# CESNET/GPUJPEG

Measured on NVIDIA H100. Metric: Mpix/s encode+decode 8k RGB q75, higher is better.
Workload: dtype f32+i32 (u8 in, i16 coefficients)

## Files before the change

gpujpeg_b200/csrc/gj_dct.cu:

```cuda
#include <cuda_runtime.h>
#include <stdint.h>
#include <stdlib.h>
#include <string.h>

#include "gj_device.cuh"
#include "gj_internal.h"
#include "gj_launch.cuh"

namespace {

constexpr int TB = 64;
constexpr int NT = 192;
constexpr int STRIP_PX = TB * 8;
constexpr int GROUPS = 8 * (STRIP_PX / 4);
constexpr int BLK_F = 68;
constexpr int K1_SMEM = 3 * TB * BLK_F * 4;
constexpr int K1_OUT_STRIDE = 9;
constexpr int K4_PLANE = 8 * STRIP_PX;

struct FdctParams {
    float fwd_zz[2][64];
};
struct IdctParams {
    uint16_t q_zz[GJ_MAX_COMP][64];
// ... 312 lines not shown
            const int row = g >> 7, gx = g & 127, px0 = gx * 4;
            float4 y4 = make_float4(0.f, 0.f, 0.f, 0.f), cb4 = y4, cr4 = y4;
            if ( row < vh && px0 < vw ) {
                const uint32_t a0 = w0[it], a1 = w1[it], a2 = w2[it];
                gj_rgb_to_ycbcr_m(gj_byte_as_magic(a0, 0), gj_byte_as_magic(a0, 1), gj_byte_as_magic(a0, 2), y4.x, cb4.x, cr4.x);
                gj_rgb_to_ycbcr_m(gj_byte_as_magic(a0, 3), gj_byte_as_magic(a1, 0), gj_byte_as_magic(a1, 1), y4.y, cb4.y, cr4.y);
                gj_rgb_to_ycbcr_m(gj_byte_as_magic(a1, 2), gj_byte_as_magic(a1, 3), gj_byte_as_magic(a2, 0), y4.z, cb4.z, cr4.z);
                gj_rgb_to_ycbcr_m(gj_byte_as_magic(a2, 1), gj_byte_as_magic(a2, 2), gj_byte_as_magic(a2, 3), y4.w, cb4.w, cr4.w);
                if ( px0 + 4 > vw ) {
                    if ( px0 + 1 >= vw ) { y4.y = cb4.y = cr4.y = 0.f; }
                    if ( px0 + 2 >= vw ) { y4.z = cb4.z = cr4.z = 0.f; }
                    if ( px0 + 3 >= vw ) { y4.w = cb4.w = cr4.w = 0.f; }
                }
            }
            *reinterpret_cast<float4*>(s_y + (half * TB + (gx >> 1)) * BLK_F + row * 8 + (gx & 1) * 4) = y4;
            const int srow = half * 8 + row;
            if ( VS == 1 || (srow & 1) == 0 ) {
                const int crow = srow / VS;
                if ( HS == 1 ) {
                    const int off = (gx >> 1) * BLK_F + crow * 8 + (gx & 1) * 4;
                    *reinterpret_cast<float4*>(s_c + off) = cb4;
                    *reinterpret_cast<float4*>(s_c + CB * BLK_F + off) = cr4;
                }
                else {
                    const int off = (gx >> 2) * BLK_F + crow * 8 + (gx & 3) * 2;
                    *reinterpret_cast<float2*>(s_c + off) = make_float2(cb4.x, cb4.z);
                    *reinterpret_cast<float2*>(s_c + CB * BLK_F + off) = make_float2(cr4.x, cr4.z);
                }
            }
        }
    }
    __syncthreads();

    auto locate = [&](int t, int& comp, int& bx, int& by) {
        if ( t < TB * VS ) {
            comp = 0;
            bx = bx0 + (t & (TB - 1));
            by = blockIdx.y * VS + t / TB;
        }
        else {
            const int u = t - TB * VS;
            comp = 1 + u / CB;
            bx = bx0 / HS + u % CB;
            by = blockIdx.y;
        }
        return bx < grid.bcx[comp] && by < grid.bcy[comp];
    };
    int comp, bx, by;
    const bool active = locate(threadIdx.x, comp, bx, by);
    float v[64];
    {
        const float4* in = reinterpret_cast<const float4*>(s_y + threadIdx.x * BLK_F);
#pragma unroll
        for ( int i = 0; i < 16; i++ ) {
            const float4 t = in[i];
            v[4 * i] = t.x; v[4 * i + 1] = t.y; v[4 * i + 2] = t.z; v[4 * i + 3] = t.w;
        }
    }
    __syncthreads();
    gj_fdct_block(v);
    uint4* const s_out = reinterpret_cast<uint4*>(smem);
    {
        uint32_t packed[32];
        const uint64_t nz = quantise_pack(v, prm.fwd_zz[comp == 0 ? 0 : 1], packed);
        if ( active ) nzmask[(size_t)grid.blk_off[comp] + (size_t)by * grid.bcx[comp] + bx] = nz;
#pragma unroll
        for ( int i = 0; i < 8; i++ )
            s_out[threadIdx.x * K1_OUT_STRIDE + i] = make_uint4(packed[4 * i], packed[4 * i + 1], packed[4 * i + 2], packed[4 * i + 3]);
    }
    __syncthreads();
#pragma unroll
    for ( int k = 0; k < 8; k++ ) {
        const int q = threadIdx.x + k * NTS;
        const int slot = q >> 3, part = q & 7;
        int c2, bx2, by2;
        if ( locate(slot, c2, bx2, by2) ) {
            const size_t bi = (size_t)grid.blk_off[c2] + (size_t)by2 * grid.bcx[c2] + bx2;
            reinterpret_cast<uint4*>(coef + bi * 64)[part] = s_out[slot * K1_OUT_STRIDE + part];
        }
    }
}


template <int VEC, int FLAVOUR, bool DEQ>
__global__ void __launch_bounds__(NT)
k_idct_rgb444(const int16_t* __restrict__ coef, int bcx, int nblk, uint8_t* __restrict__ raw, int width, int height,
              size_t pitch, const __grid_constant__ IdctParams prm)
{
    gj_pdl_wait();
    __shared__ __align__(16) uint8_t s_pl[3 * K4_PLANE];

    const int bx0 = blockIdx.x * TB;
    const int by = blockIdx.y;
    const int x0 = bx0 * 8;
    const int vw = min(STRIP_PX, width - x0);
    const int vh = min(8, height - by * 8);

    {
        const int comp = threadIdx.x >> 6;
        const int b = threadIdx.x & 63;
        if ( bx0 + b < bcx ) {
            const uint4* src = reinterpret_cast<const uint4*>(coef + ((size_t)comp * nblk + (size_t)by * bcx + bx0 + b) * 64);
            uint32_t packed[32];
#pragma unroll
            for ( int i = 0; i < 8; i++ ) {
                const uint4 t = __ldg(src + i);
                packed[4 * i] = t.x; packed[4 * i + 1] = t.y; packed[4 * i + 2] = t.z; packed[4 * i + 3] = t.w;
            }
            const uint16_t* q = prm.q_zz[comp];
            uint32_t px[16];
            if ( FLAVOUR == 0 ) {
                int v[64];
#pragma unroll
                for ( int k = 0; k < 64; k++ ) {
                    const int c = (k & 1) ? (int)packed[k >> 1] >> 16 : (int)(short)(packed[k >> 1] & 0xFFFFu);
                    v[gj_zz2nat(k)] = DEQ ? gj_s16(c * (int)(short)q[k]) : c;
                }
                gj_idct_int_block_px(v);
#pragma unroll
                for ( int i = 0; i < 16; i++ )
                    px[i] = pack4_sat_u8(v[4 * i], v[4 * i + 1], v[4 * i + 2], v[4 * i + 3]);
            }
            else {
                float f[64];
#pragma unroll
                for ( int k = 0; k < 64; k++ ) {
                    const int c = (k & 1) ? (int)packed[k >> 1] >> 16 : (int)(short)(packed[k >> 1] & 0xFFFFu);
                    f[gj_zz2nat(k)] = (float)(c * (int)q[k]);
                }
                gj_idct_float_block(f);
#pragma unroll
                for ( int i = 0; i < 16; i++ )
                    px[i] = pack4_sat_u8(GJ_RINT(GJ_FADD(f[4 * i], 128.0f)), GJ_RINT(GJ_FADD(f[4 * i + 1], 128.0f)),
                                         GJ_RINT(GJ_FADD(f[4 * i + 2], 128.0f)), GJ_RINT(GJ_FADD(f[4 * i + 3], 128.0f)));
            }
            uint8_t* dst = s_pl + comp * K4_PLANE + b * 8;
#pragma unroll
            for ( int r = 0; r < 8; r++ )
                *reinterpret_cast<uint2*>(dst + r * STRIP_PX) = make_uint2(px[2 * r], px[2 * r + 1]);
        }
    }
    __syncthreads();

    uint8_t* out = raw + (size_t)by * 8 * pitch + (size_t)x0 * 3;
    for ( int g = threadIdx.x; g < GROUPS; g += NT ) {
        const int row = g >> 7, gx = g & 127;
        const int px0 = gx * 4;
        if ( row >= vh || px0 >= vw ) continue;
        const uint32_t yw = *reinterpret_cast<const uint32_t*>(s_pl + row * STRIP_PX + px0);
        const uint32_t bw = *reinterpret_cast<const uint32_t*>(s_pl + K4_PLANE + row * STRIP_PX + px0);
        const uint32_t rw = *reinterpret_cast<const uint32_t*>(s_pl + 2 * K4_PLANE + row * STRIP_PX + px0);
        int r[4], gg[4], bb[4];
#pragma unroll
        for ( int j = 0; j < 4; j++ )
            gj_ycbcr_to_rgb_raw((yw >> (8 * j)) & 0xFF, (bw >> (8 * j)) & 0xFF, (rw >> (8 * j)) & 0xFF, r[j], gg[j], bb[j]);
        const uint32_t o0 = pack4_sat_u8(r[0], gg[0], bb[0], r[1]);
        const uint32_t o1 = pack4_sat_u8(gg[1], bb[1], r[2], gg[2]);
        const uint32_t o2 = pack4_sat_u8(bb[2], r[3], gg[3], bb[3]);
        uint8_t* p = out + (size_t)row * pitch + gx * 12;
        if ( VEC == 4 && px0 + 4 <= vw ) {
            uint32_t* w = reinterpret_cast<uint32_t*>(p);
            w[0] = o0;
            w[1] = o1;
            w[2] = o2;
        }
        else {
            const int nb = min(12, (vw - px0) * 3);
            const uint32_t o[3] = {o0, o1, o2};
#pragma unroll
            for ( int i = 0; i < 12; i++ )
                if ( i < nb ) p[i] = (uint8_t)(o[i >> 2] >> (8 * (i & 3)));
        }
    }
}

template <int HS, int VS, int VEC, int FLAVOUR, bool DEQ>
__global__ void __launch_bounds__(TB * VS + 2 * TB / HS)
k_idct_rgb_ss(const int16_t* __restrict__ coef, const __grid_constant__ SsGrid grid, uint8_t* __restrict__ raw, int width,
              int height, size_t pitch, const __grid_constant__ IdctParams prm)
{
    gj_pdl_wait();
    constexpr int NTS = TB * VS + 2 * TB / HS;
    constexpr int CB = TB / HS;
    constexpr int CW = STRIP_PX / HS;
    __shared__ __align__(16) uint8_t s_y[8 * VS * STRIP_PX];
    __shared__ __align__(16) uint8_t s_c[2][8 * CW];

    const int bx0 = blockIdx.x * TB;
    const int x0 = bx0 * 8;
    const int y0 = blockIdx.y * 8 * VS;
    const int vw = min(STRIP_PX, width - x0);
    const int vh = min(8 * VS, height - y0);

    {
        int comp, bx, by;
        uint8_t* dst;
        int dpitch;
        if ( threadIdx.x < TB * VS ) {
            comp = 0;
            const int b = threadIdx.x & (TB - 1), byl = threadIdx.x / TB;
            bx = bx0 + b;
            by = blockIdx.y * VS + byl;
            dst = s_y + byl * 8 * STRIP_PX + b * 8;
            dpitch = STRIP_PX;
        }
        else {
            const int u = threadIdx.x - TB * VS;
            comp = 1 + u / CB;
            bx = bx0 / HS + u % CB;
            by = blockIdx.y;
            dst = s_c[comp - 1] + (u % CB) * 8;
            dpitch = CW;
        }
        if ( bx < grid.bcx[comp] && by < grid.bcy[comp] ) {
            const uint4* src =
                reinterpret_cast<const uint4*>(coef + ((size_t)grid.blk_off[comp] + (size_t)by * grid.bcx[comp] + bx) * 64);
            uint32_t packed[32];
#pragma unroll
            for ( int i = 0; i < 8; i++ ) {
                const uint4 t = __ldg(src + i);
                packed[4 * i] = t.x; packed[4 * i + 1] = t.y; packed[4 * i + 2] = t.z; packed[4 * i + 3] = t.w;
            }
            const uint16_t* q = prm.q_zz[comp];
            uint32_t px[16];
            if ( FLAVOUR == 0 ) {
                int v[64];
#pragma unroll
                for ( int k = 0; k < 64; k++ ) {
                    const int c = (k & 1) ? (int)packed[k >> 1] >> 16 : (int)(short)(packed[k >> 1] & 0xFFFFu);
                    v[gj_zz2nat(k)] = DEQ ? gj_s16(c * (int)(short)q[k]) : c;
                }
                gj_idct_int_block_px(v);
#pragma unroll
                for ( int i = 0; i < 16; i++ )
                    px[i] = pack4_sat_u8(v[4 * i], v[4 * i + 1], v[4 * i + 2], v[4 * i + 3]);
            }
            else {
                float f[64];
#pragma unroll
                for ( int k = 0; k < 64; k++ ) {
                    const int c = (k & 1) ? (int)packed[k >> 1] >> 16 : (int)(short)(packed[k >> 1] & 0xFFFFu);
                    f[gj_zz2nat(k)] = (float)(c * (int)q[k]);
                }
                gj_idct_float_block(f);
#pragma unroll
                for ( int i = 0; i < 16; i++ )
                    px[i] = pack4_sat_u8(GJ_RINT(GJ_FADD(f[4 * i], 128.0f)), GJ_RINT(GJ_FADD(f[4 * i + 1], 128.0f)),
                                         GJ_RINT(GJ_FADD(f[4 * i + 2], 128.0f)), GJ_RINT(GJ_FADD(f[4 * i + 3], 128.0f)));
            }
#pragma unroll
            for ( int r = 0; r < 8; r++ )
                *reinterpret_cast<uint2*>(dst + r * dpitch) = make_uint2(px[2 * r], px[2 * r + 1]);
        }
    }
    __syncthreads();

    uint8_t* out = raw + (size_t)y0 * pitch + (size_t)x0 * 3;
    for ( int g = threadIdx.x; g < GROUPS * VS; g += NTS ) {
        const int row = g >> 7, gx = g & 127;
        const int px0 = gx * 4;
        if ( row >= vh || px0 >= vw ) continue;
        const uint32_t yw = *reinterpret_cast<const uint32_t*>(s_y + row * STRIP_PX + px0);
        uint32_t bw, rw;
        if ( HS == 1 ) {
            bw = *reinterpret_cast<const uint32_t*>(s_c[0] + (row / VS) * CW + px0);
            rw = *reinterpret_cast<const uint32_t*>(s_c[1] + (row / VS) * CW + px0);
        }
        else {
            const uint32_t b2 = *reinterpret_cast<const uint16_t*>(s_c[0] + (row / VS) * CW + px0 / 2);
            const uint32_t r2 = *reinterpret_cast<const uint16_t*>(s_c[1] + (row / VS) * CW + px0 / 2);
            bw = __byte_perm(b2, 0u, 0x1100);
            rw = __byte_perm(r2, 0u, 0x1100);
        }
        int r[4], gg[4], bb[4];
#pragma unroll
        for ( int j = 0; j < 4; j++ )
            gj_ycbcr_to_rgb_raw((yw >> (8 * j)) & 0xFF, (bw >> (8 * j)) & 0xFF, (rw >> (8 * j)) & 0xFF, r[j], gg[j], bb[j]);
        const uint32_t o0 = pack4_sat_u8(r[0], gg[0], bb[0], r[1]);
        const uint32_t o1 = pack4_sat_u8(gg[1], bb[1], r[2], gg[2]);
        const uint32_t o2 = pack4_sat_u8(bb[2], r[3], gg[3], bb[3]);
        uint8_t* p = out + (size_t)row * pitch + gx * 12;
        if ( VEC == 4 && px0 + 4 <= vw ) {
            uint32_t* w = reinterpret_cast<uint32_t*>(p);
            w[0] = o0;
            w[1] = o1;
            w[2] = o2;
        }
        else {
            const int nb = min(12, (vw - px0) * 3);
            const uint32_t o[3] = {o0, o1, o2};
#pragma unroll
            for ( int i = 0; i < 12; i++ )
                if ( i < nb ) p[i] = (uint8_t)(o[i >> 2] >> (8 * (i & 3)));
        }
    }
}

struct SampleGrid {
    unsigned long long off[GJ_MAX_COMP], pitch[GJ_MAX_COMP];
    int xs[GJ_MAX_COMP], cw[GJ_MAX_COMP], ch[GJ_MAX_COMP], bcx[GJ_MAX_COMP], blk_off[GJ_MAX_COMP + 1], table[GJ_MAX_COMP];
};
constexpr int SG_THREADS = 128;

__global__ void __launch_bounds__(SG_THREADS)
k_fdct_samples(const uint8_t* __restrict__ raw, const __grid_constant__ SampleGrid g, int total_blocks,
               int16_t* __restrict__ coef, uint64_t* __restrict__ nzmask, const __grid_constant__ FdctParams prm)
{
    const int bi = blockIdx.x * SG_THREADS + threadIdx.x;
    if ( bi >= total_blocks ) return;
    const int comp = (bi >= g.blk_off[1]) + (bi >= g.blk_off[2]) + (bi >= g.blk_off[3]);
    const int local = bi - g.blk_off[comp];
    const int by = local / g.bcx[comp], bx = local - by * g.bcx[comp];
    const int vw = min(8, g.cw[comp] - bx * 8), vh = min(8, g.ch[comp] - by * 8);
    const uint8_t* src = raw + g.off[comp] + (size_t)by * 8 * g.pitch[comp] + (size_t)bx * 8 * g.xs[comp];
    float v[64];
    const bool rows8 = g.xs[comp] == 1 && vw == 8 && ((reinterpret_cast<uintptr_t>(src) | g.pitch[comp]) & 7) == 0;
#pragma unroll
    for ( int y = 0; y < 8; y++ ) {
        if ( y < vh && rows8 ) {
            const uint2 t = __ldg(reinterpret_cast<const uint2*>(src + (size_t)y * g.pitch[comp]));
#pragma unroll
            for ( int x = 0; x < 8; x++ )
                v[8 * y + x] = (float)(((x < 4 ? t.x : t.y) >> (8 * (x & 3))) & 0xFFu);
        }
        else {
#pragma unroll
            for ( int x = 0; x < 8; x++ )
                v[8 * y + x] = (y < vh && x < vw) ? (float)__ldg(src + (size_t)y * g.pitch[comp] + (size_t)x * g.xs[comp]) : 0.f;
        }
    }
    gj_fdct_block(v);
    quantise_store(v, prm.fwd_zz[g.table[comp]], coef + (size_t)bi * 64, nzmask + bi);
}

template <int FLAVOUR, bool DEQ>
__global__ void __launch_bounds__(SG_THREADS)
k_idct_samples(const int16_t* __restrict__ coef, const __grid_constant__ SampleGrid g, int total_blocks,
               uint8_t* __restrict__ raw, const __grid_constant__ IdctParams prm)
{
    const int bi = blockIdx.x * SG_THREADS + threadIdx.x;
    if ( bi >= total_blocks ) return;
    const int comp = (bi >= g.blk_off[1]) + (bi >= g.blk_off[2]) + (bi >= g.blk_off[3]);
    const int local = bi - g.blk_off[comp];
    const int by = local / g.bcx[comp], bx = local - by * g.bcx[comp];
    const int vw = min(8, g.cw[comp] - bx * 8), vh = min(8, g.ch[comp] - by * 8);
    if ( vw <= 0 || vh <= 0 ) return;
    const uint4* src = reinterpret_cast<const uint4*>(coef + (size_t)bi * 64);
    uint32_t packed[32];
#pragma unroll
    for ( int i = 0; i < 8; i++ ) {
        const uint4 t = __ldg(src + i);
        packed[4 * i] = t.x; packed[4 * i + 1] = t.y; packed[4 * i + 2] = t.z; packed[4 * i + 3] = t.w;
    }
    const uint16_t* q = prm.q_zz[comp];
    uint32_t px[16];
    if ( FLAVOUR == 0 ) {
        int v[64];
#pragma unroll
        for ( int k = 0; k < 64; k++ ) {
            const int c = (k & 1) ? (int)packed[k >> 1] >> 16 : (int)(short)(packed[k >> 1] & 0xFFFFu);
            v[gj_zz2nat(k)] = DEQ ? gj_s16(c * (int)(short)q[k]) : c;
        }
        gj_idct_int_block_px(v);
#pragma unroll
        for ( int i = 0; i < 16; i++ )
            px[i] = pack4_sat_u8(v[4 * i], v[4 * i + 1], v[4 * i + 2], v[4 * i + 3]);
    }
    else {
        float f[64];
#pragma unroll
        for ( int k = 0; k < 64; k++ ) {
            const int c = (k & 1) ? (int)packed[k >> 1] >> 16 : (int)(short)(packed[k >> 1] & 0xFFFFu);
            f[gj_zz2nat(k)] = (float)(c * (int)q[k]);
        }
        gj_idct_float_block(f);
#pragma unroll
        for ( int i = 0; i < 16; i++ )
            px[i] = pack4_sat_u8(GJ_RINT(GJ_FADD(f[4 * i], 128.0f)), GJ_RINT(GJ_FADD(f[4 * i + 1], 128.0f)),
                                 GJ_RINT(GJ_FADD(f[4 * i + 2], 128.0f)), GJ_RINT(GJ_FADD(f[4 * i + 3], 128.0f)));
    }
    uint8_t* dst = raw + g.off[comp] + (size_t)by * 8 * g.pitch[comp] + (size_t)bx * 8 * g.xs[comp];
    const bool rows8 = g.xs[comp] == 1 && vw == 8 && ((reinterpret_cast<uintptr_t>(dst) | g.pitch[comp]) & 7) == 0;
#pragma unroll
    for ( int y = 0; y < 8; y++ ) {
        if ( y >= vh ) continue;
        if ( rows8 ) {
            *reinterpret_cast<uint2*>(dst + (size_t)y * g.pitch[comp]) = make_uint2(px[2 * y], px[2 * y + 1]);
        }
        else {
#pragma unroll
            for ( int x = 0; x < 8; x++ )
                if ( x < vw ) dst[(size_t)y * g.pitch[comp] + (size_t)x * g.xs[comp]] = (uint8_t)(px[2 * y + (x >> 2)] >> (8 * (x & 3)));
        }
    }
}

int pick_vec(const void* p, size_t pitch)
{
    const uintptr_t a = reinterpret_cast<uintptr_t>(p) | pitch;
    return (a & 3) == 0 ? 4 : 1;
}

}

static int launch_fdct_rgb444(const uint8_t* d_raw, int width, int height, int pitch, int16_t* d_coef, uint64_t* d_nzmask,
                              int bcx, int bcy, int nblk, const struct gj_dev_enc_tables* h_tables, gj_stream_t stream)
{
    FdctParams prm;
    memcpy(prm.fwd_zz, h_tables->fwd_zz, sizeof prm.fwd_zz);
    const dim3 grid((bcx + TB - 1) / TB, bcy);
    static int attr_done[64];
    int dev = 0;
    if ( cudaGetDevice(&dev) != cudaSuccess || dev < 0 || dev >= 64 ) return -1;
    if ( !__atomic_load_n(&attr_done[dev], __ATOMIC_ACQUIRE) ) {
        if ( cudaFuncSetAttribute(k_fdct_rgb444<4>, cudaFuncAttributeMaxDynamicSharedMemorySize, K1_SMEM) != cudaSuccess ||
             cudaFuncSetAttribute(k_fdct_rgb444<1>, cudaFuncAttributeMaxDynamicSharedMemorySize, K1_SMEM) != cudaSuccess )
            return -1;
        __atomic_store_n(&attr_done[dev], 1, __ATOMIC_RELEASE);
    }
    static int use_bulk = -1;
    if ( use_bulk < 0 ) {
        const char* e = getenv("GPUJPEG_B200_K1");
        use_bulk = e && strcmp(e, "bulk") == 0;
    }
    const bool aligned16 = ((reinterpret_cast<uintptr_t>(d_raw) | (size_t)pitch) & 15) == 0 && ((size_t)(width % STRIP_PX) * 3) % 16 == 0;
    if ( use_bulk && aligned16 ) {
        static int bulk_attr[64];
        if ( !__atomic_load_n(&bulk_attr[dev], __ATOMIC_ACQUIRE) ) {
            if ( cudaFuncSetAttribute(k_fdct_rgb444_bulk, cudaFuncAttributeMaxDynamicSharedMemorySize, K1T_SMEM) != cudaSuccess ) return -1;
            __atomic_store_n(&bulk_attr[dev], 1, __ATOMIC_RELEASE);
        }
        int sms = 132;
        cudaDeviceGetAttribute(&sms, cudaDevAttrMultiProcessorCount, dev);
        const int n_strips = (int)grid.x * (int)grid.y;
        const int ctas = n_strips < sms * 3 ? n_strips : sms * 3;
        k_fdct_rgb444_bulk<<<ctas, NT, K1T_SMEM, stream>>>(d_raw, width, height, (size_t)pitch, d_coef, d_nzmask, bcx, bcy, nblk, prm);
    }
    else if ( pick_vec(d_raw, (size_t)pitch) == 4 )
        gj_launch_pdl(k_fdct_rgb444<4>, grid, dim3(NT), K1_SMEM, stream, d_raw, width, height, (size_t)pitch, d_coef, d_nzmask, bcx, nblk, prm);
    else
        gj_launch_pdl(k_fdct_rgb444<1>, grid, dim3(NT), K1_SMEM, stream, d_raw, width, height, (size_t)pitch, d_coef, d_nzmask, bcx, nblk, prm);
    return cudaGetLastError() == cudaSuccess ? 0 : -1;
}

extern "C" int gj_launch_fdct_rgb444(const uint8_t* d_raw, int width, int height, int pitch, int16_t* d_coef,
                                     uint64_t* d_nzmask, int bcx, int bcy, const struct gj_dev_enc_tables* h_tables,
                                     gj_stream_t stream)
{
    return launch_fdct_rgb444(d_raw, width, height, pitch, d_coef, d_nzmask, bcx, bcy, bcx * bcy, h_tables, stream);
}
extern "C" int gj_launch_fdct_rgb444_rows(const uint8_t* d_raw, int width, int height, int pitch, int16_t* d_coef,
                                          uint64_t* d_nzmask, int bcx, int bcy, int by0, int by1,
                                          const struct gj_dev_enc_tables* h_tables, gj_stream_t stream)
{
    if ( by0 < 0 || by1 > bcy || by0 >= by1 ) return -1;
    const int rows = (by1 * 8 < height ? by1 * 8 : height) - by0 * 8;
    return launch_fdct_rgb444(d_raw + (ptrdiff_t)by0 * 8 * pitch, width, rows, pitch, d_coef + (size_t)by0 * bcx * 64,
                              d_nzmask + (size_t)by0 * bcx, bcx, by1 - by0, bcx * bcy, h_tables, stream);
}

static int launch_idct_rgb444(const int16_t* d_coef, int bcx, int bcy, int nblk, const int comp_tq[3], uint8_t* d_raw, int width,
                              int height, int pitch, int idct_flavour, int coef_dequantized,
                              const struct gj_dev_dec_tables* h_tables, gj_stream_t stream)
{
    IdctParams prm;
    for ( int c = 0; c < 3; c++ )
        memcpy(prm.q_zz[c], h_tables->qinv_zz[comp_tq[c]], sizeof prm.q_zz[c]);
    const dim3 grid((bcx + TB - 1) / TB, bcy);
    const int vec = pick_vec(d_raw, (size_t)pitch);
    if ( idct_flavour != 0 && coef_dequantized ) return -1;
#define GJ_K4(V, F, D) gj_launch_pdl(k_idct_rgb444<V, F, D>, grid, dim3(NT), 0, stream, d_coef, bcx, nblk, d_raw, width, height, (size_t)pitch, prm)
    if ( idct_flavour == 0 && coef_dequantized ) {
        if ( vec == 4 ) GJ_K4(4, 0, false); else GJ_K4(1, 0, false);
    }
    else if ( idct_flavour == 0 ) {
        if ( vec == 4 ) GJ_K4(4, 0, true); else GJ_K4(1, 0, true);
    }
    else {
        if ( vec == 4 ) GJ_K4(4, 1, true); else GJ_K4(1, 1, true);
    }
#undef GJ_K4
    return cudaGetLastError() == cudaSuccess ? 0 : -1;
}
extern "C" int gj_launch_idct_rgb444(const int16_t* d_coef, int bcx, int bcy, const int comp_tq[3], uint8_t* d_raw,
                                     int width, int height, int pitch, int idct_flavour, int coef_dequantized,
                                     const struct gj_dev_dec_tables* h_tables, gj_stream_t stream)
{
    return launch_idct_rgb444(d_coef, bcx, bcy, bcx * bcy, comp_tq, d_raw, width, height, pitch, idct_flavour, coef_dequantized,
                              h_tables, stream);
}
extern "C" int gj_launch_idct_rgb444_rows(const int16_t* d_coef, int bcx, int bcy, int by0, int by1, const int comp_tq[3],
                                          uint8_t* d_raw, int width, int height, int pitch, int idct_flavour,
                                          int coef_dequantized, const struct gj_dev_dec_tables* h_tables, gj_stream_t stream)
{
    if ( by0 < 0 || by1 > bcy || by0 >= by1 ) return -1;
    const int rows = (by1 * 8 < height ? by1 * 8 : height) - by0 * 8;
    return launch_idct_rgb444(d_coef + (size_t)by0 * bcx * 64, bcx, by1 - by0, bcx * bcy, comp_tq, d_raw + (ptrdiff_t)by0 * 8 * pitch,
                              width, rows, pitch, idct_flavour, coef_dequantized, h_tables, stream);
}

static int ss_grid_rows(SsGrid* sg, const struct gj_comp_geo comp[3], int my0, int my1, int height)
{
    const int vs = comp[0].vs;
    for ( int c = 0; c < 3; c++ ) {
        const int per = c == 0 ? vs : 1;
        const int lo = my0 * per, hi = my1 * per < comp[c].bcy ? my1 * per : comp[c].bcy;
        sg->bcx[c] = comp[c].bcx;
        sg->bcy[c] = hi > lo ? hi - lo : 0;
        sg->blk_off[c] = comp[c].blk_off + lo * comp[c].bcx;
    }
    const int y0 = my0 * 8 * vs, y1 = my1 * 8 * vs < height ? my1 * 8 * vs : height;
    return y1 > y0 ? y1 - y0 : 0;
}

extern "C" int gj_launch_fdct_rgb_ss_rows(const uint8_t* d_raw, int width, int height, int pitch, int16_t* d_coef,
                                          uint64_t* d_nzmask, const struct gj_comp_geo comp[3], int my0, int my1,
                                          const struct gj_dev_enc_tables* h_tables, gj_stream_t stream)
{
    FdctParams prm;
    memcpy(prm.fwd_zz, h_tables->fwd_zz, sizeof prm.fwd_zz);
    const int hs = comp[0].hs, vs = comp[0].vs;
    if ( comp[1].hs != 1 || comp[1].vs != 1 || comp[2].hs != 1 || comp[2].vs != 1 ) return -1;
    const int mcu_rows = (comp[0].bcy + vs - 1) / vs;
    if ( my0 < 0 || my1 > mcu_rows || my0 >= my1 ) return -1;
    SsGrid sg;
    height = ss_grid_rows(&sg, comp, my0, my1, height);
    d_raw += (ptrdiff_t)my0 * 8 * vs * pitch;
    const dim3 grid((comp[0].bcx + TB - 1) / TB, my1 - my0);
    const int vec = pick_vec(d_raw, (size_t)pitch);
    static int attr_done[64][4];
    int dev = 0;
    if ( cudaGetDevice(&dev) != cudaSuccess || dev < 0 || dev >= 64 ) return -1;
#define GJ_K1SS(H, V)                                                                                                        \
    do {                                                                                                                     \
        constexpr int nt = TB * V + 2 * TB / H;                                                                              \
        constexpr int sm = nt * BLK_F * 4;                                                                                   \
        if ( !__atomic_load_n(&attr_done[dev][H * 2 + V - 3], __ATOMIC_ACQUIRE) ) {                                          \
            if ( cudaFuncSetAttribute(k_fdct_rgb_ss<H, V, 4>, cudaFuncAttributeMaxDynamicSharedMemorySize, sm) != cudaSuccess || \
                 cudaFuncSetAttribute(k_fdct_rgb_ss<H, V, 1>, cudaFuncAttributeMaxDynamicSharedMemorySize, sm) != cudaSuccess )  \
                return -1;                                                                                                   \
            __atomic_store_n(&attr_done[dev][H * 2 + V - 3], 1, __ATOMIC_RELEASE);                                           \
        }                                                                                                                    \
        if ( vec == 4 )                                                                                                      \
            gj_launch_pdl(k_fdct_rgb_ss<H, V, 4>, grid, dim3(nt), sm, stream, d_raw, width, height, (size_t)pitch, d_coef, d_nzmask, sg, prm); \
        else                                                                                                                 \
            gj_launch_pdl(k_fdct_rgb_ss<H, V, 1>, grid, dim3(nt), sm, stream, d_raw, width, height, (size_t)pitch, d_coef, d_nzmask, sg, prm); \
    } while ( 0 )
    if ( hs == 2 && vs == 2 ) GJ_K1SS(2, 2);
    else if ( hs == 2 && vs == 1 ) GJ_K1SS(2, 1);
    else if ( hs == 1 && vs == 2 ) GJ_K1SS(1, 2);
    else return -1;
#undef GJ_K1SS
    return cudaGetLastError() == cudaSuccess ? 0 : -1;
}
extern "C" int gj_launch_fdct_rgb_ss(const uint8_t* d_raw, int width, int height, int pitch, int16_t* d_coef,
                                     uint64_t* d_nzmask, const struct gj_comp_geo comp[3],
                                     const struct gj_dev_enc_tables* h_tables, gj_stream_t stream)
{
    const int vs = comp[0].vs > 0 ? comp[0].vs : 1;
    return gj_launch_fdct_rgb_ss_rows(d_raw, width, height, pitch, d_coef, d_nzmask, comp, 0, (comp[0].bcy + vs - 1) / vs, h_tables,
                                      stream);
}

extern "C" int gj_launch_idct_rgb_ss_rows(const int16_t* d_coef, const struct gj_comp_geo comp[3], int my0, int my1,
                                          const int comp_tq[3], uint8_t* d_raw, int width, int height, int pitch, int idct_flavour,
                                          int coef_dequantized, const struct gj_dev_dec_tables* h_tables, gj_stream_t stream)
{
    IdctParams prm;
    for ( int c = 0; c < 3; c++ )
        memcpy(prm.q_zz[c], h_tables->qinv_zz[comp_tq[c]], sizeof prm.q_zz[c]);
    const int hs = comp[0].hs, vs = comp[0].vs;
    if ( comp[1].hs != 1 || comp[1].vs != 1 || comp[2].hs != 1 || comp[2].vs != 1 ) return -1;
    if ( idct_flavour != 0 && coef_dequantized ) return -1;
    const int mcu_rows = (comp[0].bcy + vs - 1) / vs;
    if ( my0 < 0 || my1 > mcu_rows || my0 >= my1 ) return -1;
    SsGrid sg;
    height = ss_grid_rows(&sg, comp, my0, my1, height);
    d_raw += (ptrdiff_t)my0 * 8 * vs * pitch;
    const dim3 grid((comp[0].bcx + TB - 1) / TB, my1 - my0);
    const int vec = pick_vec(d_raw, (size_t)pitch);
#define GJ_K4SS2(H, V, VE, F, D) \
    gj_launch_pdl(k_idct_rgb_ss<H, V, VE, F, D>, grid, dim3(TB * V + 2 * TB / H), 0, stream, d_coef, sg, d_raw, width, height, (size_t)pitch, prm)
#define GJ_K4SS(H, V)                                                                  \
    do {                                                                               \
        if ( idct_flavour == 0 && coef_dequantized ) {                                 \
            if ( vec == 4 ) GJ_K4SS2(H, V, 4, 0, false); else GJ_K4SS2(H, V, 1, 0, false); \
        }                                                                              \
        else if ( idct_flavour == 0 ) {                                                \
            if ( vec == 4 ) GJ_K4SS2(H, V, 4, 0, true); else GJ_K4SS2(H, V, 1, 0, true);   \
        }                                                                              \
        else {                                                                         \
            if ( vec == 4 ) GJ_K4SS2(H, V, 4, 1, true); else GJ_K4SS2(H, V, 1, 1, true);   \
        }                                                                              \
    } while ( 0 )
    if ( hs == 2 && vs == 2 ) GJ_K4SS(2, 2);
    else if ( hs == 2 && vs == 1 ) GJ_K4SS(2, 1);
    else if ( hs == 1 && vs == 2 ) GJ_K4SS(1, 2);
    else return -1;
#undef GJ_K4SS
#undef GJ_K4SS2
    return cudaGetLastError() == cudaSuccess ? 0 : -1;
}
extern "C" int gj_launch_idct_rgb_ss(const int16_t* d_coef, const struct gj_comp_geo comp[3], const int comp_tq[3],
                                     uint8_t* d_raw, int width, int height, int pitch, int idct_flavour,
                                     int coef_dequantized, const struct gj_dev_dec_tables* h_tables, gj_stream_t stream)
{
    const int vs = comp[0].vs > 0 ? comp[0].vs : 1;
    return gj_launch_idct_rgb_ss_rows(d_coef, comp, 0, (comp[0].bcy + vs - 1) / vs, comp_tq, d_raw, width, height, pitch,
                                      idct_flavour, coef_dequantized, h_tables, stream);
}

static int sample_grid(SampleGrid* sg, const struct gj_raw_layout* raw, const struct gj_comp_geo* comp, int comp_count,
                       const uint8_t* comp_tbl)
{
    if ( comp_count < 1 || comp_count > GJ_MAX_COMP || raw->comp_count != comp_count ) return -1;
    memset(sg, 0, sizeof *sg);
    int total = 0;
    for ( int c = 0; c < GJ_MAX_COMP; c++ ) {
        const int k = c < comp_count ? c : comp_count - 1;
        sg->off[c] = raw->comp[k].off;
        sg->pitch[c] = raw->comp[k].pitch;
        sg->xs[c] = raw->comp[k].xs;
        sg->cw[c] = comp[k].width;
        sg->ch[c] = comp[k].height;
        sg->bcx[c] = comp[k].bcx;
        sg->table[c] = comp_tbl ? comp_tbl[k] : ((c == 0 || c == 3) ? 0 : 1);
        if ( c < comp_count ) {
            sg->blk_off[c] = comp[c].blk_off;
            total = comp[c].blk_off + comp[c].nblk;
        }
    }
    for ( int c = comp_count; c <= GJ_MAX_COMP; c++ )
        sg->blk_off[c] = 0x7FFFFFFF;
    return total;
}

extern "C" int gj_launch_fdct_samples(const uint8_t* d_raw, const struct gj_raw_layout* raw, int16_t* d_coef,
                                      uint64_t* d_nzmask, const struct gj_comp_geo* comp, int comp_count,
                                      const uint8_t* comp_tbl, const struct gj_dev_enc_tables* h_tables, gj_stream_t stream)
{
    FdctParams prm;
    memcpy(prm.fwd_zz, h_tables->fwd_zz, sizeof prm.fwd_zz);
    SampleGrid sg;
    const int total = sample_grid(&sg, raw, comp, comp_count, comp_tbl);
    if ( total <= 0 ) return -1;
    k_fdct_samples<<<(total + SG_THREADS - 1) / SG_THREADS, SG_THREADS, 0, stream>>>(d_raw, sg, total, d_coef, d_nzmask, prm);
    return cudaGetLastError() == cudaSuccess ? 0 : -1;
}

extern "C" int gj_launch_idct_samples(const int16_t* d_coef, const struct gj_comp_geo* comp, int comp_count, const int* comp_tq,
                                      uint8_t* d_raw, const struct gj_raw_layout* raw, int idct_flavour, int coef_dequantized,
                                      const struct gj_dev_dec_tables* h_tables, gj_stream_t stream)
{
    IdctParams prm;
    for ( int c = 0; c < GJ_MAX_COMP; c++ )
        memcpy(prm.q_zz[c], h_tables->qinv_zz[comp_tq[c < comp_count ? c : 0]], sizeof prm.q_zz[c]);
    SampleGrid sg;
    const int total = sample_grid(&sg, raw, comp, comp_count, nullptr);
    if ( total <= 0 ) return -1;
    if ( idct_flavour != 0 && coef_dequantized ) return -1;
    const int grid = (total + SG_THREADS - 1) / SG_THREADS;
    if ( idct_flavour == 0 && coef_dequantized )
        k_idct_samples<0, false><<<grid, SG_THREADS, 0, stream>>>(d_coef, sg, total, d_raw, prm);
    else if ( idct_flavour == 0 )
        k_idct_samples<0, true><<<grid, SG_THREADS, 0, stream>>>(d_coef, sg, total, d_raw, prm);
    else
        k_idct_samples<1, true><<<grid, SG_THREADS, 0, stream>>>(d_coef, sg, total, d_raw, prm);
    return cudaGetLastError() == cudaSuccess ? 0 : -1;
}
```

gpujpeg_b200/csrc/gj_decoder.c:

```c
#include <stdlib.h>
#include <string.h>

#include "gj_internal.h"

#define GJ_MK_OTHER_CAP 256
#define GJ_CTA_BYTES0 (64 * 1024)
#define GJ_MK_WORDS (8 + 4 * GJ_MK_OTHER_CAP)

#define GJ_STRIPES 8
#define GJ_STRIPE_MIN_BYTES ((size_t)8 << 20)

struct gpujpeg_decoder {
    gj_stream_t stream;
    gj_stream_t copy_stream;
    void* ev_stripe[GJ_STRIPES]; void* ev_done;
    int stripes;
    size_t stripe_min_bytes;
    int k3_parts;
    int device;
    int verbose, perf_stats;
    struct gpujpeg_parameters param;
    struct gpujpeg_image_parameters param_image;
    struct gj_geometry geo;
    int initialised;
    enum gpujpeg_pixel_format req_pixel_format;
    enum gpujpeg_color_space req_color_space;
    int idct_flavour;
    int flipped;
    unsigned channel_remap;
    int thread_per_segment;
    int force_lanes[GJ_MAX_COMP];
    int sm_count;
    int ff_cs_itu601_is_709;
    int out_mode;
    uint8_t* d_planes; size_t d_planes_size;
    struct gj_raw_layout raw;
    struct gpujpeg_image_metadata metadata;

    struct gj_dev_dec_tables h_tab, h_tab_prev;
    struct gj_dev_dec_tables* d_tab;
    int tab_valid;

    uint8_t* d_file; size_t d_file_size;
    uint32_t* d_list_pos; size_t d_list_pos_size;
    uint8_t* d_list_code; size_t d_list_code_size;
    uint32_t* d_list_cpos; size_t d_list_cpos_size;
    uint8_t* d_clean; size_t d_clean_size;
    uint32_t* d_seg_tab; size_t d_seg_tab_size;
    uint32_t* d_seg_off; uint32_t* h_seg_off; size_t seg_off_size;
    int used_segment_info;
    int ignore_segment_info;
    unsigned long long* d_cta; size_t d_cta_size;
    uint32_t* d_mk;
    uint32_t* d_k3_ctr;
    uint32_t* h_mk;
    int16_t* d_coef; size_t d_coef_size;
    uint8_t* d_raw; size_t d_raw_size;
    uint8_t* h_raw; size_t h_raw_size;

    struct gj_timer t_to, t_from, t_huff, t_dct, t_gpu;
    int timers_ok;
    struct gpujpeg_duration_stats stats;
    int stats_valid;

    struct gj_huff_dec_args last_args;
    size_t last_ecs_begin; uint32_t last_list_cap;
    int last_tq[GJ_MAX_COMP];
    int last_valid;

    int last_progressive;
    struct gj_prog_args last_prog;
    struct gj_prog_scan* prog_scans;
    struct gj_dec_lut* h_prog_luts;
    struct gj_dec_lut* d_prog_luts;
};

void gpujpeg_decoder_output_set_default(struct gpujpeg_decoder_output* output)
{
    memset(output, 0, sizeof *output);
    output->type = GPUJPEG_DECODER_OUTPUT_INTERNAL_BUFFER;
}
void gpujpeg_decoder_output_set_custom(struct gpujpeg_decoder_output* output, uint8_t* custom_buffer)
{
    memset(output, 0, sizeof *output);
    output->type = GPUJPEG_DECODER_OUTPUT_CUSTOM_BUFFER;
    output->data = custom_buffer;
}
void gpujpeg_decoder_output_set_texture(struct gpujpeg_decoder_output* output, struct gpujpeg_opengl_texture* texture)
{
    memset(output, 0, sizeof *output);
    output->type = GPUJPEG_DECODER_OUTPUT_OPENGL_TEXTURE;
    output->texture = texture;
}
void gpujpeg_decoder_output_set_cuda_buffer(struct gpujpeg_decoder_output* output)
{
    memset(output, 0, sizeof *output);
    output->type = GPUJPEG_DECODER_OUTPUT_CUDA_BUFFER;
}
void gpujpeg_decoder_output_set_custom_cuda(struct gpujpeg_decoder_output* output, uint8_t* d_custom_buffer)
{
    memset(output, 0, sizeof *output);
    output->type = GPUJPEG_DECODER_OUTPUT_CUSTOM_CUDA_BUFFER;
    output->data = d_custom_buffer;
}

struct gpujpeg_decoder_init_parameters gpujpeg_decoder_default_init_parameters(void)
{
    struct gpujpeg_decoder_init_parameters p;
    memset(&p, 0, sizeof p);
    return p;
}

struct gpujpeg_decoder* gpujpeg_decoder_create_with_params(const struct gpujpeg_decoder_init_parameters* params)
{
    struct gpujpeg_decoder* d = (struct gpujpeg_decoder*)calloc(1, sizeof *d);
    if ( !d ) return NULL;
    d->stream = (gj_stream_t)params->stream;
    d->verbose = params->verbose;
    d->perf_stats = params->perf_stats;
    d->ff_cs_itu601_is_709 = params->ff_cs_itu601_is_709;
    d->device = gj_cuda_get_device();
    d->sm_count = gj_cuda_sm_count();
    d->req_pixel_format = GPUJPEG_PIXFMT_AUTODETECT;
    d->k3_parts = -1;
    d->req_color_space = GPUJPEG_CS_DEFAULT;
    if ( d->device < 0 || gj_cuda_malloc((void**)&d->d_tab, sizeof *d->d_tab) ||
         gj_cuda_malloc((void**)&d->d_mk, GJ_MK_WORDS * 4 + GJ_CTA_BYTES0) || gj_cuda_malloc((void**)&d->d_k3_ctr, 32) ||
         gj_cuda_memset_async(d->d_k3_ctr, 0, 32, d->stream) || gj_cuda_stream_sync(d->stream) ||
         gj_cuda_malloc_host((void**)&d->h_mk, GJ_MK_WORDS * 4) ) {
        GJ_ERR("Decoder allocation failed: %s\n", gj_cuda_last_error());
        free(d);
        return NULL;
    }
    d->timers_ok = !(gj_timer_create(&d->t_to) || gj_timer_create(&d->t_from) || gj_timer_create(&d->t_huff) ||
                     gj_timer_create(&d->t_dct) || gj_timer_create(&d->t_gpu));
    return d;
}

struct gpujpeg_decoder* gpujpeg_decoder_create(cudaStream_t stream)
{
    struct gpujpeg_decoder_init_parameters p = gpujpeg_decoder_default_init_parameters();
    p.stream = stream;
    return gpujpeg_decoder_create_with_params(&p);
}

int gpujpeg_decoder_destroy(struct gpujpeg_decoder* d)
{
    if ( !d ) return -1;
    gj_cuda_free(d->d_tab);
    gj_cuda_free(d->d_file);
    gj_cuda_free(d->d_list_pos);
    gj_cuda_free(d->d_list_code);
    gj_cuda_free(d->d_list_cpos);
    gj_cuda_free(d->d_clean);
    gj_cuda_free(d->d_seg_tab);
    gj_cuda_free(d->d_seg_off);
    if ( d->h_seg_off ) gj_cuda_free_host(d->h_seg_off);
    gj_cuda_free(d->d_mk);
    gj_cuda_free(d->d_k3_ctr);
    gj_cuda_free_host(d->h_mk);
    gj_cuda_free(d->d_coef);
    gj_cuda_free(d->d_planes);
    gj_cuda_free(d->d_raw);
    gj_cuda_free_host(d->h_raw);
    gj_cuda_free(d->d_prog_luts);
    free(d->prog_scans);
    free(d->h_prog_luts);
    if ( d->copy_stream ) gj_cuda_stream_destroy(d->copy_stream);
    gj_cuda_event_destroy(d->ev_done);
    for ( int i = 0; i < GJ_STRIPES; i++ )
        gj_cuda_event_destroy(d->ev_stripe[i]);
    gj_timer_destroy(&d->t_to);
    gj_timer_destroy(&d->t_from);
    gj_timer_destroy(&d->t_huff);
    gj_timer_destroy(&d->t_dct);
    gj_timer_destroy(&d->t_gpu);
    free(d);
    return 0;
}

static int grow_dev(void** p, size_t* have, size_t want)
{
    if ( *have >= want ) return 0;
    gj_cuda_free(*p);
    *p = NULL;
    *have = 0;
    if ( gj_cuda_malloc(p, want) ) return -1;
    *have = want;
    return 0;
}
static int grow_host(void** p, size_t* have, size_t want)
{
    if ( *have >= want ) return 0;
    gj_cuda_free_host(*p);
    *p = NULL;
    *have = 0;
    if ( gj_cuda_malloc_host(p, want) ) return -1;
    *have = want;
    return 0;
}

static int grow_mk_cta(struct gpujpeg_decoder* d, size_t cta_bytes)
{
    if ( d->d_cta && cta_bytes <= d->d_cta_size ) return 0;
    if ( !d->d_cta && cta_bytes <= GJ_CTA_BYTES0 ) {
        d->d_cta = (unsigned long long*)(d->d_mk + GJ_MK_WORDS);
        d->d_cta_size = GJ_CTA_BYTES0;
        return 0;
    }
    const size_t want = cta_bytes + cta_bytes / 4;
    uint32_t* fresh = NULL;
    if ( gj_cuda_stream_sync(d->stream) || gj_cuda_malloc((void**)&fresh, GJ_MK_WORDS * 4 + want) ) return -1;
    gj_cuda_free(d->d_mk);
    d->d_mk = fresh;
    d->d_cta = (unsigned long long*)(fresh + GJ_MK_WORDS);
    d->d_cta_size = want;
    return 0;
}

int gpujpeg_decoder_init(struct gpujpeg_decoder* d, const struct gpujpeg_parameters* param,
                         const struct gpujpeg_image_parameters* param_image)
{
    d->verbose = param->verbose;
    d->perf_stats = param->perf_stats || param->verbose >= GPUJPEG_LL_STATUS;
    if ( param_image->width <= 0 || param_image->height <= 0 || param->comp_count <= 0 ) return 0;
    if ( (size_t)param_image->width * (size_t)param_image->height > ((size_t)1 << 30) ) {
        GJ_ERR("Image size %dx%d exceeds the supported maximum of 2^30 pixels.\n", param_image->width, param_image->height);
        return -1;
    }
    struct gpujpeg_parameters p = *param;
    struct gpujpeg_image_parameters pi = *param_image;
    if ( p.comp_count != 3 && p.comp_count != 1 && p.comp_count != 4 ) {
        GJ_ERR("This build decodes 1-, 3- and 4-component images only.\n");
        return -1;
    }
    if ( (int)pi.pixel_format < 0 )
        pi.pixel_format = p.comp_count == 1 ? GPUJPEG_U8 : p.comp_count == 4 ? GPUJPEG_4444_U8_P0123 : GPUJPEG_444_U8_P012;
    gj_geometry_init(&d->geo, &p, &pi);
    const struct gj_geometry* g = &d->geo;
    if ( grow_dev((void**)&d->d_coef, &d->d_coef_size, g->coef_count * 2) ||
         grow_dev((void**)&d->d_raw, &d->d_raw_size, g->raw_size) ) {
        GJ_ERR("Decoder device allocation failed: %s\n", gj_cuda_last_error());
        return -1;
    }
    d->param = p;
    d->param_image = pi;
    d->initialised = 1;
    return 0;
}

void gpujpeg_decoder_set_output_format(struct gpujpeg_decoder* decoder, enum gpujpeg_color_space color_space,
                                       enum gpujpeg_pixel_format pixel_format)
{
    decoder->req_color_space = color_space;
    decoder->req_pixel_format = pixel_format;
}

enum { GJ_OUT_RGB = 1, GJ_OUT_SAMPLES = 2, GJ_OUT_GENERIC = 3 };

static int choose_output(const struct gpujpeg_decoder* d, const struct gj_stream* st, struct gpujpeg_image_parameters* pi)
{
    enum gpujpeg_pixel_format pf = d->req_pixel_format;
    enum gpujpeg_color_space cs = d->req_color_space;
    const int special = (int)pf < 0;
    if ( st->comp_count == 1 ) {
        if ( !special && pf != GPUJPEG_U8 ) {
            GJ_ERR("This build decodes 1-component JPEGs to GPUJPEG_U8 only (%s requested).\n", gpujpeg_pixel_format_get_name(pf));
            return 0;
        }
        pi->pixel_format = GPUJPEG_U8;
        pi->color_space = (cs == GPUJPEG_CS_DEFAULT || cs == GPUJPEG_NONE) ? GPUJPEG_YCBCR_JPEG : cs;
        return GJ_OUT_SAMPLES;
    }
    const int lh = st->comp_hv[0] >> 4, lv = st->comp_hv[0] & 15;
    if ( cs == GPUJPEG_CS_DEFAULT ) cs = GPUJPEG_RGB;
    if ( cs == GPUJPEG_NONE ) cs = st->color_space;
    if ( special ) {
        const int planar_by_sampling = pf == GPUJPEG_PIXFMT_STD && cs != GPUJPEG_RGB;
        if ( pf == GPUJPEG_PIXFMT_NATIVE && st->comp_count == 4 ) pf = GPUJPEG_4444_U8_P0123;
        else if ( pf == GPUJPEG_PIXFMT_NATIVE || planar_by_sampling ) {
            const int il = pf == GPUJPEG_PIXFMT_NATIVE && st->scan[0].ncomp > 1;
            if ( lh == 2 && lv == 2 ) pf = GPUJPEG_420_U8_P0P1P2;
            else if ( lh == 2 && lv == 1 ) pf = il ? GPUJPEG_422_U8_P1020 : GPUJPEG_422_U8_P0P1P2;
            else pf = il ? GPUJPEG_444_U8_P012 : GPUJPEG_444_U8_P0P1P2;
        }
        else {
            pf = st->comp_count == 4 && pf != GPUJPEG_PIXFMT_NO_ALPHA ? GPUJPEG_4444_U8_P0123 : GPUJPEG_444_U8_P012;
        }
    }
    pi->pixel_format = pf;
    pi->color_space = cs;
    if ( st->comp_count == 3 && cs == GPUJPEG_RGB && pf == GPUJPEG_444_U8_P012 && st->color_space == GPUJPEG_YCBCR_BT601_256LVLS )
        return GJ_OUT_RGB;
    if ( cs != GPUJPEG_RGB && cs != GPUJPEG_YCBCR_BT601 && cs != GPUJPEG_YCBCR_BT601_256LVLS && cs != GPUJPEG_YCBCR_BT709 ) {
        GJ_ERR("Colour space %s is not produced by this build.\n", gpujpeg_color_space_get_name(cs));
        return 0;
    }
    struct gj_raw_layout rl;
    if ( gj_raw_layout_init(&rl, pi) || rl.comp_count != 3 ) {
        GJ_ERR("Pixel format %s (%dx%d) is not produced by this build.\n", gpujpeg_pixel_format_get_name(pf), pi->width,
               pi->height);
        return 0;
    }
    if ( st->comp_count == 4 || cs != st->color_space || rl.sampling[0].horizontal != lh || rl.sampling[0].vertical != lv ||
         rl.alpha_off ) {
        if ( (pi->width & 1) && rl.sampling[0].horizontal == 2 && pf != GPUJPEG_420_U8_P0P1P2 ) {
            GJ_ERR("Odd widths are only produced without colour / sampling conversion for this pixel format.\n");
            return 0;
        }
        return GJ_OUT_GENERIC;
    }
    return GJ_OUT_SAMPLES;
}

static int launch_k4(struct gpujpeg_decoder* d, const int comp_tq[GJ_MAX_COMP], uint8_t* d_out, int coef_dequantized)
{
    const struct gj_geometry* g = &d->geo;
    if ( d->out_mode == GJ_OUT_SAMPLES )
        return gj_launch_idct_samples(d->d_coef, g->comp, g->comp_count, comp_tq, d_out, &d->raw, d->idct_flavour,
                                      coef_dequantized, &d->h_tab, d->stream);
    if ( d->out_mode == GJ_OUT_GENERIC ) {
        struct gj_raw_layout pl;
        struct gj_comp_geo padded[GJ_MAX_COMP];
        gj_planes_layout(&pl, padded, g->comp, g->comp_count);
        if ( gj_launch_idct_samples(d->d_coef, padded, g->comp_count, comp_tq, d->d_planes, &pl, d->idct_flavour,
                                    coef_dequantized, &d->h_tab, d->stream) )
            return -1;
        if ( d->flipped && gj_launch_flip_planes(d->d_planes, padded, g->comp_count, d->stream) ) return -1;
        return gj_launch_convert_out(d->d_planes, d_out, &d->raw, d->param_image.pixel_format, d->param_image.color_space,
                                     d->param.color_space_internal,
                                     g->width, g->height, g->comp, g->comp_count, g->max_hs, g->max_vs, d->stream);
    }
    int pitch = g->pitch;
    if ( d->flipped ) {
        d_out += (size_t)(g->height - 1) * (size_t)g->pitch;
        pitch = -pitch;
    }
    if ( g->lay.simple )
        return gj_launch_idct_rgb444(d->d_coef, g->bcx, g->bcy, comp_tq, d_out, g->width, g->height, pitch, d->idct_flavour,
                                     coef_dequantized, &d->h_tab, d->stream);
    return gj_launch_idct_rgb_ss(d->d_coef, g->comp, comp_tq, d_out, g->width, g->height, pitch, d->idct_flavour,
                                 coef_dequantized, &d->h_tab, d->stream);
}

static int stripes_usable(struct gpujpeg_decoder* d)
{
    const struct gj_geometry* g = &d->geo;
    if ( d->out_mode != GJ_OUT_RGB || d->flipped || d->channel_remap ) return 0;
    if ( d->stripes == 0 ) {
        const char* v = getenv("GPUJPEG_B200_STRIPES");
        const char* m = getenv("GPUJPEG_B200_STRIPE_MIN_BYTES");
        d->stripe_min_bytes = m ? (size_t)strtoull(m, NULL, 0) : GJ_STRIPE_MIN_BYTES;
        d->stripes = v ? atoi(v) : GJ_STRIPES;
        if ( d->stripes < 1 ) d->stripes = 1;
        if ( d->stripes > GJ_STRIPES ) d->stripes = GJ_STRIPES;
    }
    if ( d->stripes < 2 || g->bcy / g->max_vs < 2 * d->stripes || g->raw_size < d->stripe_min_bytes ) return 0;
    if ( !d->copy_stream ) {
        if ( gj_cuda_stream_create(&d->copy_stream) || gj_cuda_event_create(&d->ev_done) ) {
            d->stripes = 1;
            return 0;
        }
        for ( int i = 0; i < GJ_STRIPES; i++ )
            if ( gj_cuda_event_create(&d->ev_stripe[i]) ) {
                d->stripes = 1;
                return 0;
            }
    }
    return 1;
}

static int decode_striped(struct gpujpeg_decoder* d, const int comp_tq[GJ_MAX_COMP], uint8_t* d_out, uint8_t* h_dst, int coef_dequantized,
                          const struct gj_huff_dec_args* k3 )
{
    const struct gj_geometry* g = &d->geo;
    struct gj_huff_dec_args part;
    int segs_done[GJ_MAX_COMP] = {0, 0, 0, 0};
    if ( k3 ) part = *k3;
    const int mcu_h = 8 * g->max_vs;
    const int mcu_rows = (g->bcy + g->max_vs - 1) / g->max_vs;
    for ( int i = 0; i < d->stripes; i++ ) {
        const int my0 = (int)((long long)mcu_rows * i / d->stripes), my1 = (int)((long long)mcu_rows * (i + 1) / d->stripes);
        const size_t row0 = (size_t)my0 * mcu_h, row1 = (size_t)my1 * mcu_h < (size_t)g->height ? (size_t)my1 * mcu_h : (size_t)g->height;
        const size_t off = row0 * (size_t)g->pitch;
        const size_t bytes = (i + 1 == d->stripes ? g->raw_size : row1 * (size_t)g->pitch) - off;
        if ( k3 ) {
            int any = 0;
            for ( int k = 0; k < g->scan_count; k++ ) {
                const int segs = g->lay.scan_seg_begin[k + 1] - g->lay.scan_seg_begin[k];
                long long hi = i + 1 == d->stripes ? segs : (((long long)my1 * g->bcx + g->seg_mcu - 1) / g->seg_mcu + 31) / 32 * 32;
                if ( hi > segs ) hi = segs;
                part.part_seg_lo[k] = segs_done[k];
                part.part_seg_hi[k] = (int)hi;
                if ( (int)hi > segs_done[k] ) any = 1;
                segs_done[k] = (int)hi;
            }
            if ( any ) {
                for ( int k = 0; k < g->scan_count; k++ )
                    if ( part.part_seg_hi[k] == 0 ) part.part_seg_lo[k] = 0;
                if ( gj_launch_huffman_decode(&part, d->stream) ) return -1;
            }
        }
        const int rc = g->lay.simple ? gj_launch_idct_rgb444_rows(d->d_coef, g->bcx, g->bcy, my0, my1, comp_tq, d_out, g->width, g->height,
                                                                  g->pitch, d->idct_flavour, coef_dequantized, &d->h_tab, d->stream)
                                     : gj_launch_idct_rgb_ss_rows(d->d_coef, g->comp, my0, my1, comp_tq, d_out, g->width, g->height, g->pitch,
                                                                  d->idct_flavour, coef_dequantized, &d->h_tab, d->stream);
        if ( rc ||
             gj_cuda_event_record(d->ev_stripe[i], d->stream) || gj_cuda_stream_wait_event(d->copy_stream, d->ev_stripe[i]) ||
             gj_cuda_memcpy_d2h_async(h_dst + off, d_out + off, bytes, d->copy_stream) )
            return -1;
    }
    if ( gj_cuda_event_record(d->ev_done, d->copy_stream) || gj_cuda_stream_wait_event(d->stream, d->ev_done) ) return -1;
    return 0;
}

static int resync_segments(struct gpujpeg_decoder* d, const struct gj_stream* st, const uint32_t first_rank[GJ_MAX_COMP],
                           const uint32_t end_rank[GJ_MAX_COMP], const uint32_t scan_cbegin[GJ_MAX_COMP], struct gj_huff_dec_args* ha)
{
    const struct gj_geometry* g = &d->geo;
    const uint32_t n_list = end_rank[g->scan_count - 1] + 1;
    uint8_t* code = (uint8_t*)malloc((size_t)n_list);
    uint32_t* pos = (uint32_t*)malloc((size_t)n_list * 8);
    uint32_t* tab = (uint32_t*)malloc((size_t)g->seg_count * 12);
    int rc = -1;
    if ( code && pos && tab && !gj_cuda_memcpy_d2h_async(code, d->d_list_code, n_list, d->stream) &&
         !gj_cuda_memcpy_d2h_async(pos, d->d_list_pos, (size_t)n_list * 4, d->stream) &&
         !gj_cuda_memcpy_d2h_async(pos + n_list, d->d_list_cpos, (size_t)n_list * 4, d->stream) && !gj_cuda_stream_sync(d->stream) ) {
        const uint32_t* cpos = pos + n_list;
        for ( int k = 0; k < g->scan_count; k++ ) {
            const int seg0 = g->lay.scan_seg_begin[k], segs = g->lay.scan_seg_begin[k + 1] - seg0;
            int n = 0, prev = 7;
            uint32_t start_raw = (uint32_t)st->scan[k].begin, start_clean = scan_cbegin[k];
            uint32_t m = first_rank[k];
            while ( m < end_rank[k] && n < segs ) {
                const int expected = (prev + 1) & 7;
                tab[3 * (seg0 + n)] = start_raw;
                tab[3 * (seg0 + n) + 1] = start_clean;
                tab[3 * (seg0 + n) + 2] = cpos[m];
                n++;
                if ( (code[m] & 7) != expected ) {
                    GJ_ERR("Expected marker 0x%X but 0x%X was presented!\n", 0xD0 + expected, code[m]);
                    uint32_t q = m + 1;
                    while ( q < end_rank[k] && code[q] != 0xD0 + expected ) q++;
                    if ( q >= end_rank[k] ) {
                        GJ_ERR("No marker 0x%X was found until end of current scan!\n", 0xD0 + expected);
                        m = end_rank[k] + 1;
                        break;
                    }
                    fprintf(stderr, "[GPUJPEG] [Recovery] Skipping %u bytes of data until marker 0x%X was found!\n",
                            pos[q] - pos[m], 0xD0 + expected);
                    m = q;
                }
                prev = expected;
                start_raw = pos[m] + 2;
                start_clean = cpos[m];
                m++;
            }
            if ( m <= end_rank[k] && n < segs ) {
                tab[3 * (seg0 + n)] = start_raw;
                tab[3 * (seg0 + n) + 1] = start_clean;
                tab[3 * (seg0 + n) + 2] = cpos[end_rank[k]];
                n++;
            }
            for ( ; n < segs; n++ ) {
                tab[3 * (seg0 + n)] = 0xFFFFFFFFu;
                tab[3 * (seg0 + n) + 1] = tab[3 * (seg0 + n) + 2] = 0;
            }
        }
        if ( !grow_dev((void**)&d->d_seg_tab, &d->d_seg_tab_size, (size_t)g->seg_count * 12) &&
             !gj_cuda_memcpy_h2d_async(d->d_seg_tab, tab, (size_t)g->seg_count * 12, d->stream) &&
             !gj_cuda_memset_async(d->d_mk + 3, 0, 4, d->stream) && !gj_cuda_stream_sync(d->stream) ) {
            ha->d_seg_tab = d->d_seg_tab;
            rc = 0;
        }
    }
    if ( rc ) GJ_ERR("Restart resynchronisation failed: %s\n", gj_cuda_last_error());
    free(code);
    free(pos);
    free(tab);
    return rc;
}

static int wants_thread_per_segment(const struct gpujpeg_decoder* d, const struct gj_geometry* g, size_t ecs_bytes)
{
    const size_t bytes_per_block_x10 = ecs_bytes * 10 / (g->coef_count / 64);
    const int many_segments = g->seg_count >= 30000;
    return d->thread_per_segment || g->lay.interleaved || g->seg_mcu * g->lay.bpm > 40 ||
           (many_segments && (bytes_per_block_x10 < 80 || bytes_per_block_x10 > 200));
// ... 267 lines not shown
        GJ_ERR("Decoder allocation failed: %s\n", gj_cuda_last_error());
        return GPUJPEG_ERROR;
    }
    const size_t ecs_begin = st->scan[0].begin;
    const uint32_t list_cap = (uint32_t)((image_size - ecs_begin) / 2 + 1 + GJ_MK_OTHER_CAP);
    uint32_t first_rank[GJ_MAX_SCANS], end_rank[GJ_MAX_SCANS], scan_cbegin[GJ_MAX_SCANS];
    memset(first_rank, 0, sizeof first_rank);
    memset(end_rank, 0, sizeof end_rank);
    memset(scan_cbegin, 0, sizeof scan_cbegin);
    if ( upload_file(d, image, image_size, ecs_begin, list_cap, stats) ||
         k0_scan_extents(d, image, image_size, ecs_begin, list_cap, st, &pos, &adobe, first_rank, end_rank, scan_cbegin) ||
         gj_reader_finish(st, adobe, d->verbose) )
        return GPUJPEG_ERROR;
    d->metadata = st->metadata;
    if ( st->color_space != early_cs ) {
        GJ_ERR("The stream's colour space (%s) is announced after its first scan header; not supported.\n",
               gpujpeg_color_space_get_name(st->color_space));
        return GPUJPEG_ERROR;
    }
    int il = 0;
    for ( int k = 0; k < st->scan_count; k++ )
        il |= st->scan[k].ncomp > 1;
    if ( il != p->interleaved ) {
        p->interleaved = il;
        if ( gpujpeg_decoder_init(d, p, pi) ) return GPUJPEG_ERROR;
        if ( d->out_mode == GJ_OUT_GENERIC && grow_dev((void**)&d->d_planes, &d->d_planes_size, d->geo.coef_count) ) return GPUJPEG_ERROR;
    }
    const struct gj_geometry* g = &d->geo;

    int nlut = 0;
    for ( int k = 0; k < st->scan_count; k++ ) {
        struct gj_prog_scan* S = &d->prog_scans[k];
        if ( gj_prog_scan_init(g, st, k, st->restart_interval, S) ) {
            GJ_ERR("Unsupported scan structure (progressive scan %d: components out of frame order or outside the frame).\n", k);
            return GPUJPEG_ERROR;
        }
        S->first_rank = first_rank[k];
        S->cbegin = scan_cbegin[k];
        if ( end_rank[k] >= list_cap || end_rank[k] - first_rank[k] != (uint32_t)(S->seg_count - 1) ) {
            GJ_ERR("JPEG stream has a broken restart-marker structure (progressive scan %d holds %u restart markers, expected %d)!\n",
                   k, end_rank[k] - first_rank[k], S->seg_count - 1);
            return GPUJPEG_ERROR;
        }
        S->lut0 = nlut;
        const int nt = S->kind == GJ_PROG_DC_FIRST ? S->ncomp : S->kind == GJ_PROG_DC_REFINE ? 0 : 1;
        for ( int i = 0; i < nt; i++ ) {
            if ( !st->scan[k].huff_at[i] ) {
                GJ_ERR("Huffman table used by progressive scan %d is missing!\n", k);
                return GPUJPEG_ERROR;
            }
            struct gj_huff_spec spec;
            gj_huff_spec_at(image, st->scan[k].huff_at[i], &spec);
            if ( gj_dec_lut_build(&spec, &d->h_prog_luts[nlut++]) ) {
                GJ_ERR("Invalid Huffman table (progressive scan %d)!\n", k);
                return GPUJPEG_ERROR;
            }
        }
    }
    memset(&d->h_tab, 0, sizeof d->h_tab);
    for ( int c = 0; c < st->comp_count; c++ ) {
        const uint8_t* q = st->have_comp_qt[c] ? st->comp_qt[c] : st->have_qt[st->comp_tq[c]] ? st->qt[st->comp_tq[c]] : NULL;
        for ( int k = 0; q && k < 64; k++ )
            d->h_tab.qinv_zz[c][k] = q[k];
    }
    const double t_reader_ms = (gpujpeg_get_time() - t_begin) * 1000.0;
    if ( !d->tab_valid || memcmp(&d->h_tab, &d->h_tab_prev, sizeof d->h_tab) != 0 ) {
        d->h_tab_prev = d->h_tab;
        if ( gj_cuda_memcpy_h2d_async(d->d_tab, &d->h_tab_prev, sizeof d->h_tab, d->stream) ) return GPUJPEG_ERROR;
        d->tab_valid = 1;
    }
    if ( nlut && gj_cuda_memcpy_h2d_async(d->d_prog_luts, d->h_prog_luts, sizeof(struct gj_dec_lut) * (size_t)nlut, d->stream) )
        return GPUJPEG_ERROR;

    struct gj_prog_args* a = &d->last_prog;
    memset(a, 0, sizeof *a);
    a->scans = d->prog_scans;
    a->scan_count = st->scan_count;
    a->d_luts = d->d_prog_luts;
    a->d_clean = (const uint32_t*)d->d_clean;
    a->d_list_cpos = d->d_list_cpos;
    a->d_list_code = d->d_list_code;
    a->d_error = d->d_mk + 3;
    a->d_coef = d->d_coef;
    a->coef_count = g->coef_count;
    a->dequantize = d->idct_flavour == 0;
    a->comp_count = g->comp_count;
    for ( int c = 0; c < g->comp_count; c++ )
        a->comp_blk_off[c] = g->comp[c].blk_off;
    a->d_tables = d->d_tab;
    d->last_args.file_size = image_size;
    d->last_ecs_begin = ecs_begin;
    d->last_list_cap = list_cap;
    d->last_progressive = 1;
    d->last_valid = 1;
    if ( stats && d->timers_ok ) {
        gj_timer_start(&d->t_gpu, d->stream);
        gj_timer_start(&d->t_huff, d->stream);
    }
    if ( gj_launch_progressive_decode(a, d->stream) ) {
        GJ_ERR("Progressive Huffman decoder launch failed: %s\n", gj_cuda_last_error());
        return GPUJPEG_ERROR;
    }
    if ( stats && d->timers_ok ) {
        gj_timer_stop(&d->t_huff, d->stream);
        gj_timer_start(&d->t_dct, d->stream);
    }
    const int to_host = output->type == GPUJPEG_DECODER_OUTPUT_INTERNAL_BUFFER || output->type == GPUJPEG_DECODER_OUTPUT_CUSTOM_BUFFER;
    const int striped = to_host && !stats && stripes_usable(d);
    if ( k4_and_output(d, output, pi, comp_tq, a->dequantize, striped, NULL, stats) ) return GPUJPEG_ERROR;
    if ( gj_cuda_memcpy_d2h_async(d->h_mk, d->d_mk, 16, d->stream) || gj_cuda_stream_sync(d->stream) ) {
        GJ_ERR("Decoder failed: %s\n", gj_cuda_last_error());
        return GPUJPEG_ERROR;
    }
    if ( d->h_mk[3] ) {
        GJ_ERR("Restart marker with the wrong number in a progressive scan; not supported.\n");
        d->last_valid = 0;
        return GPUJPEG_ERROR;
    }
    output->metadata = &d->metadata;
    record_stats(d, output, pi, stats, t_reader_ms, t_begin);
    return GPUJPEG_NOERR;
}

int gpujpeg_decoder_decode(struct gpujpeg_decoder* d, uint8_t* image, size_t image_size,
                           struct gpujpeg_decoder_output* output)
{
    if ( !d || !image || !output ) return GPUJPEG_ERROR;
    const int stats = d->perf_stats || d->verbose >= GPUJPEG_LL_STATUS;
    const double t_begin = gpujpeg_get_time();

    struct gj_stream st;
    gj_reader_begin(&st, d->ff_cs_itu601_is_709);
    st.verbose = d->verbose;
    if ( image_size < 4 || image[0] != 0xFF || image[1] != 0xD8 ) {
        GJ_ERR("JPEG data should begin with SOI marker!\n");
        return GPUJPEG_ERROR;
    }
    if ( image_size >= 0xFFFFFFFFull ) {
        GJ_ERR("JPEG streams of 4 GiB or more are not supported.\n");
        return GPUJPEG_ERROR;
    }
    size_t pos = 2;
    int adobe = -1;
    if ( gj_reader_walk(image, image_size, &pos, &st, &adobe) != 1 ) {
        GJ_ERR("Decoder failed when decoding image data (no scan found)!\n");
        return GPUJPEG_ERROR;
    }
    if ( st.comp_count != 3 && st.comp_count != 1 && st.comp_count != 4 ) {
        GJ_ERR("This build decodes 1-, 3- and 4-component JPEGs only (stream has %d).\n", st.comp_count);
        return GPUJPEG_ERROR;
    }
    if ( st.comp_count == 1 ) st.comp_hv[0] = 0x11;
    if ( st.comp_count >= 3 ) {
        const int lh = st.comp_hv[0] >> 4, lv = st.comp_hv[0] & 15;
        if ( lh < 1 || lh > 2 || lv < 1 || lv > 2 || st.comp_hv[1] != 0x11 || st.comp_hv[2] != 0x11 ||
             (st.comp_count == 4 && st.comp_hv[3] != st.comp_hv[0]) ) {
            GJ_ERR("This build decodes 4:4:4, 4:2:2, 4:2:0 and 4:4:0 only (sampling factors %dx%d %dx%d %dx%d).\n", lh, lv,
                   st.comp_hv[1] >> 4, st.comp_hv[1] & 15, st.comp_hv[2] >> 4, st.comp_hv[2] & 15);
            return GPUJPEG_ERROR;
        }
    }
    st.interleaved = st.scan[0].ncomp > 1;
    if ( !st.progressive && st.interleaved && st.scan[0].ncomp != st.comp_count ) {
        GJ_ERR("Unsupported scan structure (%d components in first scan).\n", st.scan[0].ncomp);
        return GPUJPEG_ERROR;
    }
// ... 98 lines not shown
        }
        for ( int k = 0; k < st.scan[s].ncomp; k++ ) {
            const int td = st.scan[s].td[k], ta = st.scan[s].ta[k];
            if ( !st.have_huff[0][td] || !st.have_huff[1][ta] ) {
                GJ_ERR("Huffman table (DC %d / AC %d) used by scan %d is missing!\n", td, ta, s);
                return GPUJPEG_ERROR;
            }
            ha.scan_comp[s][k] = st.scan[s].comp[k];
            ha.scan_td[s][k] = td;
            ha.scan_tq[s][k] = st.comp_tq[st.scan[s].comp[k]];
            ha.scan_ta[s][k] = ta;
        }
        ha.scan_begin[s] = (uint32_t)st.scan[s].begin;
    }
    for ( int cls = 0; cls < 2; cls++ )
        for ( int id = 0; id < 4; id++ )
            if ( st.have_huff[cls][id] ) {
                if ( gj_dec_lut_build(&st.huff[cls][id], &d->h_tab.lut[cls][id]) ) {
                    GJ_ERR("Invalid Huffman table (class %d id %d)!\n", cls, id);
                    return GPUJPEG_ERROR;
                }
                gj_dec_fast_build(&st.huff[cls][id], cls, &d->h_tab.fast[cls][id]);
            }
    const double t_reader_ms = (gpujpeg_get_time() - t_begin) * 1000.0;

    if ( !d->tab_valid || memcmp(&d->h_tab, &d->h_tab_prev, sizeof d->h_tab) != 0 ) {
        d->h_tab_prev = d->h_tab;
        if ( gj_cuda_memcpy_h2d_async(d->d_tab, &d->h_tab_prev, sizeof d->h_tab, d->stream) ) return GPUJPEG_ERROR;
        d->tab_valid = 1;
    }
    if ( stats && d->timers_ok ) {
        gj_timer_start(&d->t_gpu, d->stream);
        gj_timer_start(&d->t_huff, d->stream);
    }
    int resync = 0;
    for ( int k = 0; k < g->scan_count && !by_table; k++ ) {
        const int segs = g->lay.scan_seg_begin[k + 1] - g->lay.scan_seg_begin[k];
        if ( end_rank[k] >= list_cap ) {
            GJ_ERR("JPEG stream has a broken restart-marker structure (scan %d holds %u restart markers, expected %d "
                   "for a %dx%d image with restart interval %d)!\n", k, end_rank[k] - first_rank[k], segs - 1, st.width,
                   st.height, st.restart_interval);
            return GPUJPEG_ERROR;
        }
        if ( end_rank[k] - first_rank[k] != (uint32_t)(segs - 1) ) resync = 1;
    }

    ha.d_file = d->d_file;
    ha.file_size = image_size;
    ha.dequantize = d->idct_flavour == 0;
    ha.d_seg_off = by_table ? d->d_seg_off : NULL;
    ha.d_seg_len = NULL;
    ha.d_list_pos = d->d_list_pos;
    ha.d_list_code = d->d_list_code;
    ha.d_error = d->d_mk + 3;
    ha.d_unit_ctr = d->d_k3_ctr;
    ha.d_clean = (const uint32_t*)d->d_clean;
    ha.d_list_cpos = d->d_list_cpos;
    ha.force_thread_per_segment = d->thread_per_segment;
    size_t ecs_bytes = 0;
    for ( int k = 0; k < g->scan_count; k++ )
        ecs_bytes += st.scan[k].end - st.scan[k].begin;
    const size_t bytes_per_block_x10 = ecs_bytes * 10 / (g->coef_count / 64);
    const int many_segments = g->seg_count >= 30000;
    ha.force_thread_per_segment = by_table || wants_thread_per_segment(d, g, ecs_bytes);
    for ( int k = 0; k < g->scan_count; k++ ) {
        ha.first_rank[k] = first_rank[k];
        ha.scan_cbegin[k] = scan_cbegin[k];
        const int segs = g->lay.scan_seg_begin[k + 1] - g->lay.scan_seg_begin[k];
        const size_t avg = (st.scan[k].end - st.scan[k].begin) / (size_t)segs;
        ha.scan_lanes[k] = (uint8_t)(g->seg_count <= 8000 ? 16
                                     : !many_segments     ? (bytes_per_block_x10 > 100 ? 16 : 8)
                                     : 32);
        if ( d->force_lanes[k] ) {
            ha.scan_lanes[k] = (uint8_t)d->force_lanes[k];
            ha.force_thread_per_segment = d->thread_per_segment;
        }
        ha.scan_bytes[k] = (uint32_t)(st.scan[k].end - st.scan[k].begin);
        ha.scan_dense[k] = avg >= (size_t)16 * (size_t)(g->seg_mcu * g->lay.bpm);
    }
    ha.seg_count = g->seg_count;
    ha.lay = g->lay;
    ha.seg_mcu = g->seg_mcu;
    ha.d_coef = d->d_coef;
    ha.d_tables = d->d_tab;
    d->last_args = ha;
    d->last_ecs_begin = ecs_begin;
    d->last_list_cap = list_cap;
    memcpy(d->last_tq, st.comp_tq, sizeof d->last_tq);
    d->last_valid = 1;
    d->last_progressive = 0;
  for ( int pass = 0;; pass++ ) {
    if ( resync ) {
        if ( resync_segments(d, &st, first_rank, end_rank, scan_cbegin, &ha) ) return GPUJPEG_ERROR;
        d->last_args = ha;
    }
    const int to_host = output->type == GPUJPEG_DECODER_OUTPUT_INTERNAL_BUFFER || output->type == GPUJPEG_DECODER_OUTPUT_CUSTOM_BUFFER;
    const int striped = to_host && !stats && stripes_usable(d);
    if ( d->k3_parts < 0 ) {
        const char* v = getenv("GPUJPEG_B200_STRIPES_K3");
        d->k3_parts = !(v && v[0] == '0');
    }
    const int k3_striped = striped && d->k3_parts && !resync && gj_huffman_decode_parts_eligible(&ha);
    if ( !k3_striped && gj_launch_huffman_decode(&ha, d->stream) ) {
        GJ_ERR("Huffman decoder launch failed: %s\n", gj_cuda_last_error());
        return GPUJPEG_ERROR;
    }
    if ( stats && d->timers_ok ) {
        gj_timer_stop(&d->t_huff, d->stream);
        gj_timer_start(&d->t_dct, d->stream);
    }

    if ( k4_and_output(d, output, &pi, st.comp_tq, ha.dequantize, striped, k3_striped ? &ha : NULL, stats) ) return GPUJPEG_ERROR;
    if ( gj_cuda_memcpy_d2h_async(d->h_mk, d->d_mk, 16, d->stream) || gj_cuda_stream_sync(d->stream) ) {
        GJ_ERR("Decoder failed: %s\n", gj_cuda_last_error());
        return GPUJPEG_ERROR;
    }
    if ( d->h_mk[3] && by_table ) {
        GJ_VERBOSE(d->verbose, "Segment info of the stream does not match its restart markers; decoding by marker scan.\n");
        d->ignore_segment_info = 1;
        const int rc = gpujpeg_decoder_decode(d, image, image_size, output);
        d->ignore_segment_info = 0;
        return rc;
    }
    if ( d->h_mk[3] && !resync && pass == 0 ) {
        resync = 1;
        continue;
    }
    break;
  }
    output->metadata = &d->metadata;

    record_stats(d, output, &pi, stats, t_reader_ms, t_begin);
    return GPUJPEG_NOERR;
}

int gpujpeg_decoder_get_stats(struct gpujpeg_decoder* decoder, struct gpujpeg_duration_stats* stats)
{
    if ( !decoder || !stats || !decoder->stats_valid ) return -1;
    *stats = decoder->stats;
    return 0;
}

int gpujpeg_decoder_get_image_info2(uint8_t* image, size_t image_size, struct gpujpeg_image_info* info, int verbose,
                                    unsigned flags)
{
    struct gj_stream st;
    if ( gj_reader_parse(image, image_size, &st, verbose) ) return -1;
    memset(info, 0, sizeof *info);
    gpujpeg_image_set_default_parameters(&info->param_image);
    gpujpeg_set_default_parameters(&info->param);
    info->param_image.width = st.width;
    info->param_image.height = st.height;
    info->param_image.color_space = st.color_space;
    info->param_image.pixel_format = st.comp_count == 1 ? GPUJPEG_U8 : st.comp_count == 4 ? GPUJPEG_4444_U8_P0123 : GPUJPEG_444_U8_P012;
    if ( st.comp_count == 3 && st.comp_hv[1] == 0x11 && st.comp_hv[2] == 0x11 ) {
        const int il = st.interleaved;
        if ( st.comp_hv[0] == 0x22 ) info->param_image.pixel_format = GPUJPEG_420_U8_P0P1P2;
        else if ( st.comp_hv[0] == 0x21 ) info->param_image.pixel_format = il ? GPUJPEG_422_U8_P1020 : GPUJPEG_422_U8_P0P1P2;
        else info->param_image.pixel_format = il ? GPUJPEG_444_U8_P012 : GPUJPEG_444_U8_P0P1P2;
    }
    info->param.comp_count = st.comp_count;
    info->param.restart_interval = st.restart_interval;
    info->param.interleaved = st.interleaved;
    info->param.color_space_internal = st.color_space;
    for ( int c = 0; c < st.comp_count; c++ ) {
        info->param.sampling_factor[c].horizontal = (uint8_t)(st.comp_hv[c] >> 4);
// ... 49 lines not shown
        if ( strcmp(val, GPUJPEG_DEC_HUFFMAN_VAL_AUTO) == 0 ) decoder->thread_per_segment = 0;
        else if ( strcmp(val, GPUJPEG_DEC_HUFFMAN_VAL_THREAD_PER_SEGMENT) == 0 ) decoder->thread_per_segment = 1;
        else {
            GJ_ERR("Unknown Huffman decoder kernel: %s\n", val);
            return GPUJPEG_ERROR;
        }
        return GPUJPEG_NOERR;
    }
    if ( strcmp(opt, GPUJPEG_DEC_OPT_HUFFMAN_LANES) == 0 ) {
        int lanes[GJ_MAX_COMP] = {0, 0, 0, 0}, count = 0;
        const char* p = val;
        while ( *p && count < GJ_MAX_COMP ) {
            const int n = atoi(p);
            if ( n < 0 || n > 32 || (n & (n - 1)) ) {
                GJ_ERR("Lanes per restart segment must be 0 (automatic) or a power of two up to 32 (got %s).\n", val);
                return GPUJPEG_ERROR;
            }
            lanes[count++] = n;
            while ( *p && *p != ',' ) p++;
            if ( *p == ',' ) p++;
        }
        for ( int k = 0; k < GJ_MAX_COMP; k++ )
            decoder->force_lanes[k] = count == 1 ? lanes[0] : lanes[k];
        return GPUJPEG_NOERR;
    }
    if ( strcmp(opt, GPUJPEG_DEC_OPT_FLIPPED_BOOL) == 0 ) {
        const int b = gj_parse_bool(val, GPUJPEG_DEC_OPT_FLIPPED_BOOL);
        if ( b < 0 ) return GPUJPEG_ERROR;
        decoder->flipped = b;
        return GPUJPEG_NOERR;
    }
    if ( strcmp(opt, GPUJPEG_DEC_OPT_CHANNEL_REMAP) == 0 ) {
        const unsigned m = gj_parse_channel_remap(val, GPUJPEG_DEC_OPT_CHANNEL_REMAP);
        if ( !m ) return GPUJPEG_ERROR;
        decoder->channel_remap = m;
        return GPUJPEG_NOERR;
    }
    if ( strcmp(opt, GPUJPEG_DEC_OPT_TGA_RLE_BOOL) == 0 || strcmp(opt, GPUJPEG_DEC_OPT_ALIGNMENT_BYTES_INT) == 0 ) {
        GJ_ERR("Decoder option %s is not implemented in this build.\n", opt);
        return GPUJPEG_ERROR;
    }
    GJ_ERR("Invalid decoder option: %s!\n", opt);
    return GPUJPEG_ERROR;
}

void gpujpeg_decoder_print_options(void)
{
    printf("\t" GPUJPEG_DEC_OPT_IDCT "=[" GPUJPEG_DEC_IDCT_VAL_INT "|" GPUJPEG_DEC_IDCT_VAL_FLOAT_GPUREF
           "] - inverse DCT flavour (default: int = gpujpeg_idct_cpu)\n");
    printf("\t" GPUJPEG_DEC_OPT_FLIPPED_BOOL "=[" GPUJPEG_VAL_FALSE "|" GPUJPEG_VAL_TRUE "] - flip the decoded image vertically\n");
    printf("\t" GPUJPEG_DEC_OPT_CHANNEL_REMAP "=XYZ[W] - output channel mapping (as the encoder option)\n");
}

GPUJPEG_API int gpujpegx_decoder_used_segment_info(const struct gpujpeg_decoder* d)
{
    return d && d->last_valid ? d->used_segment_info : -1;
}

GPUJPEG_API int gpujpegx_decoder_run_resident(struct gpujpeg_decoder* d, uint8_t* d_out, int stage_mask)
{
    if ( !d || !d->last_valid ) return -1;
    if ( d->last_progressive ) {
        static const int comp_tq[GJ_MAX_COMP] = {0, 1, 2, 3};
        if ( (stage_mask & 4) &&
             gj_launch_marker_scan(d->d_file, d->last_ecs_begin, d->last_args.file_size, d->d_cta, d->d_list_pos, d->d_list_code,
                                   d->d_list_cpos, d->last_list_cap, d->d_clean, d->d_mk, d->d_mk + 8, GJ_MK_OTHER_CAP, d->stream) )
            return -1;
        if ( (stage_mask & 1) && gj_launch_progressive_decode(&d->last_prog, d->stream) ) return -1;
        if ( (stage_mask & 2) && launch_k4(d, comp_tq, d_out ? d_out : d->d_raw, d->last_prog.dequantize) ) return -1;
        return 0;
    }
    if ( (stage_mask & 4) && !d->used_segment_info &&
         gj_launch_marker_scan(d->d_file, d->last_ecs_begin, d->last_args.file_size, d->d_cta, d->d_list_pos, d->d_list_code,
                               d->d_list_cpos, d->last_list_cap, d->d_clean, d->d_mk, d->d_mk + 8, GJ_MK_OTHER_CAP, d->stream) )
        return -1;
    if ( (stage_mask & 1) && gj_launch_huffman_decode(&d->last_args, d->stream) ) return -1;
    if ( (stage_mask & 2) && launch_k4(d, d->last_tq, d_out ? d_out : d->d_raw, d->last_args.dequantize) ) return -1;
    return 0;
}

GPUJPEG_API int gpujpegx_decoder_get_coefficients(struct gpujpeg_decoder* d, int16_t* out, size_t count)
{
    if ( !d || !d->initialised || !d->last_valid || count != d->geo.coef_count ) return -1;
    if ( gj_coef_to_host_natural(d->d_coef, count, out, d->stream) ) return -1;
    return (d->last_progressive ? d->last_prog.dequantize : d->last_args.dequantize) ? 1 : 0;
}
```

gpujpeg_b200/csrc/gj_device.cuh:

```cuda
#ifndef GJ_DEVICE_CUH
#define GJ_DEVICE_CUH

#include <stdint.h>
#include <math.h>

#include "gj_internal.h"

#if defined(__CUDA_ARCH__)
#define GJ_HD __host__ __device__ __forceinline__
#define GJ_FADD(a, b) __fadd_rn((a), (b))
#define GJ_FSUB(a, b) __fsub_rn((a), (b))
#define GJ_FMUL(a, b) __fmul_rn((a), (b))
#define GJ_FMA(a, b, c) __fmaf_rn((a), (b), (c))
#define GJ_RINT(a) __float2int_rn(a)
#elif defined(__CUDACC__)
#define GJ_HD __host__ __device__ __forceinline__
#define GJ_FADD(a, b) ((a) + (b))
#define GJ_FSUB(a, b) ((a) - (b))
#define GJ_FMUL(a, b) ((a) * (b))
#define GJ_FMA(a, b, c) fmaf((a), (b), (c))
#define GJ_RINT(a) ((int)rintf(a))
#else
#define GJ_HD static inline
#define GJ_FADD(a, b) ((a) + (b))
#define GJ_FSUB(a, b) ((a) - (b))
#define GJ_FMUL(a, b) ((a) * (b))
#define GJ_FMA(a, b, c) fmaf((a), (b), (c))
#define GJ_RINT(a) ((int)rintf(a))
#endif


GJ_HD constexpr int gj_zz2nat(int k)
{
    constexpr int t[64] = {0,  1,  8,  16, 9,  2,  3,  10, 17, 24, 32, 25, 18, 11, 4,  5,  12, 19, 26, 33, 40, 48,
                           41, 34, 27, 20, 13, 6,  7,  14, 21, 28, 35, 42, 49, 56, 57, 50, 43, 36, 29, 22, 15, 23,
                           30, 37, 44, 51, 58, 59, 52, 45, 38, 31, 39, 46, 53, 60, 61, 54, 47, 55, 62, 63};
    return t[k];
}
GJ_HD constexpr int gj_nat2zz(int n)
{
    constexpr int t[64] = {0,  1,  5,  6,  14, 15, 27, 28, 2,  4,  7,  13, 16, 26, 29, 42, 3,  8,  12, 17, 25, 30,
                           41, 43, 9,  11, 18, 24, 31, 40, 44, 53, 10, 19, 23, 32, 39, 45, 52, 54, 20, 22, 33, 38,
                           46, 51, 55, 60, 21, 34, 37, 47, 50, 56, 59, 61, 35, 36, 48, 49, 57, 58, 62, 63};
    return t[n];
}


#define GJ_MAGIC23 8388608.0f
#define GJ_MAGIC15 12582912.0f
GJ_HD float gj_byte_as_magic(uint32_t word, int i)
{
#if defined(__CUDA_ARCH__)
    return __uint_as_float(__byte_perm(word, 0x4B000000u, 0x7440 + i));
#else
    union { uint32_t u; float f; } c;
    c.u = 0x4B000000u | ((word >> (8 * i)) & 0xFFu);
    return c.f;
#endif
}
GJ_HD float gj_scale255_m(float cm) { return fmaxf(cm, fmaf(cm, 2.0f, -(GJ_MAGIC23 + 254.0f))) - GJ_MAGIC23; }
GJ_HD float gj_round_clamp255(float acc) { return fminf(acc + GJ_MAGIC15, GJ_MAGIC15 + 255.0f) - GJ_MAGIC15; }
GJ_HD void gj_rgb_to_ycbcr_m(float rm, float gm, float bm, float& y, float& cb, float& cr)
{
    const float r = gj_scale255_m(rm), g = gj_scale255_m(gm), b = gj_scale255_m(bm);
    const float e = 1.0f / 512.0f;
    y = gj_round_clamp255(fmaf(77.0f / 256.0f, r, fmaf(150.0f / 256.0f, g, fmaf(29.0f / 256.0f, b, e))));
    cb = gj_round_clamp255(fmaf(-43.0f / 256.0f, r, fmaf(-85.0f / 256.0f, g, fmaf(128.0f / 256.0f, b, 128.0f + e))));
    cr = gj_round_clamp255(fmaf(128.0f / 256.0f, r, fmaf(-107.0f / 256.0f, g, fmaf(-21.0f / 256.0f, b, 128.0f + e))));
}
GJ_HD void gj_rgb_to_ycbcr(float r, float g, float b, float& y, float& cb, float& cr)
{
    gj_rgb_to_ycbcr_m(r + GJ_MAGIC23, g + GJ_MAGIC23, b + GJ_MAGIC23, y, cb, cr);
}

GJ_HD int gj_clamp8(int v) { return v < 0 ? 0 : (v > 255 ? 255 : v); }
GJ_HD void gj_ycbcr_to_rgb_raw(int Y, int Cb, int Cr, int& r, int& g, int& b)
{
    const int y = Y * 256 + ((Y + 1) & 0x100) + 128;
    const int cb = Cb - 128, cr = Cr - 128;
    r = (y + 359 * cr) >> 8;
    g = (y - 88 * cb - 183 * cr) >> 8;
    b = (y + 454 * cb) >> 8;
}
GJ_HD void gj_ycbcr_to_rgb(int Y, int Cb, int Cr, int& r, int& g, int& b)
{
    gj_ycbcr_to_rgb_raw(Y, Cb, Cr, r, g, b);
    r = gj_clamp8(r);
    g = gj_clamp8(g);
    b = gj_clamp8(b);
}


GJ_HD void gj_fdct1(float& a0, float& a1, float& a2, float& a3, float& a4, float& a5, float& a6, float& a7,
                    const float shift)
{
    const float d0 = GJ_FADD(a0, a7), d1 = GJ_FADD(a1, a6), d2 = GJ_FADD(a2, a5), d3 = GJ_FADD(a3, a4);
    const float d4 = GJ_FSUB(a3, a4), d5 = GJ_FSUB(a2, a5), d6 = GJ_FSUB(a1, a6), d7 = GJ_FSUB(a0, a7);
    const float e0 = GJ_FADD(d0, d3), e1 = GJ_FADD(d1, d2), e2 = GJ_FSUB(d1, d2), e3 = GJ_FSUB(d0, d3);
    const float ed = GJ_FADD(e2, e3);
    const float o0 = GJ_FADD(d4, d5), o1 = GJ_FADD(d5, d6), o2 = GJ_FADD(d6, d7);
    const float od5 = GJ_FMUL(GJ_FSUB(o0, o2), 0.382683433f);
    const float od4 = GJ_FMA(1.306562965f, o2, od5);
    const float od3 = GJ_FMA(-0.707106781f, o1, d7);
    const float od2 = GJ_FMA(0.541196100f, o0, od5);
    const float od1 = GJ_FMA(0.707106781f, o1, d7);
    a0 = GJ_FADD(GJ_FADD(e0, e1), shift);
    a4 = GJ_FSUB(e0, e1);
    a2 = GJ_FMA(ed, 0.707106781f, e3);
    a6 = GJ_FMA(ed, -0.707106781f, e3);
    a1 = GJ_FADD(od1, od4);
    a7 = GJ_FSUB(od1, od4);
    a3 = GJ_FSUB(od3, od2);
    a5 = GJ_FADD(od3, od2);
}

GJ_HD void gj_fdct_block(float (&v)[64])
{
#pragma unroll
    for ( int x = 0; x < 8; x++ )
        gj_fdct1(v[x], v[8 + x], v[16 + x], v[24 + x], v[32 + x], v[40 + x], v[48 + x], v[56 + x], -1024.0f);
#pragma unroll
    for ( int y = 0; y < 8; y++ )
        gj_fdct1(v[8 * y], v[8 * y + 1], v[8 * y + 2], v[8 * y + 3], v[8 * y + 4], v[8 * y + 5], v[8 * y + 6],
                 v[8 * y + 7], 0.0f);
}

#define GJ_QUANT_ZERO 0x4B400000u
GJ_HD uint32_t gj_quant_bits(float c, float t)
// ... 410 lines not shown
```

gpujpeg_b200/csrc/gj_encoder.c:

```c
#include <assert.h>
#include <stdlib.h>
#include <string.h>

#include "gj_internal.h"

#define GJ_STRIPES 8
#define GJ_STRIPE_MIN_BYTES ((size_t)8 << 20)

struct gpujpeg_encoder {
    gj_stream_t stream;
    int device;
    struct gpujpeg_parameters param;
    struct gpujpeg_image_parameters param_image;
    int initialised;
    struct gj_geometry geo;
    int input_mode;
    uint8_t* d_planes; size_t d_planes_size;
    struct gj_raw_layout raw;
    int quality;
    enum gpujpeg_header_type header_type;
    enum gpujpeg_header_type header_written;
    int flipped;
    int flip_mode;
    unsigned channel_remap;
// ... 966 lines not shown
    }
    if ( strcmp(opt, GPUJPEG_ENC_OPT_CHANNEL_REMAP) == 0 ) {
        const unsigned m = gj_parse_channel_remap(val, GPUJPEG_ENC_OPT_CHANNEL_REMAP);
        if ( !m ) return GPUJPEG_ERROR;
        encoder->channel_remap = m;
        return GPUJPEG_NOERR;
    }
    if ( strcmp(opt, GPUJPEG_ENC_OPT_EXIF_TAG) == 0 ) {
        encoder->header_type = GPUJPEG_HEADER_EXIF;
        encoder->extras_dirty = 1;
        return gj_exif_add_tag((struct gj_exif_tags**)&encoder->extras.exif_tags, val) == 0 ? GPUJPEG_NOERR : GPUJPEG_ERROR;
    }
    if ( strcmp(opt, GPUJPEG_ENC_OPT_METADATA) == 0 ) {
        encoder->extras_dirty = 1;
        return add_metadata(&encoder->extras.metadata, val);
    }
    if ( strcmp(opt, GPUJPEG_ENC_OPT_HUFFMAN) == 0 ) {
        if ( strcmp(val, GPUJPEG_ENC_HUFFMAN_VAL_STANDARD) == 0 ) encoder->huff_optimized = 0;
        else if ( strcmp(val, GPUJPEG_ENC_HUFFMAN_VAL_OPTIMIZED) == 0 ) encoder->huff_optimized = 1;
        else {
            GJ_ERR("Unknown Huffman table choice: %s\n", val);
            return GPUJPEG_ERROR;
        }
        return GPUJPEG_NOERR;
    }
    GJ_ERR("Invalid encoder option: %s!\n", opt);
    return GPUJPEG_ERROR;
}

void gpujpeg_encoder_print_options(void)
{
    printf("\t" GPUJPEG_ENC_OPT_OUT "=[" GPUJPEG_ENC_OUT_VAL_PAGEABLE "|" GPUJPEG_ENC_OUT_VAL_PINNED
           "] - output buffer in pageable or pinned host memory\n");
    printf("\t" GPUJPEG_ENC_OPT_HDR "=[" GPUJPEG_ENC_HDR_VAL_JFIF "|" GPUJPEG_ENC_HDR_VAL_ADOBE "|" GPUJPEG_ENC_HDR_VAL_EXIF "|" GPUJPEG_ENC_HDR_VAL_SPIFF
           "] - output JPEG header (default: by internal colour space)\n");
    printf("\t" GPUJPEG_ENC_OPT_EXIF_TAG "=<key>=<value>|help - custom EXIF tag (use help for syntax)\n");
    printf("\t" GPUJPEG_ENC_OPT_METADATA "=<key>=<value>|help - set image metadata\n");
    printf("\t" GPUJPEG_ENC_OPT_FLIPPED_BOOL "=[" GPUJPEG_VAL_FALSE "|" GPUJPEG_VAL_TRUE
           "] - whether is the input image should be vertically flipped (prior encode)\n");
    printf("\t" GPUJPEG_ENC_OPT_CHANNEL_REMAP "=XYZ[W] - input channel mapping, eg. '210F' for GBRX,\n"
           "\t\t'210' for GBR; special placeholders 'F' and 'Z' to set a channel to all-ones or all-zeros\n");
    printf("\t" GPUJPEG_ENC_OPT_HUFFMAN "=[" GPUJPEG_ENC_HUFFMAN_VAL_STANDARD "|" GPUJPEG_ENC_HUFFMAN_VAL_OPTIMIZED
           "] - Huffman tables of T.81 Annex K (default) or fitted to every frame\n");
}

GPUJPEG_API int gpujpegx_encoder_run_resident(struct gpujpeg_encoder* e, const uint8_t* d_raw, int stage_mask)
{
    if ( !e || !e->initialised ) return -1;
    if ( !d_raw ) d_raw = e->d_raw;
    if ( !d_raw ) return -1;
    if ( (stage_mask & 1) && launch_k1(e, d_raw) ) return -1;
    if ( (stage_mask & 8) && launch_stats(e) ) return -1;
    if ( (stage_mask & 2) && launch_k2(e) ) return -1;
    return 0;
}

GPUJPEG_API int gpujpegx_encoder_get_symbol_counts(struct gpujpeg_encoder* e, uint64_t out[2][2][256])
{
    if ( !e || !e->initialised || !e->counts_valid || !out ) return -1;
    if ( gj_cuda_memcpy_d2h_async(e->h_counts, e->d_counts, GJ_HUFF_COUNTS_BYTES, e->stream) || gj_cuda_stream_sync(e->stream) )
        return -1;
    memcpy(out, e->h_counts, GJ_HUFF_COUNTS_BYTES);
    return 0;
}

GPUJPEG_API long long gpujpegx_encoder_get_stream(struct gpujpeg_encoder* e, uint8_t* out, size_t capacity)
{
    if ( !e || !e->initialised || e->with_segment_info || !e->d_info_cur ) return -1;
    if ( gj_cuda_memcpy_d2h_async(e->h_info, e->d_info_cur, 32, e->stream) || gj_cuda_stream_sync(e->stream) ) return -1;
    const size_t total = (size_t)e->h_info[0];
    if ( e->h_info[1] || total < e->header_size + 2 || total > e->d_stream_size ) return -1;
    if ( !out ) return (long long)total;
    if ( total > capacity ) return -1;
    if ( gj_cuda_memcpy_d2h_async(out + e->header_size, e->d_stream + e->header_size, total - e->header_size, e->stream) ||
         gj_cuda_stream_sync(e->stream) )
        return -1;
    memcpy(out, e->header, e->header_size);
    return (long long)total;
}

GPUJPEG_API int gpujpegx_encoder_get_coefficients(struct gpujpeg_encoder* e, int16_t* out, size_t count)
{
    if ( !e || !e->initialised || count != e->geo.coef_count ) return -1;
    return gj_coef_to_host_natural(e->d_coef, count, out, e->stream);
}
```

gpujpeg_b200/csrc/gj_huffdec.cu:

```cuda
#include <cuda_runtime.h>
#include <stddef.h>
#include <stdint.h>
#include <stdlib.h>

#include <type_traits>

#include "gj_device.cuh"
#include "gj_internal.h"
#include "gj_launch.cuh"

namespace {

constexpr unsigned FULL = 0xFFFFFFFFu;
constexpr int SD_WARPS = 16;
constexpr int SD_THREADS = SD_WARPS * 32;
constexpr int SD_MAXBLK = 40;
constexpr int SD_MAXLEN = 32760;
constexpr int SD_MINSUB = 8;
constexpr int SD_HEAD = 16;

struct SdTable {
    uint32_t fast[1 << GJ_DEC_FAST_BITS];
    uint32_t sub[GJ_DEC_FAST_SUBS][1 << (16 - GJ_DEC_FAST_BITS)];
    uint32_t maxcode[18];
    int32_t valoff[18];
    uint8_t vals[256];
};
static_assert(sizeof(SdTable) % 16 == 0, "tables are copied with 16-byte accesses");

struct SdParams {
    gj_scan_layout lay;
    const uint32_t* clean;
    const uint32_t* list_cpos;
    const uint8_t* list_code;
    const uint32_t* seg_tab;
    uint32_t first_rank[GJ_MAX_COMP], scan_cbegin[GJ_MAX_COMP];
    int cta_begin[GJ_MAX_COMP + 1];
    int unit_lo[GJ_MAX_COMP], unit_hi[GJ_MAX_COMP];
    int dynamic;
    uint32_t* unit_ctr;
    uint8_t lanes_log2[GJ_MAX_COMP];
    uint8_t staged[GJ_MAX_COMP];
    int8_t scan_td[GJ_MAX_COMP][GJ_MAX_COMP], scan_ta[GJ_MAX_COMP][GJ_MAX_COMP], scan_tq[GJ_MAX_COMP][GJ_MAX_COMP];
    int seg_mcu;
    int ncomp_tab;
    int tgt_entries, stage_bytes;
    int cmp_words;
    int warm_x8;
    uint32_t* error;
    int16_t* coef;
    const gj_dev_dec_tables* tables;
};

__device__ __forceinline__ uint32_t block_target(const gj_scan_layout& L, int scan, int first_mcu, int j)
{
    if ( !L.interleaved ) return (uint32_t)(L.blk_off[scan] + first_mcu + j);
    if ( L.simple ) {
        const int cps = L.comp_count;
        const int mcu = j / cps;
        return (uint32_t)(L.blk_off[j - mcu * cps] + first_mcu + mcu);
    }
    const int mcu = j / L.bpm, i = j - mcu * L.bpm;
    const int m = first_mcu + mcu;
    const int my = m / L.mcu_x, mx = m - my * L.mcu_x;
    const int comp = L.idx_comp[i];
    return (uint32_t)(L.blk_off[comp] + (my * L.comp_vs[comp] + L.idx_dy[i]) * L.bcx[comp] + mx * L.comp_hs[comp] + L.idx_dx[i]);
}

constexpr uint32_t E_TOTAL = GJ_DEC_FAST_TOTAL_MASK;
__device__ __forceinline__ uint32_t make_entry(uint32_t kadv, uint32_t total, uint32_t size)
{
    return kadv | total << GJ_DEC_FAST_TOTAL_SHIFT | size << GJ_DEC_FAST_SIZE_SHIFT;
}

__device__ __forceinline__ uint32_t smem_addr(const void* p) { return (uint32_t)__cvta_generic_to_shared(p); }
__device__ __forceinline__ uint32_t lds32(uint32_t a)
{
    uint32_t v;
    asm volatile("ld.shared.u32 %0, [%1];" : "=r"(v) : "r"(a));
    return v;
}
__device__ __forceinline__ uint32_t lds32_next(uint32_t a)
{
    uint32_t v;
    asm volatile("ld.shared.u32 %0, [%1+4];" : "=r"(v) : "r"(a));
    return v;
}
__device__ __forceinline__ uint32_t lds16(uint32_t a)
{
    uint32_t v;
    asm volatile("ld.shared.u16 %0, [%1];" : "=r"(v) : "r"(a));
    return v;
}
__device__ __forceinline__ uint32_t lds8(uint32_t a)
{
    uint32_t v;
    asm volatile("ld.shared.u8 %0, [%1];" : "=r"(v) : "r"(a));
    return v;
}
__device__ __forceinline__ void sts16(uint32_t a, uint32_t v) { asm volatile("st.shared.u16 [%0], %1;" ::"r"(a), "r"(v)); }

__device__ __noinline__ uint32_t search_code(uint32_t T, uint32_t win, uint32_t ac)
{
    const uint32_t peek = win >> 16;
    const uint32_t mc = T + (uint32_t)offsetof(SdTable, maxcode);
    uint32_t l = GJ_DEC_FAST_BITS + 1;
#pragma unroll
    for ( int q = GJ_DEC_FAST_BITS + 1; q < 16; q++ )
        l += peek >= lds32(mc + 4u * q) ? 1u : 0u;
    if ( peek >= lds32(mc + 4u * l) ) return make_entry(ac ? 64u : 1u, 16u, 0u);
    const int off = (int)lds32(T + (uint32_t)offsetof(SdTable, valoff) + 4u * l);
    const uint32_t sym = lds8(T + (uint32_t)offsetof(SdTable, vals) + (uint32_t)(((int)(peek >> (16u - l)) + off) & 255));
    const uint32_t size = sym & 15u, run = sym >> 4;
    const uint32_t kadv = !ac ? 1u : size ? run + 1u : run == 15u ? 16u : 64u;
    return make_entry(kadv, l + size, size);
}

__device__ __forceinline__ uint32_t long_code(uint32_t T, uint32_t win, uint32_t e, uint32_t ac)
{
    if ( e ) e = lds32(T + (uint32_t)offsetof(SdTable, sub) - 256u + (e & 127u) * 256u + ((win >> 14) & 0xFCu));
    if ( e == 0 ) e = search_code(T, win, ac);
    return e;
}

__device__ __forceinline__ uint32_t lookup(const SdTable* T, uint32_t win, bool ac)
{
    uint32_t e = T->fast[win >> (32 - GJ_DEC_FAST_BITS)];
    if ( (e & E_TOTAL) == 0 ) e = long_code(smem_addr(T), win, e, ac);
    return e;
}

struct Walk {
    const uint32_t* cw;
// ... 77 lines not shown
    };
    if ( q < q_cross ) {
        do step(); while ( q < q_cross );
        nb = 0;
        cross = make_state(q - W.bit0, k, c);
    }
    while ( q < q_end ) step();
    blocks = nb;
    return make_state(q - W.bit0, k, c);
}

struct RegWindow {
    uint32_t hi, lo, nxt;
    __device__ __forceinline__ void init(uint32_t S)
    {
        const uint32_t a = (S >> 10) & 0x3FFFCu;
        hi = lds32(a);
        lo = lds32_next(a);
        nxt = lds32(a + 8u);
    }
    __device__ __forceinline__ uint32_t peek(uint32_t S) const { return __funnelshift_l(lo, hi, S >> 7); }
    __device__ __forceinline__ void advance(uint32_t S_old, uint32_t S_new)
    {
        if ( (S_old ^ S_new) & 0x1000u ) {
            hi = lo;
            lo = nxt;
            nxt = lds32(((S_new >> 10) & 0x3FFFCu) + 8u);
        }
    }
};

template <bool IL>
__device__ __forceinline__ uint32_t walk_state_sm(const Walk& W, uint32_t st, uint32_t p_cross, uint32_t p_end, int& blocks,
                                                  uint32_t& cross)
{
    uint32_t c = st >> 25;
    const uint32_t p = st & 0x3FFFFu;
    blocks = 0;
    cross = st;
    if ( p >= p_end ) return st;
    constexpr uint32_t TS = (uint32_t)sizeof(SdTable);
    uint32_t S = ((st >> 18) & 127u) | (W.sbit0 + p) << 7;
    const uint32_t S_end = (W.sbit0 + p_end) << 7, S_cross = (W.sbit0 + p_cross) << 7;
    uint32_t tdc = W.stab + (IL ? 2u * TS * ((W.cimap >> (2 * c)) & 3u) : 0u);
    uint32_t T = (S & 127u) ? tdc + TS : tdc;
    int nb = 0;
    RegWindow R;
    R.init(S);
    auto step = [&]() {
        const uint32_t win = R.peek(S);
        uint32_t e = lds16(T + ((win >> 20) & 0xFFCu));
        if ( __builtin_expect((e & E_TOTAL) == 0, 0) ) e = long_code(T, win, e, S & 127u) & 0xFFFFu;
        const uint32_t S_old = S;
        S += e;
        R.advance(S_old, S);
        const bool eob = (S & 64u) != 0;
        if ( eob ) {
            S &= ~127u;
            nb++;
            if ( IL ) {
                c = c + 1u == W.bpm ? 0u : c + 1u;
                tdc = W.stab + 2u * TS * ((W.cimap >> (2 * c)) & 3u);
            }
        }
        T = eob ? tdc : tdc + TS;
    };
    if ( S < S_cross ) {
        do step(); while ( S < S_cross );
        nb = 0;
        cross = make_state((S >> 7) - W.sbit0, S & 127u, c);
    }
    while ( S < S_end ) step();
    blocks = nb;
    return make_state((S >> 7) - W.sbit0, S & 127u, c);
}

enum { M_STAGED = 0, M_SPLIT = 1 };
template <int MODE>
struct StageStride { static constexpr int value = MODE == M_STAGED ? 64 : SD_HEAD; };

template <bool DEQ, bool IL, int MODE, bool SM>
__device__ __forceinline__ void walk_write(const Walk& W, uint32_t st, uint32_t p_end, int n, int nblocks,
                                           const uint32_t* __restrict__ tgt, int16_t* __restrict__ stage,
                                           int16_t* __restrict__ glob, int16_t* __restrict__ coef)
{
    uint32_t k = (st >> 18) & 127u, c = st >> 25;
    const uint32_t p = st & 0x3FFFFu;
    if ( n >= nblocks || p >= p_end ) return;
    uint32_t q = W.bit0 + p;
    const uint32_t q_end = W.bit0 + p_end;
    Src<SM> src;
    src.init(W, q);
    uint32_t ci = IL ? (W.cimap >> (2 * c)) & 3u : 0u;
    const SdTable* t_dc = W.tab + 2u * ci;
    const uint16_t* qt = W.q + 64u * ci;
    constexpr int SS = StageStride<MODE>::value;
    auto block_at = [&](int nn) -> int16_t* { return MODE == M_STAGED ? stage + (size_t)nn * 64 : !IL ? glob + (size_t)nn * 64 : coef + (size_t)tgt[nn] * 64; };
    int16_t* o = block_at(n);
    int16_t* so = stage + (size_t)n * SS;
    while ( q < q_end ) {
        const uint32_t win = src.peek(q);
        const SdTable* T = k ? t_dc + 1 : t_dc;
        const uint32_t e = lookup(T, win, k != 0);
        const uint32_t total = (e >> GJ_DEC_FAST_TOTAL_SHIFT) & 31u, kadv = e & 127u, size = e >> GJ_DEC_FAST_SIZE_SHIFT;
        const uint32_t bits = ((win << (total - size)) >> 1) >> (31u - size);
        const uint32_t neg = ((bits >> ((size - 1u) & 31u)) & 1u) ^ 1u;
        int v = (int)bits - (int)(neg ? (1u << size) - 1u : 0u);
        const uint32_t idx = k + kadv - 1u;
        if ( k == 0u ) {
            so[0] = (int16_t)v;
        }
        else if ( size && idx < 64u ) {
            const int16_t dv = (int16_t)(DEQ ? v * (int)qt[idx] : v);
            if ( MODE == M_SPLIT && idx < (uint32_t)SD_HEAD ) so[idx] = dv;
            else o[idx] = dv;
        }
        q += total;
        k += kadv;
        if ( k >= 64u ) {
            k = 0;
            if ( ++n >= nblocks ) break;
            if ( IL ) {
                c = c + 1u == W.bpm ? 0u : c + 1u;
                ci = (W.cimap >> (2 * c)) & 3u;
                t_dc = W.tab + 2u * ci;
                qt = W.q + 64u * ci;
            }
            o = block_at(n);
            so = stage + (size_t)n * SS;
        }
    }
}

template <bool DEQ, bool IL, int MODE>
__device__ __forceinline__ void walk_write_sm(const Walk& W, uint32_t st, uint32_t p_end, int n, int nblocks,
                                              const uint32_t* __restrict__ tgt, int16_t* __restrict__ stage,
                                              int16_t* __restrict__ glob, int16_t* __restrict__ coef)
{
    uint32_t c = st >> 25;
    const uint32_t p = st & 0x3FFFFu;
    if ( n >= nblocks || p >= p_end ) return;
    constexpr uint32_t TS = (uint32_t)sizeof(SdTable);
    uint32_t S = ((st >> 18) & 127u) | (W.sbit0 + p) << 7;
    const uint32_t S_end = (W.sbit0 + p_end) << 7;
    uint32_t ci = IL ? (W.cimap >> (2 * c)) & 3u : 0u;
    uint32_t tdc = W.stab + 2u * TS * ci;
    uint32_t T = (S & 127u) ? tdc + TS : tdc;
    uint32_t qt = W.sq + 128u * ci;
    constexpr uint32_t SS = (uint32_t)StageStride<MODE>::value;
    const uint32_t s_out = smem_addr(stage);
    int16_t* const g_out = IL ? coef : glob;
    auto block_at = [&](int nn) -> uint32_t { return IL ? tgt[nn] * 64u : (uint32_t)nn * 64u; };
    uint32_t sb = s_out + 2u * SS * (uint32_t)n;
    uint32_t gb = MODE == M_SPLIT ? block_at(n) : 0u;
    RegWindow R;
    R.init(S);
    bool pend = false;
    uint32_t pend_at = 0, pend_q = 1;
    uint32_t pend_sb = 0, pend_gb = 0;
    int pend_v = 0;
    auto flush = [&]() {
        if ( pend ) {
            const int dv = DEQ ? pend_v * (int)pend_q : pend_v;
            if ( MODE == M_STAGED || pend_at < SS ) sts16(pend_sb + 2u * pend_at, (uint32_t)dv);
            else g_out[pend_gb + pend_at] = (int16_t)dv;
        }
    };
    while ( S < S_end ) {
        const uint32_t win = R.peek(S);
        uint32_t e = lds32(T + ((win >> 20) & 0xFFCu));
        flush();
        if ( __builtin_expect((e & E_TOTAL) == 0, 0) ) e = long_code(T, win, e, S & 127u);
        const uint32_t size = e >> GJ_DEC_FAST_SIZE_SHIFT;
        const uint32_t mask = (1u << size) - 1u;
        const uint32_t bits = __funnelshift_l(win, 0u, e >> GJ_DEC_FAST_TOTAL_SHIFT) & mask;
        const int v = (int)bits - (int)(2u * bits <= mask ? mask : 0u);
        const bool dc = (S & 127u) == 0u;
        const uint32_t S_old = S;
        S += e & 0xFFFFu;
        R.advance(S_old, S);
        const uint32_t kn = S & 127u;
        pend = !dc && size && kn <= 64u;
        if ( dc ) {
            sts16(sb, (uint32_t)v);
        }
        else if ( pend ) {
            if ( DEQ ) pend_q = lds16(qt + 2u * kn - 2u);
            pend_v = v;
            pend_at = kn - 1u;
            pend_sb = sb;
            pend_gb = gb;
        }
        const bool eob = (S & 64u) != 0;
        if ( eob ) {
            S &= ~127u;
            if ( ++n >= nblocks ) break;
            if ( IL ) {
                c = c + 1u == W.bpm ? 0u : c + 1u;
                ci = (W.cimap >> (2 * c)) & 3u;
                tdc = W.stab + 2u * TS * ci;
                qt = W.sq + 128u * ci;
            }
            sb += 2u * SS;
            if ( MODE == M_SPLIT ) gb = block_at(n);
        }
        T = eob ? tdc : tdc + TS;
    }
    flush();
}

template <bool DEQ, bool IL, int MODE>
__device__ __forceinline__ void run_units(const SdParams& P, const int scan, const bool at_home, Walk W, uint32_t* const s_tgt,
                                          int16_t* const s_stage, uint32_t* const s_cmp)
{
    const gj_scan_layout& L = P.lay;
    const int lane = threadIdx.x & 31, warp = threadIdx.x >> 5, nwarps = blockDim.x >> 5;
    const int ncomp = IL ? L.comp_count : 1;
    const int lanes_log2 = P.lanes_log2[scan], lanes = 1 << lanes_log2;
    const int spu = 32 >> lanes_log2;
    const int slot = lane >> lanes_log2, gl = lane & (lanes - 1);
    const int segblk = P.seg_mcu * L.bpm;
    const int scan_segs = L.scan_seg_begin[scan + 1] - L.scan_seg_begin[scan];
    const int scan_units = P.unit_hi[scan];
    const int unit_lo = P.unit_lo[scan];
    uint32_t* const ctr = P.unit_ctr + scan;
    const int scan_warps = (P.cta_begin[scan + 1] - P.cta_begin[scan]) * nwarps;
    int unit = unit_lo + ((int)blockIdx.x - P.cta_begin[scan]) * nwarps + warp;
    if ( !at_home ) {
        if ( lane == 0 ) unit = unit_lo + scan_warps + (int)atomicAdd(ctr, 1u);
        unit = __shfl_sync(FULL, unit, 0);
    }
    uint32_t* const tgt = s_tgt + slot * segblk;
    constexpr int SS = StageStride<MODE>::value;
    int16_t* const seg_stage = s_stage + (size_t)slot * segblk * SS;

    for ( ;; ) {
        if ( unit >= scan_units ) break;
        int next_unit = scan_units;
        if ( P.dynamic && lane == 0 ) next_unit = unit_lo + scan_warps + (int)atomicAdd(ctr, 1u);
        const int s = unit * spu + slot;
        const bool valid = s < scan_segs;

        const int s_first = unit * spu, s_last = min(s_first + spu, scan_segs) - 1;
        uint32_t cs0 = 0, ce1 = 0;
        if ( !P.seg_tab ) {
            cs0 = s_first ? __ldg(P.list_cpos + P.first_rank[scan] + s_first - 1) : P.scan_cbegin[scan];
            ce1 = __ldg(P.list_cpos + P.first_rank[scan] + s_last);
        }
        const uint32_t wbase = (cs0 >> 2) & ~3u;
        const uint32_t need = ce1 > cs0 ? ((ce1 + 3u) >> 2) - wbase + 8u : 8u;
        const bool fits = !P.seg_tab && need <= (uint32_t)P.cmp_words;
        if ( fits ) {
            const uint4* src = reinterpret_cast<const uint4*>(P.clean + wbase);
            uint4* dst = reinterpret_cast<uint4*>(s_cmp);
            for ( uint32_t i = lane; i < (need + 3u) >> 2; i += 32 )
                dst[i] = __ldg(src + i);
        }

        int nblocks = 0, first_mcu = 0;
        uint32_t len = 0;
        W.cw = P.clean;
        W.sw = s_cmp;
        W.bit0 = 0;
        W.sbit0 = smem_addr(s_cmp) * 8u;
        if ( valid ) {
            first_mcu = s * P.seg_mcu;
            nblocks = min(P.seg_mcu, L.scan_mcus[scan] - first_mcu) * L.bpm;
            uint32_t cs, ce;
            if ( P.seg_tab ) {
                const uint32_t* t = P.seg_tab + 3 * (size_t)(L.scan_seg_begin[scan] + s);
                cs = __ldg(t + 1);
                ce = __ldg(t + 2);
            }
            else {
                const uint32_t r = P.first_rank[scan] + (uint32_t)s;
                ce = __ldg(P.list_cpos + r);
                cs = s ? __ldg(P.list_cpos + r - 1) : P.scan_cbegin[scan];
                if ( s && gl == 0 && __ldg(P.list_code + r - 1) != (uint8_t)(0xD0 + ((s - 1) & 7)) ) atomicExch(P.error, 1u);
            }
            len = ce > cs ? min(ce - cs, (uint32_t)SD_MAXLEN) : 0u;
            W.cw = P.clean + (cs >> 2);
            W.sw = s_cmp + ((cs >> 2) - wbase);
            W.bit0 = (cs & 3u) * 8u;
            W.sbit0 = (smem_addr(s_cmp) + 4u * ((cs >> 2) - wbase)) * 8u + W.bit0;
        }
        int16_t* const seg_glob = IL ? P.coef : P.coef + ((size_t)L.blk_off[scan] + first_mcu) * 64;
        if ( IL ) {
            for ( int j = gl; j < nblocks; j += lanes )
                tgt[j] = block_target(L, scan, first_mcu, j);
        }
        __syncwarp();
        const uint32_t bits_all = len * 8u;

        auto body = [&](auto sm_tag) {
            constexpr bool SM = decltype(sm_tag)::value;
            if ( MODE == M_SPLIT ) {
                const uint4 z = make_uint4(0u, 0u, 0u, 0u);
                constexpr int H16 = SD_HEAD / 8;
                const int n16 = nblocks * 8;
                auto zero_at = [&](int i) {
                    if ( (i & 7) < H16 ) return;
                    if ( !IL ) reinterpret_cast<uint4*>(seg_glob)[i] = z;
                    else reinterpret_cast<uint4*>(P.coef + (size_t)tgt[i >> 3] * 64)[i & 7] = z;
                };
                int i = gl;
                for ( ; i + 3 * lanes < n16; i += 4 * lanes ) {
                    zero_at(i);
                    zero_at(i + lanes);
                    zero_at(i + 2 * lanes);
                    zero_at(i + 3 * lanes);
                }
                for ( ; i < n16; i += lanes )
                    zero_at(i);
                __syncwarp();
            }

            const uint32_t sub = max((uint32_t)SD_MINSUB, (len + lanes - 1) >> lanes_log2) * 8u;
            const uint32_t p_begin = (uint32_t)gl * sub;
            const uint32_t p_end = min(p_begin + sub, bits_all);
            const bool active = valid && (gl == 0 || p_begin < bits_all);

            const uint32_t warm = min(256u, max(32u, (uint32_t)P.warm_x8 * bits_all / (8u * (uint32_t)max(nblocks, 1))));
            const uint32_t p_warm = gl == 0 ? 0u : p_begin - min(p_begin, warm);
            uint32_t start = make_state(p_begin, 0, 0), end = start;
            int dn = 0;
            if ( active ) {
                if constexpr ( SM ) end = walk_state_sm<IL>(W, make_state(p_warm, 0, 0), p_begin, p_end, dn, start);
                else end = walk_state<IL, false>(W, make_state(p_warm, 0, 0), p_begin, p_end, dn, start);
            }
            for ( ;; ) {
                const uint32_t left = __shfl_up_sync(FULL, end, 1, lanes);
                const bool dirty = active && gl != 0 && left != start;
                if ( !__any_sync(FULL, dirty) ) break;
                if ( dirty ) {
                    uint32_t same;
                    if constexpr ( SM ) end = walk_state_sm<IL>(W, left, 0u, p_end, dn, same);
                    else end = walk_state<IL, false>(W, left, 0u, p_end, dn, same);
                    start = left;
                }
            }
            int incl = active ? dn : 0;
            for ( int d = 1; d < lanes; d <<= 1 ) {
                const int t = __shfl_up_sync(FULL, incl, d, lanes);
                if ( gl >= d ) incl += t;
            }
            const int n0 = incl - (active ? dn : 0);

            if ( active ) {
                if constexpr ( SM ) walk_write_sm<DEQ, IL, MODE>(W, start, p_end, n0, nblocks, tgt, seg_stage, seg_glob, P.coef);
                else walk_write<DEQ, IL, MODE, false>(W, start, p_end, n0, nblocks, tgt, seg_stage, seg_glob, P.coef);
            }
        };
        if ( fits ) body(std::true_type{});
        else body(std::false_type{});
        __syncwarp();

        {
            const int bpl = (nblocks + lanes - 1) >> lanes_log2;
            const int j0 = min(nblocks, gl * bpl), j1 = min(nblocks, j0 + bpl);
            auto diff_at = [&](int j) -> int { return (int)seg_stage[j * SS]; };
            int sum[GJ_MAX_COMP] = {0, 0, 0, 0};
            uint32_t c = IL ? (uint32_t)j0 % W.bpm : 0u;
            for ( int j = j0; j < j1; j++ ) {
                const int dv = diff_at(j);
                if ( IL ) {
                    const uint32_t ci = (W.cimap >> (2 * c)) & 3u;
                    sum[0] += ci == 0 ? dv : 0;
                    sum[1] += ci == 1 ? dv : 0;
                    sum[2] += ci == 2 ? dv : 0;
                    sum[3] += ci == 3 ? dv : 0;
                    c = c + 1u == W.bpm ? 0u : c + 1u;
                }
                else {
                    sum[0] += dv;
                }
            }
            int pred[GJ_MAX_COMP] = {0, 0, 0, 0};
#pragma unroll
            for ( int qi = 0; qi < GJ_MAX_COMP; qi++ ) {
                if ( qi < ncomp ) {
                    int x = sum[qi];
                    for ( int d = 1; d < lanes; d <<= 1 ) {
                        const int t = __shfl_up_sync(FULL, x, d, lanes);
                        if ( gl >= d ) x += t;
                    }
                    pred[qi] = x - sum[qi];
                }
            }
            c = IL ? (uint32_t)j0 % W.bpm : 0u;
            for ( int j = j0; j < j1; j++ ) {
                const int dv = diff_at(j);
                uint32_t ci = 0;
                int pr;
                if ( IL ) {
                    ci = (W.cimap >> (2 * c)) & 3u;
                    if ( ci == 0 ) pr = (pred[0] += dv);
                    else if ( ci == 1 ) pr = (pred[1] += dv);
                    else if ( ci == 2 ) pr = (pred[2] += dv);
                    else pr = (pred[3] += dv);
                    c = c + 1u == W.bpm ? 0u : c + 1u;
                }
                else {
                    pr = (pred[0] += dv);
                }
                seg_stage[j * SS] = (int16_t)(DEQ ? pr * (int)W.q[ci * 64] : pr);
            }
        }
        __syncwarp();

        {
            constexpr int S16 = SS / 8;
            uint4* const src = reinterpret_cast<uint4*>(seg_stage);
            uint4* const dst = reinterpret_cast<uint4*>(seg_glob);
            const int n16 = nblocks * S16;
            auto flush_at = [&](int i) {
                const uint4 v = src[i];
                src[i] = make_uint4(0u, 0u, 0u, 0u);
                const int blk = i / S16, part = i % S16;
                if ( !IL ) dst[blk * 8 + part] = v;
                else reinterpret_cast<uint4*>(P.coef + (size_t)tgt[blk] * 64)[part] = v;
            };
            int i = gl;
            for ( ; i + lanes < n16; i += 2 * lanes ) {
                flush_at(i);
                flush_at(i + lanes);
            }
            if ( i < n16 ) flush_at(i);
        }
        __syncwarp();
        unit = __shfl_sync(FULL, next_unit, 0);
    }
}

// ... 36 lines not shown
    W.bpm = (uint32_t)L.bpm;
    W.cimap = 0;
    if ( L.interleaved )
        for ( int i = 0; i < L.bpm; i++ )
            W.cimap |= (uint32_t)(L.simple ? i : L.idx_comp[i]) << (2 * i);

    for ( int round = 0; round < L.scan_count; round++ ) {
    const int scan = home + round < L.scan_count ? home + round : home + round - L.scan_count;
    if ( round > 0 ) {
        if ( !P.dynamic ) break;
        __syncthreads();
        if ( threadIdx.x == 0 ) {
            const int units = P.unit_hi[scan] - P.unit_lo[scan];
            const int handed = (P.cta_begin[scan + 1] - P.cta_begin[scan]) * (int)(blockDim.x >> 5) + (int)*(volatile uint32_t*)(P.unit_ctr + scan);
            s_go = handed < units;
        }
        __syncthreads();
        if ( !s_go ) continue;
    }
    for ( int t = 0; t < 2 * ncomp; t++ ) {
        const int ci = t >> 1, cls = t & 1;
        const int id = cls ? P.scan_ta[scan][ci] : P.scan_td[scan][ci];
        const uint4* f = reinterpret_cast<const uint4*>(&P.tables->fast[cls][id]);
        uint4* d = reinterpret_cast<uint4*>(&s_tab[t]);
        for ( int i = threadIdx.x; i < (int)(sizeof(gj_dec_fast) / 16); i += blockDim.x )
            d[i] = __ldg(f + i);
        const gj_dec_lut& lu = P.tables->lut[cls][id];
        for ( int i = threadIdx.x; i < 18; i += blockDim.x ) {
            s_tab[t].maxcode[i] = lu.maxcode[i];
            s_tab[t].valoff[i] = lu.valoff[i];
        }
        for ( int i = threadIdx.x; i < 256; i += blockDim.x )
            s_tab[t].vals[i] = lu.vals[i];
    }
    for ( int i = threadIdx.x; i < ncomp * 64; i += blockDim.x )
        s_q[i] = P.tables->qinv_zz[P.scan_tq[scan][i >> 6]][i & 63];
    __syncthreads();

    const int mode = P.staged[scan] ? M_STAGED : M_SPLIT;
    if ( L.interleaved ) {
        if ( mode == M_STAGED ) run_units<DEQ, true, M_STAGED>(P, scan, round == 0, W, s_tgt, s_stage, s_cmp);
        else run_units<DEQ, true, M_SPLIT>(P, scan, round == 0, W, s_tgt, s_stage, s_cmp);
    }
    else {
        if ( mode == M_STAGED ) run_units<DEQ, false, M_STAGED>(P, scan, round == 0, W, s_tgt, s_stage, s_cmp);
        else run_units<DEQ, false, M_SPLIT>(P, scan, round == 0, W, s_tgt, s_stage, s_cmp);
    }
    }
    if ( !P.dynamic ) return;
    __syncthreads();
    if ( threadIdx.x == 0 ) {
        __threadfence();
        if ( atomicAdd(P.unit_ctr + 4, 1u) == gridDim.x - 1 ) {
            for ( int i = 0; i < 5; i++ )
                P.unit_ctr[i] = 0;
            __threadfence();
        }
    }
}

}

extern "C" int gj_huffman_decode_sync_eligible(const struct gj_huff_dec_args* a)
{
    if ( !a->d_clean || !a->d_list_cpos || !a->d_unit_ctr || a->seg_mcu * a->lay.bpm > SD_MAXBLK ) return 0;
    for ( int s = 0; s < a->lay.scan_count; s++ ) {
        const int n = a->scan_lanes[s];
        if ( n < 2 || n > 32 || (n & (n - 1)) ) return 0;
    }
    return 1;
}

extern "C" int gj_launch_huffman_decode_sync(const struct gj_huff_dec_args* a, gj_stream_t stream)
{
    SdParams P;
    P.lay = a->lay;
    P.clean = a->d_clean;
    P.list_cpos = a->d_list_cpos;
    P.list_code = a->d_list_code;
    P.seg_tab = a->d_seg_tab;
    P.seg_mcu = a->seg_mcu;
    P.error = a->d_error;
    P.coef = a->d_coef;
    P.tables = a->d_tables;
    const int segblk = a->seg_mcu * a->lay.bpm;
    int total_units = 0, max_spu_tgt = 0;
    size_t stage_bytes = 0;
    size_t cmp_bytes = 0;
    int units[GJ_MAX_COMP] = {0, 0, 0, 0};
    for ( int s = 0; s < GJ_MAX_COMP; s++ ) {
        P.first_rank[s] = a->first_rank[s];
        P.scan_cbegin[s] = a->scan_cbegin[s];
        P.lanes_log2[s] = 5;
        P.staged[s] = 0;
        P.unit_lo[s] = P.unit_hi[s] = 0;
        for ( int k = 0; k < GJ_MAX_COMP; k++ ) {
            P.scan_td[s][k] = (int8_t)a->scan_td[s][k];
            P.scan_ta[s][k] = (int8_t)a->scan_ta[s][k];
            P.scan_tq[s][k] = (int8_t)a->scan_tq[s][k];
        }
        if ( s >= a->lay.scan_count ) continue;
        int l2 = 0;
        while ( (1 << l2) < a->scan_lanes[s] ) l2++;
        P.lanes_log2[s] = (uint8_t)l2;
        const int spu = 32 >> l2;
        P.staged[s] = spu <= 2 && a->scan_dense[s];
        const int segs = a->lay.scan_seg_begin[s + 1] - a->lay.scan_seg_begin[s];
        const int scan_units = (segs + spu - 1) / spu;
        P.unit_lo[s] = a->part_seg_hi[s] ? a->part_seg_lo[s] / spu : 0;
        P.unit_hi[s] = a->part_seg_hi[s] ? (a->part_seg_hi[s] + spu - 1) / spu : scan_units;
        if ( P.unit_hi[s] > scan_units ) P.unit_hi[s] = scan_units;
        if ( P.unit_lo[s] > P.unit_hi[s] ) P.unit_lo[s] = P.unit_hi[s];
        units[s] = P.unit_hi[s] - P.unit_lo[s];
        total_units += units[s];
        const size_t want = 2 * ((size_t)a->scan_bytes[s] / (size_t)(segs > 0 ? segs : 1) + 16) * (size_t)spu + 64;
        if ( want > cmp_bytes ) cmp_bytes = want;
        if ( a->lay.interleaved && spu > max_spu_tgt ) max_spu_tgt = spu;
        {
            const size_t sb = (size_t)spu * segblk * (P.staged[s] ? 128 : SD_HEAD * 2);
            if ( sb > stage_bytes ) stage_bytes = sb;
        }
    }
    int sms = 132;
    int dev = 0;
    if ( cudaGetDevice(&dev) != cudaSuccess ) return -1;
    cudaDeviceGetAttribute(&sms, cudaDevAttrMultiProcessorCount, dev);
    P.unit_ctr = a->d_unit_ctr;
    {
        const char* e = getenv("GPUJPEG_B200_K3_WARM");
        const int w = e ? atoi(e) : 0;
        P.warm_x8 = w >= 1 && w <= 64 ? w : 16;
    }
    P.ncomp_tab = a->lay.interleaved ? a->lay.comp_count : 1;
    P.tgt_entries = max_spu_tgt * segblk;
    P.stage_bytes = (int)stage_bytes;
    if ( cmp_bytes > 40 * 1024 ) cmp_bytes = 40 * 1024;
    P.cmp_words = (int)((cmp_bytes + 15) / 16) * 4;
    const size_t tgt_bytes = ((size_t)P.tgt_entries * 4 + 15) & ~(size_t)15;
    const size_t warp_bytes = tgt_bytes + (size_t)P.stage_bytes + (size_t)P.cmp_words * 4;
    const size_t cta_bytes = (size_t)P.ncomp_tab * (2 * sizeof(SdTable) + 128);
    static int attr_done[64];
    if ( dev < 0 || dev >= 64 ) return -1;
    if ( !__atomic_load_n(&attr_done[dev], __ATOMIC_ACQUIRE) ) {
        if ( cudaFuncSetAttribute(k_huff_decode_sync<true>, cudaFuncAttributeMaxDynamicSharedMemorySize, 200 * 1024) != cudaSuccess ||
             cudaFuncSetAttribute(k_huff_decode_sync<false>, cudaFuncAttributeMaxDynamicSharedMemorySize, 200 * 1024) != cudaSuccess )
            return -1;
        __atomic_store_n(&attr_done[dev], 1, __ATOMIC_RELEASE);
    }
    int cap = total_units / (4 * sms);
    cap = cap < 1 ? 1 : cap > SD_WARPS ? SD_WARPS : cap;
    {
        const char* e = getenv("GPUJPEG_B200_K3_WARPS");
        const int w = e ? atoi(e) : 0;
        if ( w >= 1 && w <= SD_WARPS ) cap = -w;
    }
    struct Pick { int dev, deq, cap, nw, occ; size_t cta_bytes, warp_bytes; };
    static thread_local Pick last = {-1, 0, 0, 0, 0, 0, 0};
    if ( last.dev != dev || last.deq != a->dequantize || last.cap != cap || last.cta_bytes != cta_bytes || last.warp_bytes != warp_bytes ) {
        Pick best = {dev, a->dequantize, cap, 0, 0, cta_bytes, warp_bytes};
        for ( int w = cap < 0 ? -cap : 1; w <= (cap < 0 ? -cap : cap); w++ ) {
            const size_t bytes = cta_bytes + (size_t)w * warp_bytes;
            if ( bytes > 200 * 1024 ) break;
            int o = 0;
            if ( (a->dequantize ? cudaOccupancyMaxActiveBlocksPerMultiprocessor(&o, k_huff_decode_sync<true>, w * 32, bytes)
                                : cudaOccupancyMaxActiveBlocksPerMultiprocessor(&o, k_huff_decode_sync<false>, w * 32, bytes)) != cudaSuccess )
                o = 0;
// ... 41 lines not shown
```

gpujpeg_b200/csrc/gj_huffman.cu:

```cuda
#include <cuda_runtime.h>
#include <stdint.h>

#include "gj_device.cuh"
#include "gj_internal.h"
#include "gj_launch.cuh"

namespace {

constexpr unsigned FULL = 0xFFFFFFFFu;

__device__ __forceinline__ int warp_incl_scan(int v, int lane)
{
#pragma unroll
    for ( int d = 1; d < 32; d <<= 1 ) {
        const int t = __shfl_up_sync(FULL, v, d);
        if ( lane >= d ) v += t;
    }
    return v;
}

__device__ __forceinline__ int scan_of_segment(const gj_scan_layout& L, int g)
{
    return (g >= L.scan_seg_begin[1]) + (g >= L.scan_seg_begin[2]) + (g >= L.scan_seg_begin[3]);
}
// ... 766 lines not shown
__device__ __forceinline__ uint32_t src_load(BitSource& r)
{
    const uint32_t w = r.nextw;
    r.nextw = r.wp < r.wend ? __ldg(r.wp) : 0u;
    r.wp++;
    return w;
}
__device__ __forceinline__ void src_bytes(BitSource& r, uint32_t w, int first)
{
#pragma unroll
    for ( int i = 0; i < 4; i++ ) {
        if ( i < first ) continue;
        const uint32_t b = (w >> (8 * i)) & 0xFFu;
        if ( r.skip_zero ) {
            r.skip_zero = false;
            if ( b == 0 ) continue;
        }
        r.acc = (r.acc << 8) | b;
        r.n += 8;
        r.skip_zero = b == 0xFFu;
    }
}
__device__ __forceinline__ void src_init(BitSource& r, const uint8_t* p, const uint8_t* file_end)
{
    const uintptr_t a = reinterpret_cast<uintptr_t>(p);
    r.wp = reinterpret_cast<const uint32_t*>(a & ~static_cast<uintptr_t>(3));
    r.wend = reinterpret_cast<const uint32_t*>((reinterpret_cast<uintptr_t>(file_end) + 3) & ~static_cast<uintptr_t>(3));
    r.acc = 0;
    r.n = 0;
    r.skip_zero = false;
    r.nextw = r.wp < r.wend ? __ldg(r.wp) : 0u;
    r.wp++;
    src_bytes(r, src_load(r), (int)(a & 3));
}
__device__ __forceinline__ void src_fill(BitSource& r)
{
    while ( r.n <= 32 ) {
        const uint32_t w = src_load(r);
        const uint32_t ff = ((w & 0x7F7F7F7Fu) + 0x01010101u) & w & 0x80808080u;
        if ( ff == 0 && !r.skip_zero ) {
            r.acc = (r.acc << 32) | __byte_perm(w, 0, 0x0123);
            r.n += 32;
        }
        else {
            src_bytes(r, w, 0);
        }
    }
}
__device__ __forceinline__ uint32_t src_peek16(const BitSource& r) { return (uint32_t)(r.acc >> (r.n - 16)) & 0xFFFFu; }
__device__ __forceinline__ uint32_t src_get(BitSource& r, int len)
{
    r.n -= len;
    return (uint32_t)(r.acc >> r.n) & ((1u << len) - 1u);
}

__device__ __forceinline__ int decode_symbol(BitSource& r, const gj_dec_lut& t)
{
    const uint32_t peek = src_peek16(r);
    const uint32_t e = t.look[peek >> (16 - GJ_DEC_LOOK_BITS)];
    if ( e & 15u ) {
        r.n -= (int)(e & 15u);
        return (int)(e >> 4);
    }
    int l = GJ_DEC_LOOK_BITS + 1;
    while ( l <= 16 && peek >= t.maxcode[l] ) l++;
    if ( l > 16 ) {
        r.n -= 16;
        return 0;
    }
    r.n -= l;
    return t.vals[((int)(peek >> (16 - l)) + t.valoff[l]) & 255];
}

struct SegOwners {
    int segs0;
    int warps0;
    int spw0, spw1;
};

template <bool DEQ>
__global__ void __launch_bounds__(HD_THREADS)
k_huff_decode(const uint8_t* __restrict__ file, const uint8_t* __restrict__ file_end, const uint32_t* __restrict__ seg_off,
              int seg_count, int seg_mcu, const __grid_constant__ gj_huff_dec_args a, const __grid_constant__ SegOwners own,
              int16_t* __restrict__ coef, const gj_dev_dec_tables* __restrict__ tables)
{
    gj_pdl_wait();
    __shared__ DecTabs s_tab;
    __shared__ uint16_t s_q[4][64];
    __shared__ __align__(16) uint32_t s_blk[HD_THREADS * 32];

    {
        const uint32_t* src = reinterpret_cast<const uint32_t*>(&tables->lut[0][0]);
        uint32_t* dst = reinterpret_cast<uint32_t*>(&s_tab);
        for ( int i = threadIdx.x; i < (int)(sizeof(DecTabs) / 4); i += HD_THREADS )
            dst[i] = src[i];
        for ( int i = threadIdx.x; i < 256; i += HD_THREADS )
            s_q[i >> 6][i & 63] = tables->qinv_zz[i >> 6][i & 63];
        for ( int i = threadIdx.x; i < HD_THREADS * 32; i += HD_THREADS )
            s_blk[i] = 0;
    }
    __syncthreads();

    const int lane = threadIdx.x & 31, warp = threadIdx.x >> 5;
    const int wg = blockIdx.x * (HD_THREADS / 32) + warp;
    int g0, SPW, g_end;
    if ( wg < own.warps0 ) {
        SPW = own.spw0;
        g0 = wg * SPW;
        g_end = own.segs0;
    }
    else {
        SPW = own.spw1;
        g0 = own.segs0 + (wg - own.warps0) * SPW;
        g_end = seg_count;
    }
    if ( g0 >= g_end ) return;
    if ( !seg_off && !a.d_seg_tab && *a.d_error ) return;
    const int g = g0 + lane;
    const bool live = lane < SPW && g < g_end;
    const gj_scan_layout& L = a.lay;
    const int bpm = L.bpm;
    const bool general = !L.simple && L.interleaved;
    int scan = 0, nblocks = 0, mybase = 0;
    int mx = 0, my = 0;
    BitSource r;
    r.n = 0;
    bool absent = false;
    if ( live ) {
        scan = scan_of_segment(L, g);
        const int s = g - L.scan_seg_begin[scan];
        nblocks = min(seg_mcu, L.scan_mcus[scan] - s * seg_mcu) * bpm;
        mybase = s * seg_mcu + (L.interleaved ? 0 : L.blk_off[a.scan_comp[scan][0]]);
        if ( general ) {
            my = (s * seg_mcu) / L.mcu_x;
            mx = s * seg_mcu - my * L.mcu_x;
        }
        uint32_t start;
        if ( a.d_seg_tab ) {
            start = a.d_seg_tab[3 * (size_t)g];
            absent = start == 0xFFFFFFFFu;
        }
        else if ( seg_off ) {
            start = seg_off[g];
            if ( s > 0 && (start < 2u || start >= (uint32_t)(file_end - file) || file[start - 2] != 0xFF ||
                           file[start - 1] != (uint8_t)(0xD0 + ((s - 1) & 7))) )
                atomicExch(a.d_error, 1u);
        }
        else if ( s == 0 ) {
            start = a.scan_begin[scan];
        }
        else {
            const uint32_t m = a.first_rank[scan] + (uint32_t)s - 1u;
            start = a.d_list_pos[m] + 2u;
            if ( a.d_list_code[m] != (uint8_t)(0xD0 + ((s - 1) & 7)) ) atomicExch(a.d_error, 1u);
        }
        if ( start >= (uint32_t)(file_end - file) ) start = 0;
        src_init(r, file + start, file_end);
    }
    const int max_blocks = seg_mcu * bpm;
    const int sw = lane & 7;
    int16_t* mine = reinterpret_cast<int16_t*>(s_blk + (warp * 32 + (lane < SPW ? lane : 0)) * 32);
    uint4* wbase = reinterpret_cast<uint4*>(s_blk + warp * 32 * 32);
    int pred[GJ_MAX_COMP] = {0, 0, 0, 0};

    int mcu = 0, bi_in_mcu = 0;
    for ( int b = 0; b < max_blocks; b++ ) {
        const int ci = general ? L.idx_comp[bi_in_mcu] : bi_in_mcu;
        if ( live && !absent && b < nblocks ) {
            const gj_dec_lut& tdc = s_tab.t[0][a.scan_td[scan][ci]];
            const gj_dec_lut& tac = s_tab.t[1][a.scan_ta[scan][ci]];
            const uint16_t* q = s_q[a.scan_tq[scan][ci]];
            src_fill(r);
            int sz = decode_symbol(r, tdc) & 15;
            int diff = 0;
            if ( sz ) diff = gj_extend((int)src_get(r, sz), sz);
            int pr;
            if ( ci == 0 ) pr = (pred[0] += diff);
            else if ( ci == 1 ) pr = (pred[1] += diff);
            else if ( ci == 2 ) pr = (pred[2] += diff);
            else pr = (pred[3] += diff);
            mine[(0 ^ sw) << 3] = (int16_t)(DEQ ? pr * (int)q[0] : pr);
            for ( int k = 1; k < 64; ) {
                src_fill(r);
                const int rs = decode_symbol(r, tac);
                const int run = rs >> 4;
                sz = rs & 15;
                if ( sz ) {
                    k += run;
                    const int v = gj_extend((int)src_get(r, sz), sz);
                    if ( k < 64 ) mine[(((k >> 3) ^ sw) << 3) | (k & 7)] = (int16_t)(DEQ ? v * (int)q[k] : v);
                    k++;
                }
                else {
                    if ( run != 15 ) break;
                    k += 16;
                }
            }
        }
        __syncwarp();
        int target;
        if ( general ) {
            const int comp = a.scan_comp[0][ci];
            target = L.blk_off[comp] + (my * L.comp_vs[comp] + L.idx_dy[bi_in_mcu]) * L.bcx[comp] + mx * L.comp_hs[comp] +
                     L.idx_dx[bi_in_mcu];
        }
        else {
            target = mybase + (L.interleaved ? L.blk_off[a.scan_comp[0][ci]] : 0) + mcu;
        }
        for ( int j = 0; j < SPW / 4; j++ ) {
            const int i = 4 * j + (lane >> 3);
            const int c = lane & 7;
            const int ob = __shfl_sync(FULL, target, i);
            const int on = __shfl_sync(FULL, nblocks, i);
            uint4* src = wbase + i * 8 + (c ^ (i & 7));
            const uint4 v = *src;
            *src = make_uint4(0u, 0u, 0u, 0u);
            if ( b < on ) reinterpret_cast<uint4*>(coef + (size_t)ob * 64)[c] = v;
        }
        __syncwarp();
        if ( ++bi_in_mcu == bpm ) {
            bi_in_mcu = 0;
            mcu++;
            if ( general && ++mx == L.mcu_x ) {
                mx = 0;
                my++;
            }
        }
    }
}

__constant__ uint8_t c_zz2nat[64] = {
    0,  1,  8,  16, 9,  2,  3,  10, 17, 24, 32, 25, 18, 11, 4,  5,  12, 19, 26, 33, 40, 48,
    41, 34, 27, 20, 13, 6,  7,  14, 21, 28, 35, 42, 49, 56, 57, 50, 43, 36, 29, 22, 15, 23,
    30, 37, 44, 51, 58, 59, 52, 45, 38, 31, 39, 46, 53, 60, 61, 54, 47, 55, 62, 63};
__global__ void k_coef_to_natural(const int16_t* __restrict__ in, int16_t* __restrict__ out, size_t nblocks)
{
    const size_t i = (size_t)blockIdx.x * blockDim.x + threadIdx.x;
    if ( i >= nblocks * 64 ) return;
    const int k = (int)(i & 63);
    out[(i & ~(size_t)63) + c_zz2nat[k]] = in[i];
}

}

static unsigned long long* place_status_of(const struct gj_huff_enc_args* a) { return reinterpret_cast<unsigned long long*>(a->d_seg_off); }

extern "C" int gj_huffman_encode_parts_eligible(const struct gj_huff_enc_args* a)
{
    return a->lay.simple && a->seg_mcu * a->lay.bpm <= HP_MAXBLK;
}

extern "C" int gj_launch_huffman_encode_part(const struct gj_huff_enc_args* a, int first, const int lo[GJ_MAX_COMP],
                                             const int n[GJ_MAX_COMP], gj_stream_t stream)
{
    const int seg_count = a->lay.scan_seg_begin[GJ_MAX_COMP];
    if ( a->seg_mcu * a->lay.bpm > HP_MAXBLK ) return -1;
    if ( first && !a->info_is_zero && cudaMemsetAsync(a->d_info, 0, 32, stream) != cudaSuccess ) return -1;
    SegPick pick;
    pick.total = 0;
    pick.zero_status = first;
    for ( int k = 0; k < GJ_MAX_COMP; k++ ) {
        const bool real = k < a->lay.scan_count;
        pick.n[k] = real ? n[k] : 0;
        pick.lo[k] = real ? a->lay.scan_seg_begin[k] + lo[k] : 0;
        if ( pick.n[k] < 0 || (real && (lo[k] < 0 || pick.lo[k] + pick.n[k] > a->lay.scan_seg_begin[k + 1])) ) return -1;
        pick.total += pick.n[k];
    }
    if ( pick.total == 0 && !first ) return 0;
    const int n_status = (seg_count + CP_SEGS - 1) / CP_SEGS;
    static int attr_done_p[64];
    int dev = 0;
    if ( cudaGetDevice(&dev) != cudaSuccess || dev < 0 || dev >= 64 ) return -1;
    if ( !__atomic_load_n(&attr_done_p[dev], __ATOMIC_ACQUIRE) ) {
        if ( cudaFuncSetAttribute(k_huff_encode_packed, cudaFuncAttributeMaxDynamicSharedMemorySize, HP_SMEM) != cudaSuccess ) return -1;
        __atomic_store_n(&attr_done_p[dev], 1, __ATOMIC_RELEASE);
    }
    const int hp_threads = max(HE_WARPS * 32, (HE_WARPS * a->seg_mcu * a->lay.bpm + 31) / 32 * 32);
    const int ctas = pick.total ? (pick.total + HE_WARPS - 1) / HE_WARPS : 1;
    gj_launch_pdl(k_huff_encode_packed, dim3(ctas), dim3(hp_threads), HP_SMEM, stream, a->d_coef, a->d_nzmask, a->lay, a->seg_mcu, pick,
                  a->d_tmp, a->slot_stride, a->d_seg_bytes, a->d_spill, a->d_tables, a->d_info, place_status_of(a), n_status);
    return cudaGetLastError() == cudaSuccess ? 0 : -1;
}

extern "C" int gj_launch_huffman_place(const struct gj_huff_enc_args* a, gj_stream_t stream)
{
    const int seg_count = a->lay.scan_seg_begin[GJ_MAX_COMP];
    const int n_status = (seg_count + CP_SEGS - 1) / CP_SEGS;
    ScanSegs segs;
    for ( int k = 0; k <= GJ_MAX_COMP; k++ )
        segs.begin[k] = a->lay.scan_seg_begin[k];
    ScanPrefix pre;
    for ( int k = 0; k < GJ_MAX_COMP; k++ ) {
        pre.len[k] = a->pre_len[k];
        pre.off[k] = a->pre_off[k];
    }
    gj_launch_pdl(k_huff_place, dim3(n_status), dim3(256), 0, stream, (const uint8_t*)a->d_tmp, a->slot_stride, (const uint32_t*)a->d_seg_bytes,
                  seg_count, segs, a->d_sos, pre, a->header_size, (uint64_t)a->stream_cap, a->d_stream,
                  (volatile unsigned long long*)place_status_of(a), a->d_seg_pos, a->d_info, a->d_info_next);
    return cudaGetLastError() == cudaSuccess ? 0 : -1;
}

extern "C" int gj_launch_huffman_encode(const struct gj_huff_enc_args* a, gj_stream_t stream)
{
    const int seg_count = a->lay.scan_seg_begin[GJ_MAX_COMP];
    if ( a->seg_mcu * a->lay.bpm <= HP_MAXBLK ) {
        int lo[GJ_MAX_COMP] = {0, 0, 0, 0}, n[GJ_MAX_COMP] = {0, 0, 0, 0};
        for ( int k = 0; k < a->lay.scan_count && k < GJ_MAX_COMP; k++ )
            n[k] = a->lay.scan_seg_begin[k + 1] - a->lay.scan_seg_begin[k];
        if ( gj_launch_huffman_encode_part(a, 1, lo, n, stream) ) return -1;
    }
    else {
        if ( !a->info_is_zero && cudaMemsetAsync(a->d_info, 0, 32, stream) != cudaSuccess ) return -1;
        const int n_status = (seg_count + CP_SEGS - 1) / CP_SEGS;
        static int attr_done[64];
        int dev = 0;
        if ( cudaGetDevice(&dev) != cudaSuccess || dev < 0 || dev >= 64 ) return -1;
        if ( !__atomic_load_n(&attr_done[dev], __ATOMIC_ACQUIRE) ) {
            if ( cudaFuncSetAttribute(k_huff_encode, cudaFuncAttributeMaxDynamicSharedMemorySize, HE_SMEM) != cudaSuccess ) return -1;
            __atomic_store_n(&attr_done[dev], 1, __ATOMIC_RELEASE);
        }
        gj_launch_pdl(k_huff_encode, dim3((seg_count + HE_WARPS - 1) / HE_WARPS), dim3(HE_WARPS * 32), HE_SMEM, stream,
                      a->d_coef, a->d_nzmask, a->lay, a->seg_mcu, seg_count, a->d_tmp, a->slot_stride, a->d_seg_bytes, a->d_spill,
                      a->d_tables, a->d_info, place_status_of(a), n_status);
        if ( cudaGetLastError() != cudaSuccess ) return -1;
    }
    return gj_launch_huffman_place(a, stream);
}

extern "C" int gj_launch_huffman_stats(const struct gj_huff_enc_args* a, uint64_t* d_counts, gj_stream_t stream)
{
    int total = 0;
    for ( int k = 0; k < a->lay.scan_count; k++ )
        total += a->lay.scan_mcus[k] * a->lay.bpm;
    if ( total <= 0 || a->seg_mcu <= 0 ) return -1;
    if ( cudaMemsetAsync(d_counts, 0, HS_BINS * sizeof(uint64_t), stream) != cudaSuccess ) return -1;
    const int ctas = min((total + HS_THREADS - 1) / HS_THREADS, HS_CTAS_PER_SM * gj_cuda_sm_count());
    gj_launch_pdl(k_huff_stats, dim3(ctas), dim3(HS_THREADS), 0, stream, a->d_coef, a->d_nzmask, a->lay, a->seg_mcu, total,
                  reinterpret_cast<unsigned long long*>(d_counts));
    return cudaGetLastError() == cudaSuccess ? 0 : -1;
}

extern "C" int gj_huffman_decode_sync_eligible(const struct gj_huff_dec_args* a);
extern "C" int gj_launch_huffman_decode_sync(const struct gj_huff_dec_args* a, gj_stream_t stream);

extern "C" int gj_huffman_decode_parts_eligible(const struct gj_huff_dec_args* a)
{
    return !a->force_thread_per_segment && gj_huffman_decode_sync_eligible(a) && !a->d_seg_tab && a->lay.simple && !a->lay.interleaved;
}

extern "C" int gj_launch_huffman_decode(const struct gj_huff_dec_args* a, gj_stream_t stream)
{
    if ( !a->force_thread_per_segment && gj_huffman_decode_sync_eligible(a) ) return gj_launch_huffman_decode_sync(a, stream);
    SegOwners own;
    const int spw_all = a->seg_count <= 8000 ? 4 : a->seg_count <= 24000 ? 8 : HD_SEGMENTS_PER_WARP;
    own.segs0 = a->seg_count;
    own.spw0 = own.spw1 = spw_all;
    if ( a->lay.scan_count > 1 ) {
        own.segs0 = a->lay.scan_seg_begin[1];
        own.spw0 = a->seg_count > 24000 ? 8 : 4;
        own.spw1 = 32;
    }
    own.warps0 = (own.segs0 + own.spw0 - 1) / own.spw0;
    const int warps = own.warps0 + (a->seg_count - own.segs0 + own.spw1 - 1) / own.spw1;
    const dim3 grid((warps + HD_THREADS / 32 - 1) / (HD_THREADS / 32));
    if ( a->dequantize )
        gj_launch_pdl(k_huff_decode<true>, dim3(grid), dim3(HD_THREADS), 0, stream, a->d_file, a->d_file + a->file_size, a->d_seg_off,
                      a->seg_count, a->seg_mcu, *a, own, a->d_coef, a->d_tables);
    else
        gj_launch_pdl(k_huff_decode<false>, dim3(grid), dim3(HD_THREADS), 0, stream, a->d_file, a->d_file + a->file_size, a->d_seg_off,
                      a->seg_count, a->seg_mcu, *a, own, a->d_coef, a->d_tables);
    return cudaGetLastError() == cudaSuccess ? 0 : -1;
}

extern "C" int gj_coef_to_host_natural(const int16_t* d_coef, size_t count, int16_t* h_out, gj_stream_t stream)
{
    int16_t* d_tmp = nullptr;
    if ( cudaMalloc(&d_tmp, count * sizeof(int16_t)) != cudaSuccess ) return -1;
    const size_t nblocks = count / 64;
    k_coef_to_natural<<<(unsigned)((count + 255) / 256), 256, 0, stream>>>(d_coef, d_tmp, nblocks);
    cudaMemcpyAsync(h_out, d_tmp, count * sizeof(int16_t), cudaMemcpyDeviceToHost, stream);
    const cudaError_t e = cudaStreamSynchronize(stream);
    cudaFree(d_tmp);
    return e == cudaSuccess ? 0 : -1;
}
```

gpujpeg_b200/csrc/gj_internal.h:

```cpp
#ifndef GJ_INTERNAL_H
#define GJ_INTERNAL_H

#include <stddef.h>
#include <stdint.h>
#include <stdio.h>

#include "../../include/gpujpeg_b200.h"

#ifdef __cplusplus
extern "C" {
#endif

#define GJ_MAX_COMP 4
#define GJ_SOS_LEN_1 10

#define GJ_ERR(...) (void)(fprintf(stderr, "[GPUJPEG] [Error] " __VA_ARGS__))
#define GJ_WARN(...) (void)(fprintf(stderr, "[GPUJPEG] [Warning] " __VA_ARGS__))
#define GJ_VERBOSE(v, ...) do { if ( (v) >= GPUJPEG_LL_VERBOSE ) (void)fprintf(stderr, "[GPUJPEG] [Verbose] " __VA_ARGS__); } while ( 0 )
#define GJ_DEBUG(v, ...) do { if ( (v) >= GPUJPEG_LL_DEBUG ) (void)fprintf(stderr, "[GPUJPEG] [Debug] " __VA_ARGS__); } while ( 0 )

extern const uint8_t gj_zigzag_to_natural[64];
extern const uint8_t gj_natural_to_zigzag[64];

struct gj_huff_spec {
// ... 125 lines not shown
    int comp[GJ_MAX_COMP];
    int td[GJ_MAX_COMP], ta[GJ_MAX_COMP];
    int ss, se, ah, al;
    size_t huff_at[GJ_MAX_COMP];
    size_t begin, end;
    int first_segment, segment_count;
};
void gj_huff_spec_at(const uint8_t* data, size_t at, struct gj_huff_spec* spec);
#define GJ_SEGINFO_MAX_PIECES 64
struct gj_seginfo {
    const uint8_t* piece[GJ_SEGINFO_MAX_PIECES];
    uint32_t piece_bytes[GJ_SEGINFO_MAX_PIECES];
    int pieces;
    size_t bytes;
};
struct gj_stream {
    int width, height, comp_count;
    int restart_interval;
    int comp_id[GJ_MAX_COMP], comp_hv[GJ_MAX_COMP], comp_tq[GJ_MAX_COMP];
    uint8_t qt[4][64];
    int have_qt[4];
    struct gj_huff_spec huff[2][4];
    int have_huff[2][4];
    size_t huff_at[2][4];
    int progressive;
    uint8_t coef_bits[GJ_MAX_COMP][64];
    uint8_t comp_qt[GJ_MAX_COMP][64];
    int have_comp_qt[GJ_MAX_COMP];
    int scan_count;
    struct gj_scan_info scan[GJ_MAX_SCANS];
    struct gj_seginfo seginfo[GJ_MAX_COMP];
    struct gj_seginfo seginfo_pending;
    enum gpujpeg_color_space color_space;
    int spiff_color_space;
    int in_spiff_directory;
    int exif_seen;
    int verbose;
    struct gpujpeg_image_metadata metadata;
    int com_color_space;
    int ff_cs_itu601_is_709;
    enum gpujpeg_header_type header_type;
    const char* comment;
    size_t header_size;
    int interleaved;
};
void gj_reader_begin(struct gj_stream* s, int ff_cs_itu601_is_709);
int gj_reader_walk(const uint8_t* data, size_t size, size_t* pos, struct gj_stream* s, int* adobe_transform);
int gj_reader_finish(struct gj_stream* s, int adobe_transform, int verbose);
enum gpujpeg_color_space gj_stream_color_space(const struct gj_stream* s, int adobe_transform);
int gj_reader_parse(const uint8_t* data, size_t size, struct gj_stream* s, int verbose);
int gj_reader_split(const uint8_t* data, struct gj_stream* s, uint32_t* seg_off, uint32_t* seg_len, int max_segments);

enum { GJ_IMGFILE_PNM = 1, GJ_IMGFILE_PAM, GJ_IMGFILE_Y4M };
struct gj_imgfile {
    int kind;
    int width, height;
    int channels, maxval;
    int subsampling, bitdepth, limited;
    size_t data_offset, data_bytes;
};
int gj_imgfile_probe(const char* filename, struct gj_imgfile* f);
int gj_imgfile_params(const char* filename, const struct gj_imgfile* f, struct gpujpeg_image_parameters* pi);
int gj_imgfile_load(const char* filename, uint8_t** image, size_t* image_size, void* (*alloc)(size_t));
int gj_imgfile_save_pam(const char* filename, const struct gpujpeg_image_parameters* pi, const uint8_t* data, int pnm);
int gj_imgfile_save_y4m(const char* filename, const struct gpujpeg_image_parameters* pi, const uint8_t* data);

typedef struct CUstream_st* gj_stream_t;

struct gj_dev_enc_tables {
    float fwd_zz[2][64];
    struct gj_enc_lut lut[2];
};
struct gj_dev_dec_tables {
    uint16_t qinv_zz[4][64];
    struct gj_dec_lut lut[2][4];
    struct gj_dec_fast fast[2][4];
};

int gj_launch_fdct_rgb444(const uint8_t* d_raw, int width, int height, int pitch, int16_t* d_coef, uint64_t* d_nzmask,
                          int bcx, int bcy, const struct gj_dev_enc_tables* d_tables, gj_stream_t stream);

int gj_launch_fdct_rgb444_rows(const uint8_t* d_raw, int width, int height, int pitch, int16_t* d_coef, uint64_t* d_nzmask,
                               int bcx, int bcy, int by0, int by1, const struct gj_dev_enc_tables* d_tables, gj_stream_t stream);
int gj_launch_idct_rgb444_rows(const int16_t* d_coef, int bcx, int bcy, int by0, int by1, const int comp_tq[3], uint8_t* d_raw,
                               int width, int height, int pitch, int idct_flavour, int coef_dequantized,
                               const struct gj_dev_dec_tables* d_tables, gj_stream_t stream);

int gj_launch_fdct_rgb_ss_rows(const uint8_t* d_raw, int width, int height, int pitch, int16_t* d_coef, uint64_t* d_nzmask,
                               const struct gj_comp_geo comp[3], int my0, int my1, const struct gj_dev_enc_tables* h_tables,
                               gj_stream_t stream);
int gj_launch_idct_rgb_ss_rows(const int16_t* d_coef, const struct gj_comp_geo comp[3], int my0, int my1, const int comp_tq[3],
                               uint8_t* d_raw, int width, int height, int pitch, int idct_flavour, int coef_dequantized,
                               const struct gj_dev_dec_tables* h_tables, gj_stream_t stream);

struct gj_huff_enc_args {
    const int16_t* d_coef;
    const uint64_t* d_nzmask;
    struct gj_scan_layout lay;
    int seg_mcu;
    uint8_t* d_tmp;
    size_t slot_stride;
    uint32_t* d_spill;
    uint32_t* d_seg_bytes;
    uint64_t* d_seg_off;
    uint8_t* d_stream;
    size_t stream_cap;
    uint32_t header_size;
    const uint8_t* d_sos;
    int pre_len[GJ_MAX_COMP], pre_off[GJ_MAX_COMP];
    uint64_t* d_seg_pos;
    uint64_t* d_info;
    uint64_t* d_info_next;
    int info_is_zero;
    const struct gj_dev_enc_tables* d_tables;
};
int gj_launch_huffman_encode(const struct gj_huff_enc_args* a, gj_stream_t stream);
int gj_huffman_encode_parts_eligible(const struct gj_huff_enc_args* a);
int gj_launch_huffman_encode_part(const struct gj_huff_enc_args* a, int first, const int lo[GJ_MAX_COMP], const int n[GJ_MAX_COMP],
                                  gj_stream_t stream);
int gj_launch_huffman_place(const struct gj_huff_enc_args* a, gj_stream_t stream);
#define GJ_HUFF_COUNTS_BYTES (2 * 2 * 256 * sizeof(uint64_t))
int gj_launch_huffman_stats(const struct gj_huff_enc_args* a, uint64_t* d_counts, gj_stream_t stream);

struct gj_huff_dec_args {
    const uint8_t* d_file;
    size_t file_size;
    const uint32_t* d_seg_off;
    const uint32_t* d_seg_tab;
    uint32_t* d_unit_ctr;
    const uint32_t* d_seg_len;
    const uint32_t* d_list_pos;
    const uint8_t* d_list_code;
    uint32_t first_rank[GJ_MAX_COMP];
    uint32_t scan_begin[GJ_MAX_COMP];
    uint32_t* d_error;
    const uint32_t* d_clean;
    const uint32_t* d_list_cpos;
    uint32_t scan_cbegin[GJ_MAX_COMP];
    uint8_t scan_lanes[GJ_MAX_COMP];
    uint32_t scan_bytes[GJ_MAX_COMP];
    uint8_t scan_dense[GJ_MAX_COMP];
    int force_thread_per_segment;
    int part_seg_lo[GJ_MAX_COMP], part_seg_hi[GJ_MAX_COMP];
    int dequantize;
    struct gj_scan_layout lay;
    int seg_count, seg_mcu;
    int scan_comp[GJ_MAX_COMP][GJ_MAX_COMP];
    int scan_td[GJ_MAX_COMP][GJ_MAX_COMP], scan_ta[GJ_MAX_COMP][GJ_MAX_COMP];
    int scan_tq[GJ_MAX_COMP][GJ_MAX_COMP];
    int16_t* d_coef;
    const struct gj_dev_dec_tables* d_tables;
};
int gj_launch_huffman_decode(const struct gj_huff_dec_args* a, gj_stream_t stream);
int gj_huffman_decode_parts_eligible(const struct gj_huff_dec_args* a);

enum { GJ_PROG_DC_FIRST = 0, GJ_PROG_DC_REFINE = 1, GJ_PROG_AC_FIRST = 2, GJ_PROG_AC_REFINE = 3 };
struct gj_prog_scan {
    int kind;
    int ss, se, ah, al;
    int ncomp;
    int bpm;
    int units, units_x;
    int seg_units;
    int seg_count;
    int lut0;
    uint32_t first_rank, cbegin;
    int blk_off[GJ_MAX_COMP], bcx[GJ_MAX_COMP], nblk[GJ_MAX_COMP], hs[GJ_MAX_COMP], vs[GJ_MAX_COMP];
    uint8_t idx_ci[GJ_MAX_MCU_BLOCKS], idx_dx[GJ_MAX_MCU_BLOCKS], idx_dy[GJ_MAX_MCU_BLOCKS];
};
int gj_prog_scan_init(const struct gj_geometry* g, const struct gj_stream* s, int k, int restart_interval, struct gj_prog_scan* out);

struct gj_prog_args {
    const struct gj_prog_scan* scans;
    int scan_count;
    const struct gj_dec_lut* d_luts;
    const uint32_t* d_clean;
    const uint32_t* d_list_cpos;
    const uint8_t* d_list_code;
    uint32_t* d_error;
    int16_t* d_coef;
    size_t coef_count;
    int dequantize;
    int comp_count;
    int comp_blk_off[GJ_MAX_COMP];
    const struct gj_dev_dec_tables* d_tables;
};
int gj_launch_progressive_decode(const struct gj_prog_args* a, gj_stream_t stream);

int gj_launch_marker_scan(const uint8_t* d_file, size_t begin, size_t end, unsigned long long* d_cta, uint32_t* d_list_pos,
                          uint8_t* d_list_code, uint32_t* d_list_cpos, uint32_t list_cap, uint8_t* d_clean, uint32_t* d_result,
                          uint32_t* d_other, uint32_t other_cap, gj_stream_t stream);

int gj_launch_idct_rgb444(const int16_t* d_coef, int bcx, int bcy, const int comp_tq[3], uint8_t* d_raw, int width,
                          int height, int pitch, int idct_flavour, int coef_dequantized,
                          const struct gj_dev_dec_tables* d_tables, gj_stream_t stream);

int gj_launch_fdct_rgb_ss(const uint8_t* d_raw, int width, int height, int pitch, int16_t* d_coef, uint64_t* d_nzmask,
                          const struct gj_comp_geo comp[3], const struct gj_dev_enc_tables* h_tables, gj_stream_t stream);
int gj_launch_idct_rgb_ss(const int16_t* d_coef, const struct gj_comp_geo comp[3], const int comp_tq[3], uint8_t* d_raw,
                          int width, int height, int pitch, int idct_flavour, int coef_dequantized,
                          const struct gj_dev_dec_tables* h_tables, gj_stream_t stream);

int gj_launch_fdct_samples(const uint8_t* d_raw, const struct gj_raw_layout* raw, int16_t* d_coef, uint64_t* d_nzmask,
                           const struct gj_comp_geo* comp, int comp_count, const uint8_t* comp_tbl,
                           const struct gj_dev_enc_tables* h_tables, gj_stream_t stream);
int gj_launch_idct_samples(const int16_t* d_coef, const struct gj_comp_geo* comp, int comp_count, const int* comp_tq,
                           uint8_t* d_raw, const struct gj_raw_layout* raw, int idct_flavour, int coef_dequantized,
                           const struct gj_dev_dec_tables* h_tables, gj_stream_t stream);

int gj_launch_convert_in(const uint8_t* d_raw, const struct gj_raw_layout* raw, enum gpujpeg_pixel_format fmt, int color_space,
                         int color_space_internal, int width, int height, uint8_t* d_planes, size_t planes_size,
                         const struct gj_comp_geo* comp, int comp_count, int max_hs, int max_vs, gj_stream_t stream);
int gj_launch_convert_out(const uint8_t* d_planes, uint8_t* d_raw, const struct gj_raw_layout* raw, enum gpujpeg_pixel_format fmt,
                          int color_space, int color_space_internal, int width, int height, const struct gj_comp_geo* comp,
                          int comp_count, int max_hs, int max_vs, gj_stream_t stream);
int gj_launch_flip_planes(uint8_t* d_planes, const struct gj_comp_geo* padded, int comp_count, gj_stream_t stream);
int gj_launch_channel_remap(uint8_t* d_raw, const struct gj_raw_layout* raw, enum gpujpeg_pixel_format fmt, int width, int height,
                            unsigned remap, gj_stream_t stream);
unsigned gj_parse_channel_remap(const char* val, const char* optname);
int gj_parse_bool(const char* val, const char* optname);
void gj_planes_layout(struct gj_raw_layout* l, struct gj_comp_geo padded[GJ_MAX_COMP], const struct gj_comp_geo* comp,
                      int comp_count);

int gj_coef_to_host_natural(const int16_t* d_coef, size_t count, int16_t* h_out, gj_stream_t stream);

int gj_cuda_malloc(void** p, size_t size);
int gj_cuda_free(void* p);
int gj_cuda_malloc_host(void** p, size_t size);
int gj_cuda_free_host(void* p);
int gj_cuda_memcpy_h2d_async(void* dst, const void* src, size_t size, gj_stream_t s);
int gj_cuda_memcpy_d2h_async(void* dst, const void* src, size_t size, gj_stream_t s);
int gj_cuda_memcpy_d2d_async(void* dst, const void* src, size_t size, gj_stream_t s);
int gj_cuda_memset_async(void* dst, int v, size_t size, gj_stream_t s);
int gj_cuda_stream_sync(gj_stream_t s);
int gj_cuda_stream_create(gj_stream_t* s);
int gj_cuda_event_create(void** ev);
void gj_cuda_event_destroy(void* ev);
int gj_cuda_event_record(void* ev, gj_stream_t s);
int gj_cuda_stream_wait_event(gj_stream_t s, void* ev);
void gj_cuda_stream_destroy(gj_stream_t s);
int gj_cuda_enable_peer(int peer);
int gj_cuda_memcpy_peer_async(void* dst, int dst_dev, const void* src, int src_dev, size_t size, gj_stream_t s);
int gj_cuda_pointer_is_device(const void* p);
const char* gj_cuda_last_error(void);
struct gj_timer { void* start; void* stop; int armed; };
int gj_timer_create(struct gj_timer* t);
void gj_timer_destroy(struct gj_timer* t);
void gj_timer_start(struct gj_timer* t, gj_stream_t s);
void gj_timer_stop(struct gj_timer* t, gj_stream_t s);
double gj_timer_ms(struct gj_timer* t);
int gj_cuda_device_count(void);
int gj_cuda_sm_count(void);
int gj_cuda_device_props(int dev, struct gpujpeg_device_info* info);
int gj_cuda_set_device(int dev);
int gj_cuda_get_device(void);
void gj_cuda_device_reset(void);

#ifdef __cplusplus
}
#endif
#endif
```

gpujpeg_b200/csrc/gj_progressive.cu:

```cuda
#include <cuda_runtime.h>
#include <stddef.h>
#include <stdint.h>

#include "gj_device.cuh"
#include "gj_internal.h"
#include "gj_launch.cuh"

namespace {

constexpr int PD_THREADS = 64;
constexpr int DQ_THREADS = 256;

template <int KIND>
__global__ void __launch_bounds__(PD_THREADS)
k_prog_decode(const __grid_constant__ gj_prog_scan S, const gj_dec_lut* __restrict__ luts, const uint32_t* __restrict__ clean,
              const uint32_t* __restrict__ list_cpos, const uint8_t* __restrict__ list_code, uint32_t* error, int16_t* coef)
{
    gj_pdl_wait();
    __shared__ gj_dec_lut s_tab[GJ_MAX_COMP];
    if ( KIND != GJ_PROG_DC_REFINE ) {
        const int nt = KIND == GJ_PROG_DC_FIRST ? S.ncomp : 1;
        const uint32_t* src = reinterpret_cast<const uint32_t*>(luts + S.lut0);
        uint32_t* dst = reinterpret_cast<uint32_t*>(s_tab);
        for ( int i = threadIdx.x; i < nt * (int)(sizeof(gj_dec_lut) / 4); i += blockDim.x )
            dst[i] = __ldg(src + i);
        __syncthreads();
    }
    const int s = blockIdx.x * blockDim.x + threadIdx.x;
    if ( s >= S.seg_count ) return;
    const uint32_t r = S.first_rank + (uint32_t)s;
    const uint32_t ce = list_cpos[r], cs = s ? list_cpos[r - 1] : S.cbegin;
    if ( s && list_code[r - 1] != (uint8_t)(0xD0 + ((s - 1) & 7)) ) atomicExch(error, 1u);
    gj_prog_segment<KIND>(S, s_tab, clean, cs, ce > cs ? ce : cs, s, coef);
}

__global__ void __launch_bounds__(DQ_THREADS) k_prog_zero(uint4* __restrict__ p, size_t n16)
{
    for ( size_t i = (size_t)blockIdx.x * blockDim.x + threadIdx.x; i < n16; i += (size_t)gridDim.x * blockDim.x )
        p[i] = make_uint4(0u, 0u, 0u, 0u);
}

struct DqComps {
    int count;
    int blk_off[GJ_MAX_COMP];
};

__global__ void __launch_bounds__(DQ_THREADS)
k_prog_dequant(int16_t* __restrict__ coef, size_t count, const __grid_constant__ DqComps C, const gj_dev_dec_tables* __restrict__ tables)
{
    gj_pdl_wait();
    for ( size_t i = (size_t)blockIdx.x * blockDim.x + threadIdx.x; i < count; i += (size_t)gridDim.x * blockDim.x ) {
        const long blk = (long)(i >> 6);
        int c = 0;
        for ( int k = 1; k < C.count; k++ )
            c += blk >= C.blk_off[k];
        coef[i] = (int16_t)((int)coef[i] * (int)__ldg(&tables->qinv_zz[c][i & 63]));
    }
}

}

extern "C" int gj_launch_progressive_decode(const struct gj_prog_args* a, gj_stream_t stream)
{
    const size_t cap = (size_t)gj_cuda_sm_count() * 8;
    {
        const size_t n16 = a->coef_count / 8;
        const size_t blocks = (n16 + DQ_THREADS - 1) / DQ_THREADS;
        k_prog_zero<<<(unsigned)(blocks < cap ? blocks : cap), DQ_THREADS, 0, stream>>>(reinterpret_cast<uint4*>(a->d_coef), n16);
        if ( cudaGetLastError() != cudaSuccess ) return -1;
    }
    for ( int k = 0; k < a->scan_count; k++ ) {
        const gj_prog_scan& S = a->scans[k];
        const dim3 grid((S.seg_count + PD_THREADS - 1) / PD_THREADS), block(PD_THREADS);
        cudaError_t e;
        switch ( S.kind ) {
            case GJ_PROG_DC_FIRST:
                e = gj_launch_pdl(k_prog_decode<GJ_PROG_DC_FIRST>, grid, block, 0, stream, S, a->d_luts, a->d_clean, a->d_list_cpos,
                                  a->d_list_code, a->d_error, a->d_coef);
                break;
            case GJ_PROG_DC_REFINE:
                e = gj_launch_pdl(k_prog_decode<GJ_PROG_DC_REFINE>, grid, block, 0, stream, S, a->d_luts, a->d_clean, a->d_list_cpos,
                                  a->d_list_code, a->d_error, a->d_coef);
                break;
            case GJ_PROG_AC_FIRST:
                e = gj_launch_pdl(k_prog_decode<GJ_PROG_AC_FIRST>, grid, block, 0, stream, S, a->d_luts, a->d_clean, a->d_list_cpos,
                                  a->d_list_code, a->d_error, a->d_coef);
                break;
            default:
                e = gj_launch_pdl(k_prog_decode<GJ_PROG_AC_REFINE>, grid, block, 0, stream, S, a->d_luts, a->d_clean, a->d_list_cpos,
                                  a->d_list_code, a->d_error, a->d_coef);
                break;
        }
        if ( e != cudaSuccess ) return -1;
    }
    if ( a->dequantize ) {
        DqComps C;
        C.count = a->comp_count;
        for ( int c = 0; c < GJ_MAX_COMP; c++ )
            C.blk_off[c] = a->comp_blk_off[c];
        size_t blocks = (a->coef_count + DQ_THREADS - 1) / DQ_THREADS;
        if ( blocks > cap ) blocks = cap;
        if ( gj_launch_pdl(k_prog_dequant, dim3((unsigned)blocks), dim3(DQ_THREADS), 0, stream, a->d_coef, a->coef_count, C,
                           a->d_tables) != cudaSuccess )
            return -1;
    }
    return cudaGetLastError() == cudaSuccess ? 0 : -1;
}
```

Baseline: 53560.

## Track per-block coefficient extent to skip loading and transforming zero tails in IDCT

Adds a per-block extent byte (cext) written by the Huffman decoder and set to full by the progressive path. The IDCT kernels use it to load only the non-zero uint4 chunks of each coefficient block. When a whole warp has small extents, they run a specialised integer IDCT that treats coefficients beyond the first 16 as zero. This cuts global memory reads and dequant/IDCT arithmetic for sparse blocks, at the cost of an extra byte array, a warp vote, and a second template instantiation that adds code size and branch divergence.

```diff
diff --git a/gpujpeg_b200/csrc/gj_dct.cu b/gpujpeg_b200/csrc/gj_dct.cu
--- a/gpujpeg_b200/csrc/gj_dct.cu
+++ b/gpujpeg_b200/csrc/gj_dct.cu
@@ -418,9 +418,24 @@
 }
 
 
+template <bool DEQ, int NZ>
+__device__ __forceinline__ void idct_int_px(const uint32_t (&packed)[32], const uint16_t* __restrict__ q, uint32_t (&px)[16])
+{
+    int v[64];
+#pragma unroll
+    for ( int k = 0; k < 64; k++ ) {
+        const int c = k >= NZ ? 0 : (k & 1) ? (int)packed[k >> 1] >> 16 : (int)(short)(packed[k >> 1] & 0xFFFFu);
+        v[gj_zz2nat(k)] = DEQ ? gj_s16(c * (int)(short)q[k]) : c;
+    }
+    gj_idct_int_block_px(v);
+#pragma unroll
+    for ( int i = 0; i < 16; i++ )
+        px[i] = pack4_sat_u8(v[4 * i], v[4 * i + 1], v[4 * i + 2], v[4 * i + 3]);
+}
+
 template <int VEC, int FLAVOUR, bool DEQ>
 __global__ void __launch_bounds__(NT)
-k_idct_rgb444(const int16_t* __restrict__ coef, int bcx, int nblk, uint8_t* __restrict__ raw, int width, int height,
+k_idct_rgb444(const int16_t* __restrict__ coef, const uint8_t* __restrict__ cext, int bcx, int nblk, uint8_t* __restrict__ raw, int width, int height,
               size_t pitch, const __grid_constant__ IdctParams prm)
 {
     gj_pdl_wait();
@@ -435,27 +450,18 @@
     {
         const int comp = threadIdx.x >> 6;
         const int b = threadIdx.x & 63;
-        if ( bx0 + b < bcx ) {
-            const uint4* src = reinterpret_cast<const uint4*>(coef + ((size_t)comp * nblk + (size_t)by * bcx + bx0 + b) * 64);
+        const bool in = bx0 + b < bcx;
+        const size_t bi = (size_t)comp * nblk + (size_t)by * bcx + bx0 + b;
+        const int ext = in ? __ldg(cext + bi) : 0;
+        const bool head = __all_sync(0xFFFFFFFFu, ext <= 2);
+        if ( in ) {
             uint32_t packed[32];
-#pragma unroll
-            for ( int i = 0; i < 8; i++ ) {
-                const uint4 t = __ldg(src + i);
-                packed[4 * i] = t.x; packed[4 * i + 1] = t.y; packed[4 * i + 2] = t.z; packed[4 * i + 3] = t.w;
-            }
+            gj_load_coef_block(coef + bi * 64, ext, packed);
             const uint16_t* q = prm.q_zz[comp];
             uint32_t px[16];
             if ( FLAVOUR == 0 ) {
-                int v[64];
-#pragma unroll
-                for ( int k = 0; k < 64; k++ ) {
-                    const int c = (k & 1) ? (int)packed[k >> 1] >> 16 : (int)(short)(packed[k >> 1] & 0xFFFFu);
-                    v[gj_zz2nat(k)] = DEQ ? gj_s16(c * (int)(short)q[k]) : c;
-                }
-                gj_idct_int_block_px(v);
-#pragma unroll
-                for ( int i = 0; i < 16; i++ )
-                    px[i] = pack4_sat_u8(v[4 * i], v[4 * i + 1], v[4 * i + 2], v[4 * i + 3]);
+                if ( head ) idct_int_px<DEQ, 16>(packed, q, px);
+                else idct_int_px<DEQ, 64>(packed, q, px);
             }
             else {
                 float f[64];
@@ -512,7 +518,7 @@
 
 template <int HS, int VS, int VEC, int FLAVOUR, bool DEQ>
 __global__ void __launch_bounds__(TB * VS + 2 * TB / HS)
-k_idct_rgb_ss(const int16_t* __restrict__ coef, const __grid_constant__ SsGrid grid, uint8_t* __restrict__ raw, int width,
+k_idct_rgb_ss(const int16_t* __restrict__ coef, const uint8_t* __restrict__ cext, const __grid_constant__ SsGrid grid, uint8_t* __restrict__ raw, int width,
               int height, size_t pitch, const __grid_constant__ IdctParams prm)
 {
     gj_pdl_wait();
@@ -548,28 +554,18 @@
             dst = s_c[comp - 1] + (u % CB) * 8;
             dpitch = CW;
         }
-        if ( bx < grid.bcx[comp] && by < grid.bcy[comp] ) {
-            const uint4* src =
-                reinterpret_cast<const uint4*>(coef + ((size_t)grid.blk_off[comp] + (size_t)by * grid.bcx[comp] + bx) * 64);
+        const bool in = bx < grid.bcx[comp] && by < grid.bcy[comp];
+        const size_t bi = (size_t)grid.blk_off[comp] + (size_t)by * grid.bcx[comp] + bx;
+        const int ext = in ? __ldg(cext + bi) : 0;
+        const bool head = __all_sync(0xFFFFFFFFu, ext <= 2);
+        if ( in ) {
             uint32_t packed[32];
-#pragma unroll
-            for ( int i = 0; i < 8; i++ ) {
-                const uint4 t = __ldg(src + i);
-                packed[4 * i] = t.x; packed[4 * i + 1] = t.y; packed[4 * i + 2] = t.z; packed[4 * i + 3] = t.w;
-            }
+            gj_load_coef_block(coef + bi * 64, ext, packed);
             const uint16_t* q = prm.q_zz[comp];
             uint32_t px[16];
             if ( FLAVOUR == 0 ) {
-                int v[64];
-#pragma unroll
-                for ( int k = 0; k < 64; k++ ) {
-                    const int c = (k & 1) ? (int)packed[k >> 1] >> 16 : (int)(short)(packed[k >> 1] & 0xFFFFu);
-                    v[gj_zz2nat(k)] = DEQ ? gj_s16(c * (int)(short)q[k]) : c;
-                }
-                gj_idct_int_block_px(v);
-#pragma unroll
-                for ( int i = 0; i < 16; i++ )
-                    px[i] = pack4_sat_u8(v[4 * i], v[4 * i + 1], v[4 * i + 2], v[4 * i + 3]);
+                if ( head ) idct_int_px<DEQ, 16>(packed, q, px);
+                else idct_int_px<DEQ, 64>(packed, q, px);
             }
             else {
                 float f[64];
@@ -671,7 +667,7 @@
 
 template <int FLAVOUR, bool DEQ>
 __global__ void __launch_bounds__(SG_THREADS)
-k_idct_samples(const int16_t* __restrict__ coef, const __grid_constant__ SampleGrid g, int total_blocks,
+k_idct_samples(const int16_t* __restrict__ coef, const uint8_t* __restrict__ cext, const __grid_constant__ SampleGrid g, int total_blocks,
                uint8_t* __restrict__ raw, const __grid_constant__ IdctParams prm)
 {
     const int bi = blockIdx.x * SG_THREADS + threadIdx.x;
@@ -681,13 +677,8 @@
     const int by = local / g.bcx[comp], bx = local - by * g.bcx[comp];
     const int vw = min(8, g.cw[comp] - bx * 8), vh = min(8, g.ch[comp] - by * 8);
     if ( vw <= 0 || vh <= 0 ) return;
-    const uint4* src = reinterpret_cast<const uint4*>(coef + (size_t)bi * 64);
     uint32_t packed[32];
-#pragma unroll
-    for ( int i = 0; i < 8; i++ ) {
-        const uint4 t = __ldg(src + i);
-        packed[4 * i] = t.x; packed[4 * i + 1] = t.y; packed[4 * i + 2] = t.z; packed[4 * i + 3] = t.w;
-    }
+    gj_load_coef_block(coef + (size_t)bi * 64, __ldg(cext + bi), packed);
     const uint16_t* q = prm.q_zz[comp];
     uint32_t px[16];
     if ( FLAVOUR == 0 ) {
@@ -795,8 +786,8 @@
                               d_nzmask + (size_t)by0 * bcx, bcx, by1 - by0, bcx * bcy, h_tables, stream);
 }
 
-static int launch_idct_rgb444(const int16_t* d_coef, int bcx, int bcy, int nblk, const int comp_tq[3], uint8_t* d_raw, int width,
-                              int height, int pitch, int idct_flavour, int coef_dequantized,
+static int launch_idct_rgb444(const int16_t* d_coef, const uint8_t* d_cext, int bcx, int bcy, int nblk, const int comp_tq[3],
+                              uint8_t* d_raw, int width, int height, int pitch, int idct_flavour, int coef_dequantized,
                               const struct gj_dev_dec_tables* h_tables, gj_stream_t stream)
 {
     IdctParams prm;
@@ -805,7 +796,7 @@
     const dim3 grid((bcx + TB - 1) / TB, bcy);
     const int vec = pick_vec(d_raw, (size_t)pitch);
     if ( idct_flavour != 0 && coef_dequantized ) return -1;
-#define GJ_K4(V, F, D) gj_launch_pdl(k_idct_rgb444<V, F, D>, grid, dim3(NT), 0, stream, d_coef, bcx, nblk, d_raw, width, height, (size_t)pitch, prm)
+#define GJ_K4(V, F, D) gj_launch_pdl(k_idct_rgb444<V, F, D>, grid, dim3(NT), 0, stream, d_coef, d_cext, bcx, nblk, d_raw, width, height, (size_t)pitch, prm)
     if ( idct_flavour == 0 && coef_dequantized ) {
         if ( vec == 4 ) GJ_K4(4, 0, false); else GJ_K4(1, 0, false);
     }
@@ -818,20 +809,20 @@
 #undef GJ_K4
     return cudaGetLastError() == cudaSuccess ? 0 : -1;
 }
-extern "C" int gj_launch_idct_rgb444(const int16_t* d_coef, int bcx, int bcy, const int comp_tq[3], uint8_t* d_raw,
-                                     int width, int height, int pitch, int idct_flavour, int coef_dequantized,
+extern "C" int gj_launch_idct_rgb444(const int16_t* d_coef, const uint8_t* d_cext, int bcx, int bcy, const int comp_tq[3],
+                                     uint8_t* d_raw, int width, int height, int pitch, int idct_flavour, int coef_dequantized,
                                      const struct gj_dev_dec_tables* h_tables, gj_stream_t stream)
 {
-    return launch_idct_rgb444(d_coef, bcx, bcy, bcx * bcy, comp_tq, d_raw, width, height, pitch, idct_flavour, coef_dequantized,
+    return launch_idct_rgb444(d_coef, d_cext, bcx, bcy, bcx * bcy, comp_tq, d_raw, width, height, pitch, idct_flavour, coef_dequantized,
                               h_tables, stream);
 }
-extern "C" int gj_launch_idct_rgb444_rows(const int16_t* d_coef, int bcx, int bcy, int by0, int by1, const int comp_tq[3],
-                                          uint8_t* d_raw, int width, int height, int pitch, int idct_flavour,
+extern "C" int gj_launch_idct_rgb444_rows(const int16_t* d_coef, const uint8_t* d_cext, int bcx, int bcy, int by0, int by1,
+                                          const int comp_tq[3], uint8_t* d_raw, int width, int height, int pitch, int idct_flavour,
                                           int coef_dequantized, const struct gj_dev_dec_tables* h_tables, gj_stream_t stream)
 {
     if ( by0 < 0 || by1 > bcy || by0 >= by1 ) return -1;
     const int rows = (by1 * 8 < height ? by1 * 8 : height) - by0 * 8;
-    return launch_idct_rgb444(d_coef + (size_t)by0 * bcx * 64, bcx, by1 - by0, bcx * bcy, comp_tq, d_raw + (ptrdiff_t)by0 * 8 * pitch,
+    return launch_idct_rgb444(d_coef + (size_t)by0 * bcx * 64, d_cext + (size_t)by0 * bcx, bcx, by1 - by0, bcx * bcy, comp_tq, d_raw + (ptrdiff_t)by0 * 8 * pitch,
                               width, rows, pitch, idct_flavour, coef_dequantized, h_tables, stream);
 }
 
@@ -898,7 +889,7 @@
                                       stream);
 }
 
-extern "C" int gj_launch_idct_rgb_ss_rows(const int16_t* d_coef, const struct gj_comp_geo comp[3], int my0, int my1,
+extern "C" int gj_launch_idct_rgb_ss_rows(const int16_t* d_coef, const uint8_t* d_cext, const struct gj_comp_geo comp[3], int my0, int my1,
                                           const int comp_tq[3], uint8_t* d_raw, int width, int height, int pitch, int idct_flavour,
                                           int coef_dequantized, const struct gj_dev_dec_tables* h_tables, gj_stream_t stream)
 {
@@ -916,7 +907,7 @@
     const dim3 grid((comp[0].bcx + TB - 1) / TB, my1 - my0);
     const int vec = pick_vec(d_raw, (size_t)pitch);
 #define GJ_K4SS2(H, V, VE, F, D) \
-    gj_launch_pdl(k_idct_rgb_ss<H, V, VE, F, D>, grid, dim3(TB * V + 2 * TB / H), 0, stream, d_coef, sg, d_raw, width, height, (size_t)pitch, prm)
+    gj_launch_pdl(k_idct_rgb_ss<H, V, VE, F, D>, grid, dim3(TB * V + 2 * TB / H), 0, stream, d_coef, d_cext, sg, d_raw, width, height, (size_t)pitch, prm)
 #define GJ_K4SS(H, V)                                                                  \
     do {                                                                               \
         if ( idct_flavour == 0 && coef_dequantized ) {                                 \
@@ -937,12 +928,12 @@
 #undef GJ_K4SS2
     return cudaGetLastError() == cudaSuccess ? 0 : -1;
 }
-extern "C" int gj_launch_idct_rgb_ss(const int16_t* d_coef, const struct gj_comp_geo comp[3], const int comp_tq[3],
+extern "C" int gj_launch_idct_rgb_ss(const int16_t* d_coef, const uint8_t* d_cext, const struct gj_comp_geo comp[3], const int comp_tq[3],
                                      uint8_t* d_raw, int width, int height, int pitch, int idct_flavour,
                                      int coef_dequantized, const struct gj_dev_dec_tables* h_tables, gj_stream_t stream)
 {
     const int vs = comp[0].vs > 0 ? comp[0].vs : 1;
-    return gj_launch_idct_rgb_ss_rows(d_coef, comp, 0, (comp[0].bcy + vs - 1) / vs, comp_tq, d_raw, width, height, pitch,
+    return gj_launch_idct_rgb_ss_rows(d_coef, d_cext, comp, 0, (comp[0].bcy + vs - 1) / vs, comp_tq, d_raw, width, height, pitch,
                                       idct_flavour, coef_dequantized, h_tables, stream);
 }
 
@@ -984,8 +975,8 @@
     return cudaGetLastError() == cudaSuccess ? 0 : -1;
 }
 
-extern "C" int gj_launch_idct_samples(const int16_t* d_coef, const struct gj_comp_geo* comp, int comp_count, const int* comp_tq,
-                                      uint8_t* d_raw, const struct gj_raw_layout* raw, int idct_flavour, int coef_dequantized,
+extern "C" int gj_launch_idct_samples(const int16_t* d_coef, const uint8_t* d_cext, const struct gj_comp_geo* comp, int comp_count,
+                                      const int* comp_tq, uint8_t* d_raw, const struct gj_raw_layout* raw, int idct_flavour, int coef_dequantized,
                                       const struct gj_dev_dec_tables* h_tables, gj_stream_t stream)
 {
     IdctParams prm;
@@ -997,10 +988,10 @@
     if ( idct_flavour != 0 && coef_dequantized ) return -1;
     const int grid = (total + SG_THREADS - 1) / SG_THREADS;
     if ( idct_flavour == 0 && coef_dequantized )
-        k_idct_samples<0, false><<<grid, SG_THREADS, 0, stream>>>(d_coef, sg, total, d_raw, prm);
+        k_idct_samples<0, false><<<grid, SG_THREADS, 0, stream>>>(d_coef, d_cext, sg, total, d_raw, prm);
     else if ( idct_flavour == 0 )
-        k_idct_samples<0, true><<<grid, SG_THREADS, 0, stream>>>(d_coef, sg, total, d_raw, prm);
+        k_idct_samples<0, true><<<grid, SG_THREADS, 0, stream>>>(d_coef, d_cext, sg, total, d_raw, prm);
     else
-        k_idct_samples<1, true><<<grid, SG_THREADS, 0, stream>>>(d_coef, sg, total, d_raw, prm);
+        k_idct_samples<1, true><<<grid, SG_THREADS, 0, stream>>>(d_coef, d_cext, sg, total, d_raw, prm);
     return cudaGetLastError() == cudaSuccess ? 0 : -1;
 }
diff --git a/gpujpeg_b200/csrc/gj_decoder.c b/gpujpeg_b200/csrc/gj_decoder.c
--- a/gpujpeg_b200/csrc/gj_decoder.c
+++ b/gpujpeg_b200/csrc/gj_decoder.c
@@ -55,6 +55,7 @@
     uint32_t* d_k3_ctr;
     uint32_t* h_mk;
     int16_t* d_coef; size_t d_coef_size;
+    uint8_t* d_cext; size_t d_cext_size;
     uint8_t* d_raw; size_t d_raw_size;
     uint8_t* h_raw; size_t h_raw_size;
 
@@ -160,6 +161,7 @@
     gj_cuda_free(d->d_k3_ctr);
     gj_cuda_free_host(d->h_mk);
     gj_cuda_free(d->d_coef);
+    gj_cuda_free(d->d_cext);
     gj_cuda_free(d->d_planes);
     gj_cuda_free(d->d_raw);
     gj_cuda_free_host(d->h_raw);
@@ -239,6 +241,7 @@
     gj_geometry_init(&d->geo, &p, &pi);
     const struct gj_geometry* g = &d->geo;
     if ( grow_dev((void**)&d->d_coef, &d->d_coef_size, g->coef_count * 2) ||
+         grow_dev((void**)&d->d_cext, &d->d_cext_size, g->coef_count / 64) ||
          grow_dev((void**)&d->d_raw, &d->d_raw_size, g->raw_size) ) {
         GJ_ERR("Decoder device allocation failed: %s\n", gj_cuda_last_error());
         return -1;
@@ -317,13 +320,13 @@
 {
     const struct gj_geometry* g = &d->geo;
     if ( d->out_mode == GJ_OUT_SAMPLES )
-        return gj_launch_idct_samples(d->d_coef, g->comp, g->comp_count, comp_tq, d_out, &d->raw, d->idct_flavour,
+        return gj_launch_idct_samples(d->d_coef, d->d_cext, g->comp, g->comp_count, comp_tq, d_out, &d->raw, d->idct_flavour,
                                       coef_dequantized, &d->h_tab, d->stream);
     if ( d->out_mode == GJ_OUT_GENERIC ) {
         struct gj_raw_layout pl;
         struct gj_comp_geo padded[GJ_MAX_COMP];
         gj_planes_layout(&pl, padded, g->comp, g->comp_count);
-        if ( gj_launch_idct_samples(d->d_coef, padded, g->comp_count, comp_tq, d->d_planes, &pl, d->idct_flavour,
+        if ( gj_launch_idct_samples(d->d_coef, d->d_cext, padded, g->comp_count, comp_tq, d->d_planes, &pl, d->idct_flavour,
                                     coef_dequantized, &d->h_tab, d->stream) )
             return -1;
         if ( d->flipped && gj_launch_flip_planes(d->d_planes, padded, g->comp_count, d->stream) ) return -1;
@@ -337,9 +340,9 @@
         pitch = -pitch;
     }
     if ( g->lay.simple )
-        return gj_launch_idct_rgb444(d->d_coef, g->bcx, g->bcy, comp_tq, d_out, g->width, g->height, pitch, d->idct_flavour,
+        return gj_launch_idct_rgb444(d->d_coef, d->d_cext, g->bcx, g->bcy, comp_tq, d_out, g->width, g->height, pitch, d->idct_flavour,
                                      coef_dequantized, &d->h_tab, d->stream);
-    return gj_launch_idct_rgb_ss(d->d_coef, g->comp, comp_tq, d_out, g->width, g->height, pitch, d->idct_flavour,
+    return gj_launch_idct_rgb_ss(d->d_coef, d->d_cext, g->comp, comp_tq, d_out, g->width, g->height, pitch, d->idct_flavour,
                                  coef_dequantized, &d->h_tab, d->stream);
 }
 
@@ -401,9 +404,9 @@
                 if ( gj_launch_huffman_decode(&part, d->stream) ) return -1;
             }
         }
-        const int rc = g->lay.simple ? gj_launch_idct_rgb444_rows(d->d_coef, g->bcx, g->bcy, my0, my1, comp_tq, d_out, g->width, g->height,
+        const int rc = g->lay.simple ? gj_launch_idct_rgb444_rows(d->d_coef, d->d_cext, g->bcx, g->bcy, my0, my1, comp_tq, d_out, g->width, g->height,
                                                                   g->pitch, d->idct_flavour, coef_dequantized, &d->h_tab, d->stream)
-                                     : gj_launch_idct_rgb_ss_rows(d->d_coef, g->comp, my0, my1, comp_tq, d_out, g->width, g->height, g->pitch,
+                                     : gj_launch_idct_rgb_ss_rows(d->d_coef, d->d_cext, g->comp, my0, my1, comp_tq, d_out, g->width, g->height, g->pitch,
                                                                   d->idct_flavour, coef_dequantized, &d->h_tab, d->stream);
         if ( rc ||
              gj_cuda_event_record(d->ev_stripe[i], d->stream) || gj_cuda_stream_wait_event(d->copy_stream, d->ev_stripe[i]) ||
@@ -837,6 +840,7 @@
     a->d_list_code = d->d_list_code;
     a->d_error = d->d_mk + 3;
     a->d_coef = d->d_coef;
+    a->d_cext = d->d_cext;
     a->coef_count = g->coef_count;
     a->dequantize = d->idct_flavour == 0;
     a->comp_count = g->comp_count;
@@ -1101,6 +1105,7 @@
     ha.lay = g->lay;
     ha.seg_mcu = g->seg_mcu;
     ha.d_coef = d->d_coef;
+    ha.d_cext = d->d_cext;
     ha.d_tables = d->d_tab;
     d->last_args = ha;
     d->last_ecs_begin = ecs_begin;
@@ -1316,6 +1321,6 @@
 GPUJPEG_API int gpujpegx_decoder_get_coefficients(struct gpujpeg_decoder* d, int16_t* out, size_t count)
 {
     if ( !d || !d->initialised || !d->last_valid || count != d->geo.coef_count ) return -1;
-    if ( gj_coef_to_host_natural(d->d_coef, count, out, d->stream) ) return -1;
+    if ( gj_coef_to_host_natural(d->d_coef, d->d_cext, count, out, d->stream) ) return -1;
     return (d->last_progressive ? d->last_prog.dequantize : d->last_args.dequantize) ? 1 : 0;
 }
diff --git a/gpujpeg_b200/csrc/gj_device.cuh b/gpujpeg_b200/csrc/gj_device.cuh
--- a/gpujpeg_b200/csrc/gj_device.cuh
+++ b/gpujpeg_b200/csrc/gj_device.cuh
@@ -44,6 +44,22 @@
                            46, 51, 55, 60, 21, 34, 37, 47, 50, 56, 59, 61, 35, 36, 48, 49, 57, 58, 62, 63};
     return t[n];
 }
+
+
+GJ_HD int gj_cext_of(int last_zz) { return (last_zz >> 3) + 1; }
+GJ_HD bool gj_cext_holds(int ext, int k) { return (k >> 3) < ext; }
+
+#if defined(__CUDACC__)
+__device__ __forceinline__ void gj_load_coef_block(const int16_t* __restrict__ blk, int ext, uint32_t (&packed)[32])
+{
+    const uint4* src = reinterpret_cast<const uint4*>(blk);
+#pragma unroll
+    for ( int i = 0; i < 8; i++ ) {
+        const uint4 t = i < ext ? __ldg(src + i) : make_uint4(0u, 0u, 0u, 0u);
+        packed[4 * i] = t.x; packed[4 * i + 1] = t.y; packed[4 * i + 2] = t.z; packed[4 * i + 3] = t.w;
+    }
+}
+#endif
 
 
 #define GJ_MAGIC23 8388608.0f
diff --git a/gpujpeg_b200/csrc/gj_encoder.c b/gpujpeg_b200/csrc/gj_encoder.c
--- a/gpujpeg_b200/csrc/gj_encoder.c
+++ b/gpujpeg_b200/csrc/gj_encoder.c
@@ -1072,5 +1072,5 @@
 GPUJPEG_API int gpujpegx_encoder_get_coefficients(struct gpujpeg_encoder* e, int16_t* out, size_t count)
 {
     if ( !e || !e->initialised || count != e->geo.coef_count ) return -1;
-    return gj_coef_to_host_natural(e->d_coef, count, out, e->stream);
-}
+    return gj_coef_to_host_natural(e->d_coef, NULL, count, out, e->stream);
+}
diff --git a/gpujpeg_b200/csrc/gj_huffdec.cu b/gpujpeg_b200/csrc/gj_huffdec.cu
--- a/gpujpeg_b200/csrc/gj_huffdec.cu
+++ b/gpujpeg_b200/csrc/gj_huffdec.cu
@@ -49,6 +49,7 @@
     int warm_x8;
     uint32_t* error;
     int16_t* coef;
+    uint8_t* cext;
     const gj_dev_dec_tables* tables;
 };
 
@@ -292,7 +293,7 @@
 template <bool DEQ, bool IL, int MODE, bool SM>
 __device__ __forceinline__ void walk_write(const Walk& W, uint32_t st, uint32_t p_end, int n, int nblocks,
                                            const uint32_t* __restrict__ tgt, int16_t* __restrict__ stage,
-                                           int16_t* __restrict__ glob, int16_t* __restrict__ coef)
+                                           int16_t* __restrict__ glob, int16_t* __restrict__ coef, uint8_t* __restrict__ ext)
 {
     uint32_t k = (st >> 18) & 127u, c = st >> 25;
     const uint32_t p = st & 0x3FFFFu;
@@ -323,7 +324,10 @@
         else if ( size && idx < 64u ) {
             const int16_t dv = (int16_t)(DEQ ? v * (int)qt[idx] : v);
             if ( MODE == M_SPLIT && idx < (uint32_t)SD_HEAD ) so[idx] = dv;
-            else o[idx] = dv;
+            else {
+                o[idx] = dv;
+                if ( MODE == M_SPLIT ) ext[!IL ? n : (int)tgt[n]] = GJ_CEXT_FULL;
+            }
         }
         q += total;
         k += kadv;
@@ -345,7 +349,7 @@
 template <bool DEQ, bool IL, int MODE>
 __device__ __forceinline__ void walk_write_sm(const Walk& W, uint32_t st, uint32_t p_end, int n, int nblocks,
                                               const uint32_t* __restrict__ tgt, int16_t* __restrict__ stage,
-                                              int16_t* __restrict__ glob, int16_t* __restrict__ coef)
+                                              int16_t* __restrict__ glob, int16_t* __restrict__ coef, uint8_t* __restrict__ ext)
 {
     uint32_t c = st >> 25;
     const uint32_t p = st & 0x3FFFFu;
@@ -373,7 +377,10 @@
         if ( pend ) {
             const int dv = DEQ ? pend_v * (int)pend_q : pend_v;
             if ( MODE == M_STAGED || pend_at < SS ) sts16(pend_sb + 2u * pend_at, (uint32_t)dv);
-            else g_out[pend_gb + pend_at] = (int16_t)dv;
+            else {
+                g_out[pend_gb + pend_at] = (int16_t)dv;
+                ext[pend_gb >> 6] = GJ_CEXT_FULL;
+            }
         }
     };
     while ( S < S_end ) {
@@ -495,6 +502,7 @@
             W.sbit0 = (smem_addr(s_cmp) + 4u * ((cs >> 2) - wbase)) * 8u + W.bit0;
         }
         int16_t* const seg_glob = IL ? P.coef : P.coef + ((size_t)L.blk_off[scan] + first_mcu) * 64;
+        uint8_t* const seg_ext = IL ? P.cext : P.cext + (size_t)L.blk_off[scan] + first_mcu;
         if ( IL ) {
             for ( int j = gl; j < nblocks; j += lanes )
                 tgt[j] = block_target(L, scan, first_mcu, j);
@@ -504,6 +512,8 @@
 
         auto body = [&](auto sm_tag) {
             constexpr bool SM = decltype(sm_tag)::value;
+            for ( int j = gl; j < nblocks; j += lanes )
+                seg_ext[IL ? (int)tgt[j] : j] = MODE == M_STAGED ? GJ_CEXT_FULL : SD_HEAD / 8;
             if ( MODE == M_SPLIT ) {
                 const uint4 z = make_uint4(0u, 0u, 0u, 0u);
                 constexpr int H16 = SD_HEAD / 8;
@@ -557,8 +567,8 @@
             const int n0 = incl - (active ? dn : 0);
 
             if ( active ) {
-                if constexpr ( SM ) walk_write_sm<DEQ, IL, MODE>(W, start, p_end, n0, nblocks, tgt, seg_stage, seg_glob, P.coef);
-                else walk_write<DEQ, IL, MODE, false>(W, start, p_end, n0, nblocks, tgt, seg_stage, seg_glob, P.coef);
+                if constexpr ( SM ) walk_write_sm<DEQ, IL, MODE>(W, start, p_end, n0, nblocks, tgt, seg_stage, seg_glob, P.coef, seg_ext);
+                else walk_write<DEQ, IL, MODE, false>(W, start, p_end, n0, nblocks, tgt, seg_stage, seg_glob, P.coef, seg_ext);
             }
         };
         if ( fits ) body(std::true_type{});
@@ -761,6 +771,7 @@
     P.seg_mcu = a->seg_mcu;
     P.error = a->d_error;
     P.coef = a->d_coef;
+    P.cext = a->d_cext;
     P.tables = a->d_tables;
     const int segblk = a->seg_mcu * a->lay.bpm;
     int total_units = 0, max_spu_tgt = 0;
diff --git a/gpujpeg_b200/csrc/gj_huffman.cu b/gpujpeg_b200/csrc/gj_huffman.cu
--- a/gpujpeg_b200/csrc/gj_huffman.cu
+++ b/gpujpeg_b200/csrc/gj_huffman.cu
@@ -872,7 +872,7 @@
 __global__ void __launch_bounds__(HD_THREADS)
 k_huff_decode(const uint8_t* __restrict__ file, const uint8_t* __restrict__ file_end, const uint32_t* __restrict__ seg_off,
               int seg_count, int seg_mcu, const __grid_constant__ gj_huff_dec_args a, const __grid_constant__ SegOwners own,
-              int16_t* __restrict__ coef, const gj_dev_dec_tables* __restrict__ tables)
+              int16_t* __restrict__ coef, uint8_t* __restrict__ cext, const gj_dev_dec_tables* __restrict__ tables)
 {
     gj_pdl_wait();
     __shared__ DecTabs s_tab;
@@ -956,6 +956,7 @@
     int mcu = 0, bi_in_mcu = 0;
     for ( int b = 0; b < max_blocks; b++ ) {
         const int ci = general ? L.idx_comp[bi_in_mcu] : bi_in_mcu;
+        int ext = 0;
         if ( live && !absent && b < nblocks ) {
             const gj_dec_lut& tdc = s_tab.t[0][a.scan_td[scan][ci]];
             const gj_dec_lut& tac = s_tab.t[1][a.scan_ta[scan][ci]];
@@ -970,7 +971,8 @@
             else if ( ci == 2 ) pr = (pred[2] += diff);
             else pr = (pred[3] += diff);
             mine[(0 ^ sw) << 3] = (int16_t)(DEQ ? pr * (int)q[0] : pr);
-            for ( int k = 1; k < 64; ) {
+            int k = 1;
+            while ( k < 64 ) {
                 src_fill(r);
                 const int rs = decode_symbol(r, tac);
                 const int run = rs >> 4;
@@ -986,6 +988,7 @@
                     k += 16;
                 }
             }
+            ext = gj_cext_of(min(k, 64) - 1);
         }
         __syncwarp();
         int target;
@@ -997,6 +1000,7 @@
         else {
             target = mybase + (L.interleaved ? L.blk_off[a.scan_comp[0][ci]] : 0) + mcu;
         }
+        if ( live && b < nblocks ) cext[target] = (uint8_t)ext;
         for ( int j = 0; j < SPW / 4; j++ ) {
             const int i = 4 * j + (lane >> 3);
             const int c = lane & 7;
@@ -1023,12 +1027,13 @@
     0,  1,  8,  16, 9,  2,  3,  10, 17, 24, 32, 25, 18, 11, 4,  5,  12, 19, 26, 33, 40, 48,
     41, 34, 27, 20, 13, 6,  7,  14, 21, 28, 35, 42, 49, 56, 57, 50, 43, 36, 29, 22, 15, 23,
     30, 37, 44, 51, 58, 59, 52, 45, 38, 31, 39, 46, 53, 60, 61, 54, 47, 55, 62, 63};
-__global__ void k_coef_to_natural(const int16_t* __restrict__ in, int16_t* __restrict__ out, size_t nblocks)
+__global__ void k_coef_to_natural(const int16_t* __restrict__ in, const uint8_t* __restrict__ cext, int16_t* __restrict__ out,
+                                  size_t nblocks)
 {
     const size_t i = (size_t)blockIdx.x * blockDim.x + threadIdx.x;
     if ( i >= nblocks * 64 ) return;
     const int k = (int)(i & 63);
-    out[(i & ~(size_t)63) + c_zz2nat[k]] = in[i];
+    out[(i & ~(size_t)63) + c_zz2nat[k]] = !cext || gj_cext_holds(cext[i >> 6], k) ? in[i] : (int16_t)0;
 }
 
 }
@@ -1155,19 +1160,19 @@
     const dim3 grid((warps + HD_THREADS / 32 - 1) / (HD_THREADS / 32));
     if ( a->dequantize )
         gj_launch_pdl(k_huff_decode<true>, dim3(grid), dim3(HD_THREADS), 0, stream, a->d_file, a->d_file + a->file_size, a->d_seg_off,
-                      a->seg_count, a->seg_mcu, *a, own, a->d_coef, a->d_tables);
+                      a->seg_count, a->seg_mcu, *a, own, a->d_coef, a->d_cext, a->d_tables);
     else
         gj_launch_pdl(k_huff_decode<false>, dim3(grid), dim3(HD_THREADS), 0, stream, a->d_file, a->d_file + a->file_size, a->d_seg_off,
-                      a->seg_count, a->seg_mcu, *a, own, a->d_coef, a->d_tables);
+                      a->seg_count, a->seg_mcu, *a, own, a->d_coef, a->d_cext, a->d_tables);
     return cudaGetLastError() == cudaSuccess ? 0 : -1;
 }
 
-extern "C" int gj_coef_to_host_natural(const int16_t* d_coef, size_t count, int16_t* h_out, gj_stream_t stream)
+extern "C" int gj_coef_to_host_natural(const int16_t* d_coef, const uint8_t* d_cext, size_t count, int16_t* h_out, gj_stream_t stream)
 {
     int16_t* d_tmp = nullptr;
     if ( cudaMalloc(&d_tmp, count * sizeof(int16_t)) != cudaSuccess ) return -1;
     const size_t nblocks = count / 64;
-    k_coef_to_natural<<<(unsigned)((count + 255) / 256), 256, 0, stream>>>(d_coef, d_tmp, nblocks);
+    k_coef_to_natural<<<(unsigned)((count + 255) / 256), 256, 0, stream>>>(d_coef, d_cext, d_tmp, nblocks);
     cudaMemcpyAsync(h_out, d_tmp, count * sizeof(int16_t), cudaMemcpyDeviceToHost, stream);
     const cudaError_t e = cudaStreamSynchronize(stream);
     cudaFree(d_tmp);
diff --git a/gpujpeg_b200/csrc/gj_internal.h b/gpujpeg_b200/csrc/gj_internal.h
--- a/gpujpeg_b200/csrc/gj_internal.h
+++ b/gpujpeg_b200/csrc/gj_internal.h
@@ -231,16 +231,16 @@
 
 int gj_launch_fdct_rgb444_rows(const uint8_t* d_raw, int width, int height, int pitch, int16_t* d_coef, uint64_t* d_nzmask,
                                int bcx, int bcy, int by0, int by1, const struct gj_dev_enc_tables* d_tables, gj_stream_t stream);
-int gj_launch_idct_rgb444_rows(const int16_t* d_coef, int bcx, int bcy, int by0, int by1, const int comp_tq[3], uint8_t* d_raw,
-                               int width, int height, int pitch, int idct_flavour, int coef_dequantized,
-                               const struct gj_dev_dec_tables* d_tables, gj_stream_t stream);
+int gj_launch_idct_rgb444_rows(const int16_t* d_coef, const uint8_t* d_cext, int bcx, int bcy, int by0, int by1,
+                               const int comp_tq[3], uint8_t* d_raw, int width, int height, int pitch, int idct_flavour,
+                               int coef_dequantized, const struct gj_dev_dec_tables* d_tables, gj_stream_t stream);
 
 int gj_launch_fdct_rgb_ss_rows(const uint8_t* d_raw, int width, int height, int pitch, int16_t* d_coef, uint64_t* d_nzmask,
                                const struct gj_comp_geo comp[3], int my0, int my1, const struct gj_dev_enc_tables* h_tables,
                                gj_stream_t stream);
-int gj_launch_idct_rgb_ss_rows(const int16_t* d_coef, const struct gj_comp_geo comp[3], int my0, int my1, const int comp_tq[3],
-                               uint8_t* d_raw, int width, int height, int pitch, int idct_flavour, int coef_dequantized,
-                               const struct gj_dev_dec_tables* h_tables, gj_stream_t stream);
+int gj_launch_idct_rgb_ss_rows(const int16_t* d_coef, const uint8_t* d_cext, const struct gj_comp_geo comp[3], int my0, int my1,
+                               const int comp_tq[3], uint8_t* d_raw, int width, int height, int pitch, int idct_flavour,
+                               int coef_dequantized, const struct gj_dev_dec_tables* h_tables, gj_stream_t stream);
 
 struct gj_huff_enc_args {
     const int16_t* d_coef;
@@ -270,6 +270,8 @@
 int gj_launch_huffman_place(const struct gj_huff_enc_args* a, gj_stream_t stream);
 #define GJ_HUFF_COUNTS_BYTES (2 * 2 * 256 * sizeof(uint64_t))
 int gj_launch_huffman_stats(const struct gj_huff_enc_args* a, uint64_t* d_counts, gj_stream_t stream);
+
+#define GJ_CEXT_FULL 8
 
 struct gj_huff_dec_args {
     const uint8_t* d_file;
@@ -298,6 +300,7 @@
     int scan_td[GJ_MAX_COMP][GJ_MAX_COMP], scan_ta[GJ_MAX_COMP][GJ_MAX_COMP];
     int scan_tq[GJ_MAX_COMP][GJ_MAX_COMP];
     int16_t* d_coef;
+    uint8_t* d_cext;
     const struct gj_dev_dec_tables* d_tables;
 };
 int gj_launch_huffman_decode(const struct gj_huff_dec_args* a, gj_stream_t stream);
@@ -328,6 +331,7 @@
     const uint8_t* d_list_code;
     uint32_t* d_error;
     int16_t* d_coef;
+    uint8_t* d_cext;
     size_t coef_count;
     int dequantize;
     int comp_count;
@@ -340,21 +344,21 @@
                           uint8_t* d_list_code, uint32_t* d_list_cpos, uint32_t list_cap, uint8_t* d_clean, uint32_t* d_result,
                           uint32_t* d_other, uint32_t other_cap, gj_stream_t stream);
 
-int gj_launch_idct_rgb444(const int16_t* d_coef, int bcx, int bcy, const int comp_tq[3], uint8_t* d_raw, int width,
-                          int height, int pitch, int idct_flavour, int coef_dequantized,
+int gj_launch_idct_rgb444(const int16_t* d_coef, const uint8_t* d_cext, int bcx, int bcy, const int comp_tq[3], uint8_t* d_raw,
+                          int width, int height, int pitch, int idct_flavour, int coef_dequantized,
                           const struct gj_dev_dec_tables* d_tables, gj_stream_t stream);
 
 int gj_launch_fdct_rgb_ss(const uint8_t* d_raw, int width, int height, int pitch, int16_t* d_coef, uint64_t* d_nzmask,
                           const struct gj_comp_geo comp[3], const struct gj_dev_enc_tables* h_tables, gj_stream_t stream);
-int gj_launch_idct_rgb_ss(const int16_t* d_coef, const struct gj_comp_geo comp[3], const int comp_tq[3], uint8_t* d_raw,
-                          int width, int height, int pitch, int idct_flavour, int coef_dequantized,
+int gj_launch_idct_rgb_ss(const int16_t* d_coef, const uint8_t* d_cext, const struct gj_comp_geo comp[3], const int comp_tq[3],
+                          uint8_t* d_raw, int width, int height, int pitch, int idct_flavour, int coef_dequantized,
                           const struct gj_dev_dec_tables* h_tables, gj_stream_t stream);
 
 int gj_launch_fdct_samples(const uint8_t* d_raw, const struct gj_raw_layout* raw, int16_t* d_coef, uint64_t* d_nzmask,
                            const struct gj_comp_geo* comp, int comp_count, const uint8_t* comp_tbl,
                            const struct gj_dev_enc_tables* h_tables, gj_stream_t stream);
-int gj_launch_idct_samples(const int16_t* d_coef, const struct gj_comp_geo* comp, int comp_count, const int* comp_tq,
-                           uint8_t* d_raw, const struct gj_raw_layout* raw, int idct_flavour, int coef_dequantized,
+int gj_launch_idct_samples(const int16_t* d_coef, const uint8_t* d_cext, const struct gj_comp_geo* comp, int comp_count,
+                           const int* comp_tq, uint8_t* d_raw, const struct gj_raw_layout* raw, int idct_flavour, int coef_dequantized,
                            const struct gj_dev_dec_tables* h_tables, gj_stream_t stream);
 
 int gj_launch_convert_in(const uint8_t* d_raw, const struct gj_raw_layout* raw, enum gpujpeg_pixel_format fmt, int color_space,
@@ -371,7 +375,7 @@
 void gj_planes_layout(struct gj_raw_layout* l, struct gj_comp_geo padded[GJ_MAX_COMP], const struct gj_comp_geo* comp,
                       int comp_count);
 
-int gj_coef_to_host_natural(const int16_t* d_coef, size_t count, int16_t* h_out, gj_stream_t stream);
+int gj_coef_to_host_natural(const int16_t* d_coef, const uint8_t* d_cext, size_t count, int16_t* h_out, gj_stream_t stream);
 
 int gj_cuda_malloc(void** p, size_t size);
 int gj_cuda_free(void* p);
diff --git a/gpujpeg_b200/csrc/gj_progressive.cu b/gpujpeg_b200/csrc/gj_progressive.cu
--- a/gpujpeg_b200/csrc/gj_progressive.cu
+++ b/gpujpeg_b200/csrc/gj_progressive.cu
@@ -34,10 +34,12 @@
     gj_prog_segment<KIND>(S, s_tab, clean, cs, ce > cs ? ce : cs, s, coef);
 }
 
-__global__ void __launch_bounds__(DQ_THREADS) k_prog_zero(uint4* __restrict__ p, size_t n16)
+__global__ void __launch_bounds__(DQ_THREADS) k_prog_zero(uint4* __restrict__ p, size_t n16, uint8_t* __restrict__ cext)
 {
-    for ( size_t i = (size_t)blockIdx.x * blockDim.x + threadIdx.x; i < n16; i += (size_t)gridDim.x * blockDim.x )
+    for ( size_t i = (size_t)blockIdx.x * blockDim.x + threadIdx.x; i < n16; i += (size_t)gridDim.x * blockDim.x ) {
         p[i] = make_uint4(0u, 0u, 0u, 0u);
+        if ( (i & 7) == 0 ) cext[i >> 3] = GJ_CEXT_FULL;
+    }
 }
 
 struct DqComps {
@@ -66,7 +68,7 @@
     {
         const size_t n16 = a->coef_count / 8;
         const size_t blocks = (n16 + DQ_THREADS - 1) / DQ_THREADS;
-        k_prog_zero<<<(unsigned)(blocks < cap ? blocks : cap), DQ_THREADS, 0, stream>>>(reinterpret_cast<uint4*>(a->d_coef), n16);
+        k_prog_zero<<<(unsigned)(blocks < cap ? blocks : cap), DQ_THREADS, 0, stream>>>(reinterpret_cast<uint4*>(a->d_coef), n16, a->d_cext);
         if ( cudaGetLastError() != cudaSuccess ) return -1;
     }
     for ( int k = 0; k < a->scan_count; k++ ) {
```

After: 55440 (median of 6 runs). 1.04x the previous value.
